# h-walk/PSA

Hardware: AMD Instinct MI355X
Metric: SED throughput (k-points*timesteps*atoms/s) (higher is better)
Workload: dtype f32 (2xf16 split MFMA, fp32 accumulate)

## Files before the change

### include/psa_hip.h

```cpp
#ifndef PSA_HIP_H
#define PSA_HIP_H

#include <stdint.h>

#ifdef __cplusplus
extern "C" {
#endif

#define PSA_HIP_ABI_VERSION 6

#define PSA_OK          0
#define PSA_EINVAL     -1
#define PSA_EHIP       -2
#define PSA_EFFT       -3
#define PSA_ERCCL      -4
#define PSA_ESTATE     -5
#define PSA_ENOMEM     -6

#define PSA_SLOT_VELOCITIES 0
#define PSA_SLOT_POSITIONS  1
#define PSA_NUM_SLOTS       2

#define PSA_F_DISPLACEMENTS  0x1
#define PSA_F_INTENSITY      0x2

#define PSA_K1_AUTO   0
#define PSA_K1_WAVE   1
#define PSA_K1_MFMA32 2
#define PSA_K1_SPLIT_BF16 3

typedef struct psa_ctx psa_ctx;

int         psa_abi_version(void);
const char* psa_last_error(void);
int         psa_device_count(int* count);
int         psa_host_alloc(size_t bytes, void** out);
int         psa_host_free(void* p);
int         psa_create(int device, psa_ctx** out);
int         psa_destroy(psa_ctx* ctx);
int         psa_synchronize(psa_ctx* ctx);
int         psa_set_k1(psa_ctx* ctx, int selector);
#define PSA_OPT_PLANES         0
#define PSA_OPT_PLANES_BUDGET  1
#define PSA_OPT_PLANES_EAGER   2
#define PSA_OPT_PLANES_MIN_K   3
#define PSA_OPT_FOLD_PAIRS     4
#define PSA_OPT_FFT_PRIME      5
#define PSA_OPT_K1_LOADER_WAVES 6
#define PSA_OPT_K1_WIDE         7
#define PSA_OPT_K1_LOWRANK      8
#define PSA_OPT_K1_LOWRANK_MIN_K 9
#define PSA_OPT_K1_LOWRANK_MIN_LOCAL 10
#define PSA_OPT_VDOS_WORK_BYTES 11
#define PSA_OPT_MODES_WORK_BYTES 12
#define PSA_OPT_DYNAMIC_WORK_BYTES 13
#define PSA_OPT_K1_LOWRANK_PAIR 15
int         psa_set_option(psa_ctx* ctx, int option, int64_t value);
int         psa_option_info(int index, int32_t* option, int64_t* default_value, const char** name);
int         psa_device_info(psa_ctx* ctx, char* name, int name_len,
                            int* compute_units, int64_t* hbm_bytes);

int psa_data_upload(psa_ctx* ctx, int slot, const float* host, int64_t T, int64_t N);
int psa_data_alloc(psa_ctx* ctx, int slot, int64_t T, int64_t N);
int psa_data_download(psa_ctx* ctx, int slot, float* host, int64_t t0, int64_t nt);
int psa_data_release(psa_ctx* ctx, int slot);
int psa_data_shape(psa_ctx* ctx, int slot, int64_t* T, int64_t* N);

int psa_data_fill_synthetic(psa_ctx* ctx, int slot, uint64_t seed, int64_t t_offset, int n_modes,
                            const float* amp, const int32_t* mode_comp,
                            const float* ct, const float* st,
                            const float* ca, const float* sa);

int psa_mean_positions(psa_ctx* ctx, int slot, float* mean_host );

int psa_host_mean_frames(const float* x , int64_t T, int64_t cols, float* mean_out, int threads);

int psa_set_atom_weights(psa_ctx* ctx, const float* w , int64_t N);

int psa_set_segments(psa_ctx* ctx, int64_t L, int64_t hop, const float* window );

int psa_sed_project(psa_ctx* ctx, int slot,
                    const float* mean_pos_all,
                    const float* k_vectors, int64_t K_local,
                    int64_t K_total, int64_t k_offset,
                    const int32_t* group_idx, const int64_t* group_off, int32_t G,
                    int32_t flags);

int psa_sed_project_upload(psa_ctx* ctx, int slot, const float* host, int64_t T, int64_t N,
                           const float* mean_pos_all, const float* k_vectors, int64_t K,
                           const int32_t* group_idx, const int64_t* group_off, int32_t G,
                           int32_t flags);

int psa_sed_finalize(psa_ctx* ctx, void* out_host, size_t out_bytes,
                     float* out_intensity, size_t out_intensity_bytes);

int psa_sed_calculate(psa_ctx* ctx, int slot, const float* mean_pos_all,
                      const float* k_vectors, int64_t K,
                      const int32_t* group_idx, const int64_t* group_off, int32_t G,
                      int32_t flags, void* out_host, size_t out_bytes,
                      float* out_intensity, size_t out_intensity_bytes);

int psa_vdos(psa_ctx* ctx, int slot, const float* mean_pos_all ,
             const int32_t* group_idx, const int64_t* group_off, int32_t G,
             int32_t flags , float* out_host , size_t out_bytes);

int psa_sed_modes(psa_ctx* ctx, int slot, const float* mean_pos_all, const float* k_vectors, int64_t K,
                  const int32_t* group_idx, const int64_t* group_off, int32_t B,
                  const void* eig , int64_t M, int32_t flags ,
                  float* out_host , size_t out_bytes);

int psa_sed_covariance(psa_ctx* ctx, int slot, const float* mean_pos_all, const float* k_vectors, int64_t K,
                       const int32_t* group_idx, const int64_t* group_off, int32_t B,
                       const float* freq_weights , int32_t n_w, int32_t flags ,
                       double* out_host , size_t out_bytes);

typedef struct {
    float   window_hwhm;
    int32_t half_window_bins;
    int32_t max_iter;
} psa_peak_opts;
int psa_fit_peaks(psa_ctx* ctx, const float* spec_host, int64_t F, int64_t C, double df, const int32_t* bands, int32_t lo,
                  int32_t hi, const psa_peak_opts* opts, float* fit , int32_t* info );
int psa_sed_modes_fit(psa_ctx* ctx, int slot, const float* mean_pos_all, const float* k_vectors, int64_t K,
                      const int32_t* group_idx, const int64_t* group_off, int32_t B, const void* eig, int64_t M,
                      int32_t flags, double df, const int32_t* bands, int32_t lo, int32_t hi, const psa_peak_opts* opts,
                      float* fit , int32_t* info , float* out_host, size_t out_bytes);

int psa_sed_modes_welch(psa_ctx* ctx, int slot, const float* mean_pos_all, const float* k_vectors, int64_t K,
                        const int32_t* group_idx, const int64_t* group_off, int32_t B,
                        const void* eig , int64_t M, int32_t flags ,
                        float* out_host , size_t out_bytes);
int psa_sed_modes_welch_fit(psa_ctx* ctx, int slot, const float* mean_pos_all, const float* k_vectors, int64_t K,
                            const int32_t* group_idx, const int64_t* group_off, int32_t B, const void* eig, int64_t M,
                            int32_t flags, double df, const int32_t* bands, int32_t lo, int32_t hi, const psa_peak_opts* opts,
                            float* fit , int32_t* info , float* out_host, size_t out_bytes);

int psa_dynamic_spectra(psa_ctx* ctx, const float* k_vectors, int64_t K, const int32_t* idx, int64_t n_g,
                        int32_t currents , float* out_host ,
                        size_t out_bytes);

int psa_lattice_spectra(psa_ctx* ctx, const double* box_inverse , const int32_t* indices , int64_t K,
                        const int32_t* bin_of , int64_t n_bins, const int32_t* idx, int64_t n_g,
                        int32_t currents , float* out_host ,
                        size_t out_bytes);

int psa_self_spectra(psa_ctx* ctx, const double* box_inverse , const int32_t* indices , int64_t K,
                     const int32_t* bin_of , int64_t n_bins, const int32_t* idx, int64_t n_g,
                     float* out_host , size_t out_bytes);

int psa_partial_spectra(psa_ctx* ctx, const double* box_inverse , const int32_t* indices , int64_t K,
                        const int32_t* bin_of , int64_t n_bins, const int32_t* idx, const int64_t* species_start ,
                        int32_t n_species, int32_t currents ,
                        float* out_host , size_t out_bytes);

int psa_lattice_correlations(psa_ctx* ctx, const double* box_inverse , const int32_t* indices , int64_t K,
                             const int32_t* bin_of , int64_t n_bins, const int32_t* idx, int64_t n_g,
                             int32_t currents , int64_t n_lags,
                             float* out_host , size_t out_bytes);

int psa_self_correlations(psa_ctx* ctx, const double* box_inverse , const int32_t* indices , int64_t K,
                          const int32_t* bin_of , int64_t n_bins, const int32_t* idx, int64_t n_g, int64_t n_lags,
                          float* out_host , size_t out_bytes);

int psa_displacement_moments(psa_ctx* ctx, const double* box , const double* box_inverse , const int32_t* idx,
                             const int64_t* group_start , int32_t n_groups, int64_t n_lags, int64_t origin_step,
                             int32_t unwrap, double* out_host , size_t out_bytes);

int psa_van_hove_self(psa_ctx* ctx, const double* box , const double* box_inverse , const int32_t* idx,
                      const int64_t* group_start , int32_t n_groups, const int64_t* lags , int64_t n_vh,
                      int64_t origin_step, int32_t unwrap, double dr, int32_t n_r, uint64_t* out_host ,
                      size_t out_bytes);

int psa_pair_histogram(psa_ctx* ctx, const double* box , const double* box_inverse , const int32_t* idx,
                       const int64_t* group_start , int32_t n_groups, const int64_t* lags , int64_t n_lags,
                       int64_t origin_step, double dr, int32_t n_r, uint64_t* out_host ,
                       size_t out_bytes);

int psa_angle_histogram(psa_ctx* ctx, const double* box , const double* box_inverse , const int32_t* idx,
                        const int64_t* group_start , int32_t n_groups, const double* r_cut , int64_t origin_step,
                        int32_t n_theta, uint64_t* angles , size_t angles_bytes,
                        uint64_t* coord , size_t coord_bytes, uint64_t* truncated );

int psa_bond_order(psa_ctx* ctx, const double* box , const double* box_inverse , const int32_t* idx,
                   const int64_t* group_start , int32_t n_groups, const double* r_cut , int64_t origin_step,
                   const int32_t* ls , int32_t n_ls, int32_t n_q, uint64_t* hist , size_t hist_bytes,
                   uint64_t* truncated , uint64_t* isolated , uint64_t* undefined ,
                   int64_t* x , int32_t* n );

#define PSA_KMAP_MIRROR 0x80000000u
int psa_k_pairs(const float* k_vectors, int64_t K, int32_t* kmap ,
                int32_t* unique_idx , int64_t* n_unique);
int psa_sed_set_kmap(psa_ctx* ctx, const int32_t* kmap, int64_t K_out);

int psa_lowrank_plan(const float* k_vectors, int64_t K, const float* mean_pos_all, int64_t N, const int32_t* idx,
                     int64_t n_g, int32_t* ok, double* geo, double* kappa, float* C, float* L, float* phi);

int psa_sed_single_bin(psa_ctx* ctx, int slot, const float* mean_pos_all, const float* k_vector,
                       const int32_t* idx, int64_t n_g, int32_t flags, int64_t i_w,
                       float* out_c64x3 );

int psa_slab_read(psa_ctx* ctx, int64_t row0, int64_t nrows, void* host);
int psa_slab_write(psa_ctx* ctx, int64_t row0, int64_t nrows, const void* host);

int psa_result_intensity(psa_ctx* ctx, float* out_host , size_t out_bytes);
int psa_result_chiral_phase(psa_ctx* ctx, int c1, int c2, float* out_host, size_t out_bytes);

int psa_last_timings(psa_ctx* ctx, double* ms );
int psa_k1_stats(psa_ctx* ctx, int64_t* launches, double* total_ms);
int psa_k1_lowrank_launches(psa_ctx* ctx, int64_t* launches);
int psa_k1_lowrank_pair_launches(psa_ctx* ctx, int64_t* launches);
int psa_lowrank_pair_image(int32_t n_stage, int64_t* index, int64_t* bytes);
int psa_debug_device_buffers(int64_t* count, int64_t* bytes);
#define PSA_SCRATCH_REAL 0
#define PSA_SCRATCH_INDEX 1
#define PSA_SCRATCH_STATE 2
int psa_debug_scratch_info(int index, const char** name, int32_t* cls);
int psa_debug_scratch_fill(psa_ctx* ctx, int byte, int64_t* buffers, int64_t* bytes);
int psa_oneoff_stats(psa_ctx* ctx, double* ms );

int psa_debug_phase_table(psa_ctx* ctx, const float* mean_pos_all,
                          const float* k_vectors, int64_t K,
                          const int32_t* idx, int64_t n_g, int64_t N,
                          void* out_host);
int psa_debug_project_only(psa_ctx* ctx, int slot, const float* mean_pos_all,
                           const float* k_vectors, int64_t K,
                           const int32_t* idx, int64_t n_g, int32_t flags,
                           void* out_host);
int psa_debug_project_route(psa_ctx* ctx, int slot, const float* mean_pos_all,
                            const float* k_vectors, int64_t K,
                            const int32_t* idx, int64_t n_g, int32_t flags,
                            void* out_host);
int psa_debug_project_frames(psa_ctx* ctx, int slot, const float* mean_pos_all,
                             const float* k_vectors, int64_t K,
                             const int32_t* idx, int64_t n_g, int32_t flags,
                             int64_t t_begin, int64_t t_count, void* out_host);
int psa_debug_mode_power(psa_ctx* ctx, const void* S_host, const void* eig, int32_t B, int64_t K, int64_t M, int64_t T,
                         float* out_host);
int psa_debug_covariance(psa_ctx* ctx, const void* S_host , int32_t B, int64_t K,
                         int64_t T, const float* freq_weights, int32_t n_w, double scale, double* out_host);
int psa_debug_mode_power_welch(psa_ctx* ctx, const void* S_host, const void* eig, int32_t B, int64_t K, int64_t M, int64_t L,
                               int64_t ns, int64_t seg_block, float scale, float* out_host);
int psa_debug_dynamic_project(psa_ctx* ctx, const float* k_vectors, int64_t K, const int32_t* idx, int64_t n_g,
                              int32_t currents, void* out_host);
int psa_debug_dynamic_sincos(psa_ctx* ctx, const float* turns, int64_t n, float* out_host);
int psa_debug_lattice_project(psa_ctx* ctx, const double* box_inverse, const int32_t* indices, int64_t K, const int32_t* idx,
                              int64_t n_g, int32_t currents, void* out_host);
int psa_debug_self_series(psa_ctx* ctx, const double* box_inverse, const int32_t* indices, int64_t K, const int32_t* idx,
                          int64_t n_g, void* out_host);
int psa_debug_dynamic_power(psa_ctx* ctx, const void* seg_host, const float* k_vectors , int64_t K, int32_t currents,
                            int64_t n_seg, int64_t L, int64_t k_block, int64_t seg_block, float scale, float* out_host);
int psa_debug_lattice_shell(psa_ctx* ctx, const void* seg_host, const float* khat , const int32_t* bin_of ,
                            int64_t K, int64_t n_bins, int32_t currents, int64_t n_seg, int64_t L, int64_t k_block,
                            int64_t seg_block, double norm, float* out_host);
int psa_debug_self_power(psa_ctx* ctx, const void* work_host, int64_t na, int64_t nv, int64_t n_seg, int64_t L,
                         const int32_t* groups, int64_t n_groups, int64_t cols, const double* scale, int32_t mirror,
                         int64_t n_chunks, int64_t atom_block, int64_t vec_block, int64_t seg_block, float* out_host);
int psa_debug_partial_project(psa_ctx* ctx, const double* box_inverse, const int32_t* indices, int64_t K, const int32_t* idx,
                              const int64_t* species_start, int32_t n_species, int32_t currents, void* out_host);
int psa_debug_partial_power(psa_ctx* ctx, const void* seg_host, const float* khat , const int32_t* bin_of ,
                            int64_t K, int64_t n_bins, int32_t n_species, int32_t currents, int64_t n_seg, int64_t L,
                            int64_t k_block, int64_t seg_block, double norm, float* out_host);
int psa_debug_plane_cache(psa_ctx* ctx, int64_t* n_sets, int64_t* bytes);

#define PSA_UNIQUE_ID_BYTES 128
int psa_comm_unique_id(void* out );
int psa_comm_init(psa_ctx* ctx, const void* unique_id, int rank, int nranks);
int psa_comm_destroy(psa_ctx* ctx);
int psa_comm_selftest(psa_ctx* ctx);
int psa_sed_gather(psa_ctx* ctx, int root, const int64_t* k_offsets, const int64_t* k_counts);
int psa_comm_barrier(psa_ctx* ctx);

int psa_sed_fs_project(psa_ctx* ctx, int slot, const float* mean_pos_all,
                       const float* k_vectors, int64_t K_total,
                       const int32_t* idx, int64_t n_g, int32_t flags,
                       int64_t T_total, int64_t k_offset, int64_t k_count);
int psa_sed_fs_exchange(psa_ctx* ctx, const int64_t* t_offsets, const int64_t* t_counts,
                        const int64_t* k_offsets, const int64_t* k_counts);
int psa_sed_fs_read(psa_ctx* ctx, int64_t k0, int64_t nk, void* host);
int psa_sed_fs_write(psa_ctx* ctx, int64_t t0, int64_t nt, const void* host);
int psa_sed_fs_finish(psa_ctx* ctx, int32_t first_group);

int psa_debug_correlation_transform(psa_ctx* ctx, const double* X_host, int64_t fields, int64_t P, int64_t cols, int64_t L,
                                    int64_t n_seg, int64_t n_lags, int32_t as_float32, float* out_host);

int psa_debug_unwrap(psa_ctx* ctx, const double* box , const double* box_inverse , const int32_t* idx, int64_t n_g,
                     int32_t unwrap, double* out_u , int32_t* out_images );

int psa_debug_pair_fractions(psa_ctx* ctx, const double* box_inverse , const int32_t* idx, int64_t n_g,
                             float* out );

int psa_debug_pair_plan(const int64_t* sizes , int32_t n_groups, int32_t sym, int64_t n_origins, int64_t* out );

int psa_debug_neighbour_lists(psa_ctx* ctx, const double* box , const double* box_inverse , const int32_t* idx,
                              const int64_t* group_start , int32_t n_groups, const double* r_cut , int64_t frame,
                              int32_t* count , int32_t* list );

#ifdef __cplusplus
}
#endif
#endif
```

### psa_amd/_hip.py

```python
from __future__ import annotations

import ctypes as C
import os
import threading
import weakref
from pathlib import Path
from typing import Optional, Sequence

import numpy as np

LIB_PATH = Path(__file__).resolve().parent / "csrc" / "libpsa_hip.so"

SLOT_VELOCITIES, SLOT_POSITIONS = 0, 1
F_DISPLACEMENTS, F_INTENSITY = 0x1, 0x2
K1_AUTO, K1_WAVE, K1_MFMA32, K1_SPLIT_BF16 = 0, 1, 2, 3
OPT_PLANES, OPT_PLANES_BUDGET, OPT_PLANES_EAGER, OPT_PLANES_MIN_K, OPT_FOLD_PAIRS, OPT_FFT_PRIME = 0, 1, 2, 3, 4, 5
OPT_K1_LOADER_WAVES = 6
OPT_K1_WIDE = 7
OPT_K1_LOWRANK = 8
OPT_K1_LOWRANK_MIN_K = 9
OPT_K1_LOWRANK_MIN_LOCAL = 10
OPT_VDOS_WORK_BYTES = 11
OPT_MODES_WORK_BYTES = 12
OPT_DYNAMIC_WORK_BYTES = 13
OPT_K1_LOWRANK_PAIR = 15
KMAP_MIRROR = 0x80000000
ABI_VERSION = 6
COV_CHAIN = 128
COV_FOLDS = 32
COV_TILE = 64
COV_CHUNK = COV_CHAIN * COV_FOLDS
COV_MAX_ROWS = 96
DYN_THREADS = 256
DYN_ATOMS = 512
DYN_CHAIN = 128
DYN_FRAMES = 4
DYN_SINCOS_ERR = 2.6e-7
LAT_THREADS = 256
LAT_KS = 512
LAT_ATOMS = 128
LAT_TABLE = 3584
LAT_CHAIN = 128
LAT_FRAMES = 4
LAT_MAX_INDEX = 64
LAT_MAX_ENTRIES = 3 * (2 * LAT_MAX_INDEX + 1)
PARTIAL_MAX_SPECIES = 8
SELF_THREADS = 256
SELF_ATOMS = 4
SELF_FRAMES = 64
SELF_ENTRIES = 24
SELF_KS = 64
MSD_LAGS = 256
MSD_ORIGINS = 1024
MSD_WINDOW = 1280
MSD_MAX_GROUPS = 8
MSD_MAX_BINS = 1024
MSD_MAX_VH_LAGS = 64
MSD_UNWRAP_FRAMES = 64
MSD_UNWRAP_ATOMS = 16
PAIR_TILE = 256
PAIR_MAX_BINS = 1024
PAIR_MAX_LAGS = 64
PAIR_MAX_SPECIES = 8
ANGLE_MAX_NEIGHBOURS = 64
ANGLE_MAX_BINS = 1024
ORDER_MAX_L = 12
ORDER_MAX_LS = 8
ORDER_MAX_BINS = 1024
ORDER_SHIFT = 24
UNIQUE_ID_BYTES = 128
TIMING_NAMES = ("h2d", "phase", "project", "fft", "epilogue", "gather", "transpose", "d2h")

_f32p = C.POINTER(C.c_float)
_i32p = C.POINTER(C.c_int32)
_i64p = C.POINTER(C.c_int64)
_f64p = C.POINTER(C.c_double)
_u64p = C.POINTER(C.c_uint64)
_ctx = C.c_void_p

SIGNATURES = {
    "psa_abi_version": (C.c_int, []),
    "psa_last_error": (C.c_char_p, []),
    "psa_device_count": (C.c_int, [C.POINTER(C.c_int)]),
    "psa_host_alloc": (C.c_int, [C.c_size_t, C.POINTER(C.c_void_p)]),
    "psa_host_free": (C.c_int, [C.c_void_p]),
    "psa_create": (C.c_int, [C.c_int, C.POINTER(_ctx)]),
    "psa_destroy": (C.c_int, [_ctx]),
    "psa_synchronize": (C.c_int, [_ctx]),
    "psa_set_k1": (C.c_int, [_ctx, C.c_int]),
    "psa_set_option": (C.c_int, [_ctx, C.c_int, C.c_int64]),
    "psa_device_info": (C.c_int, [_ctx, C.c_char_p, C.c_int, C.POINTER(C.c_int), _i64p]),
    "psa_data_upload": (C.c_int, [_ctx, C.c_int, _f32p, C.c_int64, C.c_int64]),
    "psa_data_alloc": (C.c_int, [_ctx, C.c_int, C.c_int64, C.c_int64]),
    "psa_data_download": (C.c_int, [_ctx, C.c_int, _f32p, C.c_int64, C.c_int64]),
    "psa_data_release": (C.c_int, [_ctx, C.c_int]),
    "psa_data_shape": (C.c_int, [_ctx, C.c_int, _i64p, _i64p]),
    "psa_data_fill_synthetic": (C.c_int, [_ctx, C.c_int, C.c_uint64, C.c_int64, C.c_int, _f32p, _i32p,
                                          _f32p, _f32p, _f32p, _f32p]),
    "psa_mean_positions": (C.c_int, [_ctx, C.c_int, _f32p]),
    "psa_host_mean_frames": (C.c_int, [_f32p, C.c_int64, C.c_int64, _f32p, C.c_int]),
    "psa_set_atom_weights": (C.c_int, [_ctx, _f32p, C.c_int64]),
    "psa_set_segments": (C.c_int, [_ctx, C.c_int64, C.c_int64, _f32p]),
    "psa_sed_project": (C.c_int, [_ctx, C.c_int, _f32p, _f32p, C.c_int64, C.c_int64, C.c_int64,
                                  _i32p, _i64p, C.c_int32, C.c_int32]),
    "psa_sed_project_upload": (C.c_int, [_ctx, C.c_int, _f32p, C.c_int64, C.c_int64, _f32p, _f32p, C.c_int64,
                                         _i32p, _i64p, C.c_int32, C.c_int32]),
    "psa_sed_finalize": (C.c_int, [_ctx, C.c_void_p, C.c_size_t, _f32p, C.c_size_t]),
    "psa_sed_calculate": (C.c_int, [_ctx, C.c_int, _f32p, _f32p, C.c_int64, _i32p, _i64p,
                                    C.c_int32, C.c_int32, C.c_void_p, C.c_size_t, _f32p, C.c_size_t]),
    "psa_vdos": (C.c_int, [_ctx, C.c_int, _f32p, _i32p, _i64p, C.c_int32, C.c_int32, _f32p, C.c_size_t]),
    "psa_sed_modes": (C.c_int, [_ctx, C.c_int, _f32p, _f32p, C.c_int64, _i32p, _i64p, C.c_int32, C.c_void_p, C.c_int64,
                                C.c_int32, _f32p, C.c_size_t]),
    "psa_fit_peaks": (C.c_int, [_ctx, _f32p, C.c_int64, C.c_int64, C.c_double, _i32p, C.c_int32, C.c_int32, C.c_void_p,
                                _f32p, _i32p]),
    "psa_sed_modes_fit": (C.c_int, [_ctx, C.c_int, _f32p, _f32p, C.c_int64, _i32p, _i64p, C.c_int32, C.c_void_p, C.c_int64,
                                    C.c_int32, C.c_double, _i32p, C.c_int32, C.c_int32, C.c_void_p, _f32p, _i32p, _f32p,
                                    C.c_size_t]),
    "psa_sed_modes_welch": (C.c_int, [_ctx, C.c_int, _f32p, _f32p, C.c_int64, _i32p, _i64p, C.c_int32, C.c_void_p, C.c_int64,
                                      C.c_int32, _f32p, C.c_size_t]),
    "psa_sed_modes_welch_fit": (C.c_int, [_ctx, C.c_int, _f32p, _f32p, C.c_int64, _i32p, _i64p, C.c_int32, C.c_void_p,
                                          C.c_int64, C.c_int32, C.c_double, _i32p, C.c_int32, C.c_int32, C.c_void_p, _f32p,
                                          _i32p, _f32p, C.c_size_t]),
    "psa_dynamic_spectra": (C.c_int, [_ctx, _f32p, C.c_int64, _i32p, C.c_int64, C.c_int32, _f32p, C.c_size_t]),
    "psa_debug_dynamic_project": (C.c_int, [_ctx, _f32p, C.c_int64, _i32p, C.c_int64, C.c_int32, C.c_void_p]),
    "psa_debug_dynamic_sincos": (C.c_int, [_ctx, _f32p, C.c_int64, _f32p]),
    "psa_lattice_spectra": (C.c_int, [_ctx, _f64p, _i32p, C.c_int64, _i32p, C.c_int64, _i32p, C.c_int64, C.c_int32,
                                      _f32p, C.c_size_t]),
    "psa_debug_lattice_project": (C.c_int, [_ctx, _f64p, _i32p, C.c_int64, _i32p, C.c_int64, C.c_int32, C.c_void_p]),
    "psa_self_spectra": (C.c_int, [_ctx, _f64p, _i32p, C.c_int64, _i32p, C.c_int64, _i32p, C.c_int64, _f32p,
                                   C.c_size_t]),
    "psa_debug_self_series": (C.c_int, [_ctx, _f64p, _i32p, C.c_int64, _i32p, C.c_int64, C.c_void_p]),
    "psa_debug_dynamic_power": (C.c_int, [_ctx, C.c_void_p, _f32p, C.c_int64, C.c_int32, C.c_int64, C.c_int64, C.c_int64, C.c_int64,
                                          C.c_float, _f32p]),
    "psa_debug_lattice_shell": (C.c_int, [_ctx, C.c_void_p, _f32p, _i32p, C.c_int64, C.c_int64, C.c_int32, C.c_int64, C.c_int64,
                                          C.c_int64, C.c_int64, C.c_double, _f32p]),
    "psa_debug_self_power": (C.c_int, [_ctx, C.c_void_p, C.c_int64, C.c_int64, C.c_int64, C.c_int64, _i32p, C.c_int64, C.c_int64,
                                       _f64p, C.c_int32, C.c_int64, C.c_int64, C.c_int64, C.c_int64, _f32p]),
    "psa_partial_spectra": (C.c_int, [_ctx, _f64p, _i32p, C.c_int64, _i32p, C.c_int64, _i32p, _i64p, C.c_int32,
                                      C.c_int32, _f32p, C.c_size_t]),
    "psa_debug_partial_project": (C.c_int, [_ctx, _f64p, _i32p, C.c_int64, _i32p, _i64p, C.c_int32, C.c_int32,
                                            C.c_void_p]),
    "psa_debug_partial_power": (C.c_int, [_ctx, C.c_void_p, _f32p, _i32p, C.c_int64, C.c_int64, C.c_int32, C.c_int32, C.c_int64,
                                          C.c_int64, C.c_int64, C.c_int64, C.c_double, _f32p]),
    "psa_lattice_correlations": (C.c_int, [_ctx, _f64p, _i32p, C.c_int64, _i32p, C.c_int64, _i32p, C.c_int64,
                                           C.c_int32, C.c_int64, _f32p, C.c_size_t]),
    "psa_self_correlations": (C.c_int, [_ctx, _f64p, _i32p, C.c_int64, _i32p, C.c_int64, _i32p, C.c_int64,
                                        C.c_int64, _f32p, C.c_size_t]),
    "psa_debug_correlation_transform": (C.c_int, [_ctx, _f64p, C.c_int64, C.c_int64, C.c_int64, C.c_int64,
                                                  C.c_int64, C.c_int64, C.c_int32, _f32p]),
    "psa_displacement_moments": (C.c_int, [_ctx, _f64p, _f64p, _i32p, _i64p, C.c_int32, C.c_int64,
                                           C.c_int64, C.c_int32, _f64p, C.c_size_t]),
    "psa_van_hove_self": (C.c_int, [_ctx, _f64p, _f64p, _i32p, _i64p, C.c_int32, _i64p, C.c_int64,
                                    C.c_int64, C.c_int32, C.c_double, C.c_int32, _u64p, C.c_size_t]),
    "psa_debug_unwrap": (C.c_int, [_ctx, _f64p, _f64p, _i32p, C.c_int64, C.c_int32,
                                   _f64p, _i32p]),
    "psa_pair_histogram": (C.c_int, [_ctx, _f64p, _f64p, _i32p, _i64p, C.c_int32, _i64p, C.c_int64,
                                     C.c_int64, C.c_double, C.c_int32, _u64p, C.c_size_t]),
    "psa_debug_pair_fractions": (C.c_int, [_ctx, _f64p, _i32p, C.c_int64, _f32p]),
    "psa_debug_pair_plan": (C.c_int, [_i64p, C.c_int32, C.c_int32, C.c_int64, _i64p]),
    "psa_angle_histogram": (C.c_int, [_ctx, _f64p, _f64p, _i32p, _i64p, C.c_int32, _f64p,
                                      C.c_int64, C.c_int32, _u64p, C.c_size_t, _u64p, C.c_size_t,
                                      _u64p]),
    "psa_debug_neighbour_lists": (C.c_int, [_ctx, _f64p, _f64p, _i32p, _i64p, C.c_int32,
                                            _f64p, C.c_int64, _i32p, _i32p]),
    "psa_bond_order": (C.c_int, [_ctx, _f64p, _f64p, _i32p, _i64p, C.c_int32, _f64p, C.c_int64,
                                 _i32p, C.c_int32, C.c_int32, _u64p, C.c_size_t, _u64p, _u64p, _u64p,
                                 _i64p, _i32p]),
    "psa_k_pairs": (C.c_int, [_f32p, C.c_int64, _i32p, _i32p, _i64p]),
    "psa_lowrank_plan": (C.c_int, [_f32p, C.c_int64, _f32p, C.c_int64, _i32p, C.c_int64, _i32p, _f64p,
                                   _f64p, _f32p, _f32p, _f32p]),
    "psa_sed_set_kmap": (C.c_int, [_ctx, _i32p, C.c_int64]),
    "psa_sed_single_bin": (C.c_int, [_ctx, C.c_int, _f32p, _f32p, _i32p, C.c_int64, C.c_int32, C.c_int64, _f32p]),
    "psa_slab_read": (C.c_int, [_ctx, C.c_int64, C.c_int64, C.c_void_p]),
    "psa_slab_write": (C.c_int, [_ctx, C.c_int64, C.c_int64, C.c_void_p]),
    "psa_result_intensity": (C.c_int, [_ctx, _f32p, C.c_size_t]),
    "psa_result_chiral_phase": (C.c_int, [_ctx, C.c_int, C.c_int, _f32p, C.c_size_t]),
    "psa_last_timings": (C.c_int, [_ctx, _f64p]),
    "psa_k1_stats": (C.c_int, [_ctx, _i64p, _f64p]),
    "psa_k1_lowrank_launches": (C.c_int, [_ctx, _i64p]),
    "psa_k1_lowrank_pair_launches": (C.c_int, [_ctx, _i64p]),
    "psa_lowrank_pair_image": (C.c_int, [C.c_int32, _i64p, _i64p]),
    "psa_oneoff_stats": (C.c_int, [_ctx, _f64p]),
    "psa_option_info": (C.c_int, [C.c_int, C.POINTER(C.c_int32), _i64p, C.POINTER(C.c_char_p)]),
    "psa_debug_device_buffers": (C.c_int, [_i64p, _i64p]),
    "psa_debug_scratch_info": (C.c_int, [C.c_int, C.POINTER(C.c_char_p), C.POINTER(C.c_int32)]),
    "psa_debug_scratch_fill": (C.c_int, [_ctx, C.c_int, _i64p, _i64p]),
    "psa_debug_phase_table": (C.c_int, [_ctx, _f32p, _f32p, C.c_int64, _i32p, C.c_int64,
                                        C.c_int64, C.c_void_p]),
    "psa_debug_project_only": (C.c_int, [_ctx, C.c_int, _f32p, _f32p, C.c_int64, _i32p,
                                         C.c_int64, C.c_int32, C.c_void_p]),
    "psa_debug_project_route": (C.c_int, [_ctx, C.c_int, _f32p, _f32p, C.c_int64, _i32p,
                                          C.c_int64, C.c_int32, C.c_void_p]),
    "psa_debug_project_frames": (C.c_int, [_ctx, C.c_int, _f32p, _f32p, C.c_int64, _i32p,
                                           C.c_int64, C.c_int32, C.c_int64, C.c_int64, C.c_void_p]),
    "psa_debug_mode_power": (C.c_int, [_ctx, C.c_void_p, C.c_void_p, C.c_int32, C.c_int64, C.c_int64, C.c_int64, _f32p]),
    "psa_debug_mode_power_welch": (C.c_int, [_ctx, C.c_void_p, C.c_void_p, C.c_int32, C.c_int64, C.c_int64, C.c_int64,
                                             C.c_int64, C.c_int64, C.c_float, _f32p]),
    "psa_sed_covariance": (C.c_int, [_ctx, C.c_int, _f32p, _f32p, C.c_int64, _i32p, _i64p, C.c_int32, _f32p, C.c_int32, C.c_int32,
                                     C.c_void_p, C.c_size_t]),
    "psa_debug_covariance": (C.c_int, [_ctx, C.c_void_p, C.c_int32, C.c_int64, C.c_int64, _f32p, C.c_int32, C.c_double,
                                       C.c_void_p]),
    "psa_debug_plane_cache": (C.c_int, [_ctx, _i64p, _i64p]),
    "psa_comm_unique_id": (C.c_int, [C.c_void_p]),
    "psa_comm_init": (C.c_int, [_ctx, C.c_void_p, C.c_int, C.c_int]),
    "psa_comm_destroy": (C.c_int, [_ctx]),
    "psa_comm_selftest": (C.c_int, [_ctx]),
    "psa_sed_gather": (C.c_int, [_ctx, C.c_int, _i64p, _i64p]),
    "psa_comm_barrier": (C.c_int, [_ctx]),
    "psa_sed_fs_project": (C.c_int, [_ctx, C.c_int, _f32p, _f32p, C.c_int64, _i32p, C.c_int64, C.c_int32,
                                     C.c_int64, C.c_int64, C.c_int64]),
    "psa_sed_fs_exchange": (C.c_int, [_ctx, _i64p, _i64p, _i64p, _i64p]),
    "psa_sed_fs_read": (C.c_int, [_ctx, C.c_int64, C.c_int64, C.c_void_p]),
    "psa_sed_fs_write": (C.c_int, [_ctx, C.c_int64, C.c_int64, C.c_void_p]),
    "psa_sed_fs_finish": (C.c_int, [_ctx, C.c_int32]),
}


class PeakOpts(C.Structure):
    _fields_ = [("window_hwhm", C.c_float), ("half_window_bins", C.c_int32), ("max_iter", C.c_int32)]


class PsaHipError(RuntimeError):
    """A libpsa_hip entry point returned a non-zero code."""


_lib = None
_lib_lock = threading.Lock()


def load_library() -> C.CDLL:
    global _lib
    with _lib_lock:
        if _lib is not None:
            return _lib
        path = Path(os.environ.get("PSA_HIP_LIBRARY", LIB_PATH))
        if not path.exists():
            raise PsaHipError(
                f"{path} not found: build it with `make -C psa_amd/csrc` (needs hipcc, gfx950). "
                "psa_amd has no CPU fallback.")
        os.environ.setdefault("HSA_ENABLE_IPC_MODE_LEGACY", "0")
        lib = C.CDLL(str(path))
        for name, (res, args) in SIGNATURES.items():
            fn = getattr(lib, name)
            fn.restype, fn.argtypes = res, args
        _lib = lib
        return lib


def _check(rc: int, what: str):
    if rc != 0:
        msg = load_library().psa_last_error().decode("utf-8", "replace")
        if rc == -1 and "out of bounds" in msg:
            raise ValueError(msg)
        raise PsaHipError(f"{what} failed (rc={rc}): {msg}")


def _f32(a: np.ndarray):
    return a.ctypes.data_as(_f32p)


def _as_f32(a, shape_tail=None) -> np.ndarray:
    arr = np.ascontiguousarray(a, dtype=np.float32)
    if shape_tail is not None and arr.shape[1:] != shape_tail:
        raise ValueError(f"expected (*,{shape_tail}) array, got {arr.shape}")
    return arr


def device_count() -> int:
    n = C.c_int(0)
    _check(load_library().psa_device_count(C.byref(n)), "psa_device_count")
    return n.value


def option_table():
    lib, rows = load_library(), []
    opt, default, name = C.c_int32(0), C.c_int64(0), C.c_char_p()
    while lib.psa_option_info(len(rows), C.byref(opt), C.byref(default), C.byref(name)) == 0:
        rows.append((opt.value, name.value.decode(), default.value))
    return rows


def device_buffers():
    n, b = C.c_int64(0), C.c_int64(0)
    _check(load_library().psa_debug_device_buffers(C.byref(n), C.byref(b)), "psa_debug_device_buffers")
    return n.value, b.value


SCRATCH_CLASSES = ("real", "index", "state")


def scratch_table():
    lib, rows = load_library(), []
    name, cls = C.c_char_p(), C.c_int32(0)
    while lib.psa_debug_scratch_info(len(rows), C.byref(name), C.byref(cls)) == 0:
        rows.append((name.value.decode(), SCRATCH_CLASSES[cls.value]))
    return rows


def k_pairs(k_vectors):
    kv = _as_f32(k_vectors, (3,)) if len(k_vectors) else np.zeros((0, 3), np.float32)
    K = kv.shape[0]
    kmap, uidx, n = np.zeros(K, np.int32), np.zeros(K, np.int32), C.c_int64(0)
    _check(load_library().psa_k_pairs(_f32(kv), K, kmap.ctypes.data_as(_i32p), uidx.ctypes.data_as(_i32p), C.byref(n)),
           "psa_k_pairs")
    return kmap.view(np.uint32), uidx[:n.value].copy()


def lowrank_plan(k_vectors, mean_pos_all, idx=None):
    kv = _as_f32(k_vectors, (3,))
    mean = _as_f32(mean_pos_all, (3,))
    K, N = kv.shape[0], mean.shape[0]
    ix = None if idx is None else np.ascontiguousarray(idx, np.int32)
    n_g = N if ix is None else ix.size
    ok, geo = C.c_int32(0), np.zeros(12, np.float64)
    kappa, cm = np.zeros(64, np.float64), np.zeros((K, 64), np.complex64)
    lw, phi = np.zeros((K, 64), np.float32), np.zeros(K, np.complex64)
    _check(load_library().psa_lowrank_plan(_f32(kv), K, _f32(mean), N, None if ix is None else ix.ctypes.data_as(_i32p), n_g,
                                           C.byref(ok), geo.ctypes.data_as(_f64p), kappa.ctypes.data_as(_f64p),
                                           cm.ctypes.data_as(_f32p), _f32(lw), phi.ctypes.data_as(_f32p)), "psa_lowrank_plan")
    if not ok.value:
        return None
    return {"u": geo[0:3].copy(), "k0": geo[3:6].copy(), "x_c": geo[6], "h_x": geo[7], "width": geo[8],
            "interval": int(geo[9]), "d_bound": geo[10], "dscale": geo[11], "kappa": kappa, "C": cm, "L": lw, "phi": phi}


def lowrank_pair_image(n_stage: int):
    index, nbytes = np.zeros((512, 32 * int(n_stage)), np.int64), C.c_int64(0)
    _check(load_library().psa_lowrank_pair_image(int(n_stage), index.ctypes.data_as(_i64p), C.byref(nbytes)), "psa_lowrank_pair_image")
    return index, nbytes.value


def host_mean_frames(x: np.ndarray, threads: int = 0) -> np.ndarray:
    if x.dtype != np.float32 or not x.flags.c_contiguous or x.ndim < 2 or x.shape[0] < 1 or x.size == 0:
        raise ValueError("host_mean_frames needs a non-empty C-contiguous float32 array")
    out = np.empty(x.shape[1:], np.float32)
    cols = int(np.prod(x.shape[1:], dtype=np.int64))
    _check(load_library().psa_host_mean_frames(_f32(x), x.shape[0], cols, _f32(out), int(threads)), "psa_host_mean_frames")
    return out


def pack_groups(groups: Optional[Sequence[np.ndarray]]):
    if groups is None:
        return None, None, 1
    off = np.zeros(len(groups) + 1, dtype=np.int64)
    off[1:] = np.cumsum([len(g) for g in groups])
    idx = (np.concatenate([np.asarray(g).ravel() for g in groups]) if off[-1] > 0
           else np.zeros(0, dtype=np.int64))
    if idx.size and (idx.min() < 0 or idx.max() >= 2 ** 31):
        raise ValueError("Atom indices in basis out of bounds.")
    return np.ascontiguousarray(idx, dtype=np.int32), off, len(groups)


class _PinnedPool:

    granule = 2 << 20
    min_bytes = 1 << 20
    keep_bytes = 4 << 30
    max_live_bytes = 16 << 30

    def __init__(self):
        self._idle = {}
        self._idle_bytes = 0
        self._live_bytes = 0
        self._lock = threading.Lock()
        self.stats = {"recycled": 0, "allocated": 0, "pageable": 0}

    def _give_back(self, address: int, size: int):
        with self._lock:
            self._live_bytes -= size
            if self._idle_bytes + size <= self.keep_bytes:
                self._idle.setdefault(size, []).append(address)
                self._idle_bytes += size
                return
        load_library().psa_host_free(C.c_void_p(address))

    def empty(self, shape, dtype) -> np.ndarray:
        dtype = np.dtype(dtype)
        nbytes = int(np.prod(shape, dtype=np.int64)) * dtype.itemsize
        if nbytes < self.min_bytes:
            return np.empty(shape, dtype)
        size = -(-nbytes // self.granule) * self.granule
        with self._lock:
            if self._live_bytes + size > self.max_live_bytes:
                self.stats["pageable"] += 1
                return np.empty(shape, dtype)
            self._live_bytes += size
            stack = self._idle.get(size)
            address = stack.pop() if stack else None
            if address is not None:
                self._idle_bytes -= size
        if address is None:
            p = C.c_void_p()
            try:
                _check(load_library().psa_host_alloc(size, C.byref(p)), "psa_host_alloc")
            except PsaHipError:
                with self._lock:
                    self._live_bytes -= size
                    self.stats["pageable"] += 1
                return np.empty(shape, dtype)
            address = p.value
            self.stats["allocated"] += 1
        else:
            self.stats["recycled"] += 1
        block = (C.c_char * size).from_address(address)
        weakref.finalize(block, self._give_back, address, size)
        return np.frombuffer(block, dtype=dtype, count=nbytes // dtype.itemsize).reshape(shape)

    def drain(self):
        with self._lock:
            idle, self._idle, self._idle_bytes = self._idle, {}, 0
        for stack in idle.values():
            for address in stack:
                load_library().psa_host_free(C.c_void_p(address))


_pinned_pool = _PinnedPool()


def pinned_empty(shape, dtype) -> np.ndarray:
    return _pinned_pool.empty(shape, dtype)


_SAMPLE_CACHE = {}


def _sample_positions(shape):
    hit = _SAMPLE_CACHE.get(shape)
    if hit is None:
        size = int(np.prod(shape, dtype=np.int64))
        lin = np.arange(0, size, max(1, size // 1021), dtype=np.int64)[:1021]
        if size > 2048:
            lin = np.concatenate([lin, np.sort(np.random.default_rng(size).integers(0, size, 1021)), [size - 1]])
        if len(_SAMPLE_CACHE) > 64:
            _SAMPLE_CACHE.clear()
        hit = _SAMPLE_CACHE[shape] = (lin, np.unravel_index(lin, shape))
    return hit


class Engine:

    def __init__(self, device: Optional[int] = None):
        self._lib = load_library()
        if device is None:
            device = int(os.environ.get("PSA_HIP_DEVICE", os.environ.get("LOCAL_RANK", "0")))
            n = device_count()
            if n == 0:
                raise PsaHipError("no HIP device visible; psa_amd has no CPU fallback")
            device %= n
        h = _ctx()
        _check(self._lib.psa_create(int(device), C.byref(h)), "psa_create")
        self._h = h
        self.device = int(device)
        self._resident = {}
        self._converted = {}
        self.lock = threading.RLock()
        self.rank, self.nranks = 0, 1
        self.result_serial = 0
        self.segment_length = 0

    def close(self):
        if getattr(self, "_h", None):
            self._lib.psa_destroy(self._h)
            self._h = None

    def __del__(self):
        try:
            self.close()
        except Exception:
            pass

    def synchronize(self):
        _check(self._lib.psa_synchronize(self._h), "psa_synchronize")

    def set_k1(self, selector: int):
        _check(self._lib.psa_set_k1(self._h, selector), "psa_set_k1")

    def device_info(self) -> dict:
        name = C.create_string_buffer(256)
        cu, mem = C.c_int(0), C.c_int64(0)
        _check(self._lib.psa_device_info(self._h, name, 256, C.byref(cu), C.byref(mem)),
               "psa_device_info")
        return {"name": name.value.decode(), "compute_units": cu.value, "hbm_bytes": mem.value}

    @staticmethod
    def _fingerprint(a: np.ndarray) -> int:
        if a.size == 0:
            return 0
        base = a
        while base is not None and not isinstance(base, np.memmap):
            base = getattr(base, "base", None)
        if base is not None and getattr(base, "filename", None):
            try:
                st = os.stat(base.filename)
                return hash((str(base.filename), st.st_size, st.st_mtime_ns, a.shape, a.strides))
            except OSError:
                pass
        lin, idx = _sample_positions(a.shape)
        if a.flags.c_contiguous:
            return hash(a.reshape(-1)[lin].tobytes())
        return hash(a[idx].tobytes())

    def _as_device_layout(self, slot: int, array: np.ndarray) -> np.ndarray:
        if array.ndim != 3 or array.shape[2] != 3:
            raise ValueError("trajectory array must be (frames, atoms, 3)")
        if array.dtype == np.float32 and array.flags.c_contiguous:
            return array
        held = self._converted.get(slot)
        fp = self._fingerprint(array)
        if held is not None and held[0]() is array and held[1] == fp:
            return held[2]
        conv = np.ascontiguousarray(array, dtype=np.float32)
        try:
            self._converted[slot] = (weakref.ref(array), fp, conv)
        except TypeError:
            self._converted.pop(slot, None)
        return conv

    def is_resident(self, slot: int, array: np.ndarray) -> bool:
        held = self._resident.get(slot)
        if held is None or held[0] is None:
            return False
        a = array if held[0]() is array else self._as_device_layout(slot, array)
        return (held[0]() is a and held[1:3] == (a.ctypes.data, a.shape) and held[3] == self._fingerprint(a))

    def _note_resident(self, slot: int, a: np.ndarray):
        try:
            ref = weakref.ref(a)
        except TypeError:
            ref = None
        self._resident[slot] = (ref, a.ctypes.data, a.shape, self._fingerprint(a))

    def ensure_resident(self, slot: int, array: np.ndarray):
        if self.is_resident(slot, array):
            return
        a = self._as_device_layout(slot, array)
        T, N = a.shape[0], a.shape[1]
        _check(self._lib.psa_data_upload(self._h, slot, _f32(a), T, N), "psa_data_upload")
        self._note_resident(slot, a)

    def invalidate(self, slot: Optional[int] = None):
        if slot is None:
            self._resident.clear()
            self._converted.clear()
        else:
            self._resident.pop(slot, None)
            self._converted.pop(slot, None)

    def alloc(self, slot: int, T: int, N: int):
        _check(self._lib.psa_data_alloc(self._h, slot, T, N), "psa_data_alloc")
        self._resident[slot] = (None, None, (T, N, 3), None)

    def fill_synthetic(self, slot: int, seed: int, amp, comp, ct, st, ca, sa, t_offset: int = 0):
        amp = np.ascontiguousarray(amp, np.float32)
        comp = np.ascontiguousarray(comp, np.int32)
        tabs = [np.ascontiguousarray(x, np.float32) for x in (ct, st, ca, sa)]
        _check(self._lib.psa_data_fill_synthetic(
            self._h, slot, C.c_uint64(seed), int(t_offset), len(amp), _f32(amp), comp.ctypes.data_as(_i32p),
            *[_f32(t) for t in tabs]), "psa_data_fill_synthetic")

    def set_option(self, option: int, value: int):
        _check(self._lib.psa_set_option(self._h, option, int(value)), "psa_set_option")

    def reset_options(self):
        for option, _, default in option_table():
            self.set_option(option, default)

    def scratch_fill(self, byte: int):
        n, b = C.c_int64(0), C.c_int64(0)
        _check(self._lib.psa_debug_scratch_fill(self._h, int(byte), C.byref(n), C.byref(b)), "psa_debug_scratch_fill")
        return n.value, b.value

    def plane_cache(self):
        n, b = C.c_int64(0), C.c_int64(0)
        _check(self._lib.psa_debug_plane_cache(self._h, C.byref(n), C.byref(b)), "psa_debug_plane_cache")
        return n.value, b.value

    def download(self, slot: int, t0: int, nt: int) -> np.ndarray:
        T, N = self.shape(slot)
        out = np.empty((nt, N, 3), np.float32)
        _check(self._lib.psa_data_download(self._h, slot, _f32(out), t0, nt), "psa_data_download")
        return out

    def release(self, slot: int):
        _check(self._lib.psa_data_release(self._h, slot), "psa_data_release")
        self._resident.pop(slot, None)

    def shape(self, slot: int):
        T, N = C.c_int64(0), C.c_int64(0)
        _check(self._lib.psa_data_shape(self._h, slot, C.byref(T), C.byref(N)), "psa_data_shape")
        return T.value, N.value

    def mean_positions(self, slot: int) -> np.ndarray:
        _, N = self.shape(slot)
        out = np.empty((N, 3), np.float32)
        _check(self._lib.psa_mean_positions(self._h, slot, _f32(out)), "psa_mean_positions")
        return out

    def set_atom_weights(self, weights: Optional[np.ndarray]):
        if weights is None:
            _check(self._lib.psa_set_atom_weights(self._h, None, 0), "psa_set_atom_weights")
            return
        w = np.ascontiguousarray(weights, np.float32)
        if w.ndim != 1 or w.size == 0:
            raise ValueError(f"atom weights must be a non-empty (N,) array, got shape {w.shape}")
        if not np.all(np.isfinite(w)):
            raise ValueError("atom weights must be finite")
        _check(self._lib.psa_set_atom_weights(self._h, _f32(w), w.shape[0]), "psa_set_atom_weights")

    def set_segments(self, segments):
        if segments is None:
            _check(self._lib.psa_set_segments(self._h, 0, 0, None), "psa_set_segments")
            self.segment_length = 0
            return
        w = np.ascontiguousarray(segments.window_array(), np.float32)
        _check(self._lib.psa_set_segments(self._h, segments.length, segments.hop, _f32(w)), "psa_set_segments")
        self.segment_length = segments.length

    def project(self, slot, mean_pos_all, k_vectors, groups=None, flags=0,
                K_total=None, k_offset=0):
        mean = _as_f32(mean_pos_all, (3,))
        kv = _as_f32(k_vectors, (3,)) if len(k_vectors) else np.zeros((0, 3), np.float32)
        idx, off, G = pack_groups(groups)
        K_local = kv.shape[0]
        self.result_serial += 1
        _check(self._lib.psa_sed_project(
            self._h, slot, _f32(mean), _f32(kv), K_local,
            K_local if K_total is None else K_total, k_offset,
            idx.ctypes.data_as(_i32p) if idx is not None else None,
            off.ctypes.data_as(_i64p) if off is not None else None, G, flags),
            "psa_sed_project")

    def project_upload(self, slot, array, mean_pos_all, k_vectors, groups=None, flags=0):
        a = self._as_device_layout(slot, array)
        mean = _as_f32(mean_pos_all, (3,))
        kv = _as_f32(k_vectors, (3,))
        idx, off, G = pack_groups(groups)
        self._resident.pop(slot, None)
        self.result_serial += 1
        _check(self._lib.psa_sed_project_upload(
            self._h, slot, _f32(a), a.shape[0], a.shape[1], _f32(mean), _f32(kv), kv.shape[0],
            idx.ctypes.data_as(_i32p) if idx is not None else None,
            off.ctypes.data_as(_i64p) if off is not None else None, G, flags), "psa_sed_project_upload")
        self._note_resident(slot, a)

    def finalize(self, T: int, K: int, intensity: bool, fetch: bool = True, with_intensity: bool = False):
        if not fetch:
            _check(self._lib.psa_sed_finalize(self._h, None, 0, None, 0), "psa_sed_finalize")
            return (None, None) if with_intensity else None
        out = pinned_empty((T, K), np.float32) if intensity else pinned_empty((T, K, 3), np.complex64)
        inten = pinned_empty((T, K), np.float32) if with_intensity and not intensity else None
        _check(self._lib.psa_sed_finalize(self._h, out.ctypes.data_as(C.c_void_p), out.nbytes,
                                          _f32(inten) if inten is not None else None,
                                          inten.nbytes if inten is not None else 0), "psa_sed_finalize")
        return (out, inten) if with_intensity else out

    def single_bin(self, slot, mean_pos_all, k_vector, idx, i_w: int, flags=0) -> np.ndarray:
        mean = _as_f32(mean_pos_all, (3,))
        kv = np.ascontiguousarray(k_vector, np.float32).reshape(3)
        ii = None if idx is None else np.ascontiguousarray(idx, np.int32)
        out = np.empty(3, np.complex64)
        _check(self._lib.psa_sed_single_bin(
            self._h, slot, _f32(mean), _f32(kv), ii.ctypes.data_as(_i32p) if ii is not None else None,
            0 if ii is None else len(ii), flags, int(i_w), out.ctypes.data_as(_f32p)), "psa_sed_single_bin")
        return out

    def calculate(self, slot, mean_pos_all, k_vectors, groups=None, flags=0, with_intensity: bool = False):
        T, _ = self.shape(slot)
        T = self.segment_length or T
        mean = _as_f32(mean_pos_all, (3,))
        kv = _as_f32(k_vectors, (3,))
        idx, off, G = pack_groups(groups)
        K = kv.shape[0]
        intensity = bool(flags & F_INTENSITY)
        out = pinned_empty((T, K), np.float32) if intensity else pinned_empty((T, K, 3), np.complex64)
        inten = pinned_empty((T, K), np.float32) if with_intensity and not intensity else None
        self.result_serial += 1
        _check(self._lib.psa_sed_calculate(
            self._h, slot, _f32(mean), _f32(kv), K,
            idx.ctypes.data_as(_i32p) if idx is not None else None,
            off.ctypes.data_as(_i64p) if off is not None else None, G, flags,
            out.ctypes.data_as(C.c_void_p), out.nbytes,
            _f32(inten) if inten is not None else None, inten.nbytes if inten is not None else 0), "psa_sed_calculate")
        return (out, inten) if with_intensity else out

    def vdos(self, slot, mean_pos_all, groups=None, flags=0) -> np.ndarray:
        T, N = self.shape(slot)
        L = self.segment_length or T
        mean = None if mean_pos_all is None else _as_f32(mean_pos_all, (3,))
        idx, off, G = pack_groups(groups)
        out = np.empty((G, 3, L // 2 + 1), np.float32)
        _check(self._lib.psa_vdos(
            self._h, slot, _f32(mean) if mean is not None else None,
            idx.ctypes.data_as(_i32p) if idx is not None else None,
            off.ctypes.data_as(_i64p) if off is not None else None, G, flags, _f32(out), out.nbytes), "psa_vdos")
        return np.ascontiguousarray(out.transpose(2, 0, 1))

    @staticmethod
    def _index_args(idx):
        if idx is None:
            return None, None, 0
        ii = np.ascontiguousarray(idx, np.int32).ravel()
        keep = ii if ii.size else np.zeros(1, np.int32)
        return keep, keep.ctypes.data_as(_i32p), int(ii.size)

    @staticmethod
    def _dynamic_args(k_vectors, idx):
        return (_as_f32(np.asarray(k_vectors, np.float32).reshape(-1, 3), (3,)),) + Engine._index_args(idx)

    def dynamic_spectra(self, k_vectors, idx=None, currents: bool = True) -> np.ndarray:
        T, _ = self.shape(SLOT_POSITIONS)
        L = self.segment_length or T
        kv, keep, ip, n_g = self._dynamic_args(k_vectors, idx)
        out = np.empty((3 if currents else 1, L, kv.shape[0]), np.float32)
        _check(self._lib.psa_dynamic_spectra(self._h, _f32(kv), kv.shape[0], ip, n_g, 1 if currents else 0, _f32(out), out.nbytes),
               "psa_dynamic_spectra")
        return out

    def debug_dynamic_project(self, k_vectors, idx=None, currents: bool = True) -> np.ndarray:
# ... 582 lines not shown
```

### psa_amd/csrc/api_core.hip

```cpp
#include "api_internal.h"

#include <unistd.h>

#include <atomic>
#include <filesystem>

namespace psa {

thread_local std::string g_error;


void set_error(const char* fmt, ...) {
    char    buf[1024];
    va_list ap;
    va_start(ap, fmt);
    vsnprintf(buf, sizeof(buf), fmt, ap);
    va_end(ap);
    g_error = buf;
}

static std::atomic<int64_t> g_devbuf_count{0}, g_devbuf_bytes{0};

int DevBuf::reserve(size_t bytes) {
    if (bytes <= cap) return PSA_OK;
// ... 228 lines not shown
static const int SCRATCH_ZERO = 0;

}

psa_ctx::psa_ctx() {
    for (const psa::Option& o : psa::OPTIONS) this->*o.field = o.def;
}

psa_ctx::~psa_ctx() {
    if (stream) (void)hipStreamSynchronize(stream);
    if (fft_primer.joinable()) fft_primer.join();
    if (comm) (void)ncclCommDestroy(comm);
    for (auto& p : timing.pending) {
        (void)hipEventDestroy(p.e0);
        (void)hipEventDestroy(p.e1);
    }
    for (auto ev : timing.pool) (void)hipEventDestroy(ev);
    psa::stager_release(this);
    if (d2h_stream) (void)hipStreamDestroy(d2h_stream);
    if (d2h_ready) (void)hipEventDestroy(d2h_ready);
    if (stream) (void)hipStreamDestroy(stream);
}

using namespace psa;

extern "C" {

int psa_abi_version(void) { return PSA_HIP_ABI_VERSION; }

const char* psa_last_error(void) { return g_error.c_str(); }

int psa_device_count(int* count) {
    PSA_REQUIRE(count != nullptr, "null count");
    PSA_HIP_CHECK(hipGetDeviceCount(count));
    return PSA_OK;
}

int psa_host_alloc(size_t bytes, void** out) {
    PSA_REQUIRE(out != nullptr && bytes > 0, "bad argument");
    PSA_HIP_CHECK(hipHostMalloc(out, bytes, hipHostMallocDefault));
    return PSA_OK;
}

int psa_host_free(void* p) {
    if (p) PSA_HIP_CHECK(hipHostFree(p));
    return PSA_OK;
}

int psa_create(int device, psa_ctx** out) {
    PSA_REQUIRE(out != nullptr, "null out");
    int n = 0;
    PSA_HIP_CHECK(hipGetDeviceCount(&n));
    PSA_REQUIRE(device >= 0 && device < n, "device %d out of range (%d visible)", device, n);
    PSA_HIP_CHECK(hipSetDevice(device));
    hipDeviceProp_t prop;
    PSA_HIP_CHECK(hipGetDeviceProperties(&prop, device));
    PSA_REQUIRE(std::strncmp(prop.gcnArchName, "gfx950", 6) == 0,
                "libpsa_hip is built for gfx950 (MI355X) only; device %d is %s", device,
                prop.gcnArchName);
    static std::once_flag fft_once;
    std::call_once(fft_once, [] {
        if (!std::getenv("ROCFFT_RTC_CACHE_PATH")) {
            std::string dir;
            if (const char* e = std::getenv("PSA_CACHE_DIR")) dir = e;
            else if (const char* x = std::getenv("XDG_CACHE_HOME")) dir = std::string(x) + "/psa_amd";
            else if (const char* h = std::getenv("HOME")) dir = std::string(h) + "/.cache/psa_amd";
            if (!dir.empty()) {
                std::error_code ec;
                std::filesystem::create_directories(dir, ec);
                if (!ec && ::access(dir.c_str(), W_OK) == 0)
                    ::setenv("ROCFFT_RTC_CACHE_PATH", (dir + "/rocfft_rtc_cache.db").c_str(), 0);
            }
        }
        (void)rocfft_setup();
    });
    psa_ctx* c = new psa_ctx();
    c->device = device;
    c->compute_units = prop.multiProcessorCount;
    if (const char* v = std::getenv("PSA_K1_LOWRANK")) c->opt_k1_lowrank = std::atoi(v) != 0;
    if (const char* v = std::getenv("PSA_K1_LOWRANK_MIN_K")) c->opt_k1_lowrank_min_k = std::max(1, std::atoi(v));
    hipError_t e = hipStreamCreateWithFlags(&c->stream, hipStreamNonBlocking);
    if (e != hipSuccess) {
        delete c;
        set_error("hipStreamCreate failed: %s", hipGetErrorString(e));
        return PSA_EHIP;
    }
    *out = c;
    return PSA_OK;
}

int psa_destroy(psa_ctx* c) {
    if (!c) return PSA_OK;
    { Guard g(c); }
    (void)hipSetDevice(c->device);
    delete c;
    return PSA_OK;
}

int psa_debug_device_buffers(int64_t* count, int64_t* bytes) {
    PSA_REQUIRE(count != nullptr && bytes != nullptr, "null argument");
    *count = g_devbuf_count.load();
    *bytes = g_devbuf_bytes.load();
    return PSA_OK;
}

int psa_debug_scratch_info(int index, const char** name, int32_t* cls) {
    PSA_REQUIRE(index >= 0 && index < (int)std::size(SCRATCH), "no device buffer at index %d", index);
    if (name) *name = SCRATCH[index].name;
    if (cls) *cls = SCRATCH[index].cls;
    return PSA_OK;
}

int psa_debug_scratch_fill(psa_ctx* c, int byte, int64_t* buffers, int64_t* bytes) {
    PSA_TRY(enter(c));
    PSA_REQUIRE(byte >= -1 && byte <= 255, "the fill byte is 0 .. 255, or -1 to disarm");
    Guard g(c);
    PSA_HIP_CHECK(hipStreamSynchronize(c->stream));
    if (c->d2h_stream) PSA_HIP_CHECK(hipStreamSynchronize(c->d2h_stream));
    if (c->stager.copy_stream) PSA_HIP_CHECK(hipStreamSynchronize(c->stager.copy_stream));
    int64_t n = 0, total = 0;
    c->scratch_byte = byte;
    for (const Scratch& s : SCRATCH) {
        DevBuf& b = c->*s.member;
        b.fill = byte < 0 || s.cls == PSA_SCRATCH_STATE ? nullptr : s.cls == PSA_SCRATCH_REAL ? &c->scratch_byte : &SCRATCH_ZERO;
        if (!b.fill || !b.ptr) continue;
        PSA_HIP_CHECK(hipMemsetAsync(b.ptr, *b.fill, b.cap, c->stream));
        n += 1;
        total += (int64_t)b.cap;
    }
    PSA_HIP_CHECK(hipStreamSynchronize(c->stream));
    if (byte >= 0) c->slab_valid = c->out_valid = c->inten_valid = false;
    if (buffers) *buffers = n;
    if (bytes) *bytes = total;
    return PSA_OK;
}

int psa_synchronize(psa_ctx* c) {
    PSA_TRY(enter(c));
    Guard g(c);
    PSA_HIP_CHECK(hipStreamSynchronize(c->stream));
    return PSA_OK;
}

int psa_set_k1(psa_ctx* c, int selector) {
    PSA_TRY(enter(c));
    PSA_REQUIRE(selector == PSA_K1_AUTO || selector == PSA_K1_WAVE || selector == PSA_K1_MFMA32 ||
                    selector == PSA_K1_SPLIT_BF16,
                "unknown K1 selector %d", selector);
    Guard g(c);
    c->k1_selector = selector;
    return PSA_OK;
}

int psa_set_option(psa_ctx* c, int option, int64_t value) {
    PSA_TRY(enter(c));
    Guard g(c);
    for (const Option& o : OPTIONS) {
        if (o.id != option) continue;
        if (o.min == OPT_FLAG) value = value != 0;
        else if (o.min == 0) PSA_REQUIRE(value >= 0, "negative plane budget");
        else PSA_REQUIRE(value >= o.min, "%s must be >= %lld", o.name, (long long)o.min);
        c->*o.field = value;
        if (option == PSA_OPT_PLANES && !value) {
            PSA_HIP_CHECK(hipStreamSynchronize(c->stream));
            c->planes.clear();
        } else if (option == PSA_OPT_K1_LOWRANK && !value) {
            PSA_HIP_CHECK(hipStreamSynchronize(c->stream));
            for (DevBuf* b : {&c->d_lr_diff, &c->d_lr_qn, &c->d_lr_L, &c->d_lr_phi, &c->d_lr_f64}) b->release();
        }
        return PSA_OK;
    }
    set_error("unknown option %d", option);
    return PSA_EINVAL;
}

int psa_option_info(int index, int32_t* option, int64_t* default_value, const char** name) {
    PSA_REQUIRE(index >= 0 && index < (int)std::size(OPTIONS), "no option at index %d", index);
    if (option) *option = OPTIONS[index].id;
    if (default_value) *default_value = OPTIONS[index].def;
    if (name) *name = OPTIONS[index].name;
    return PSA_OK;
}

int psa_device_info(psa_ctx* c, char* name, int name_len, int* compute_units, int64_t* hbm_bytes) {
    PSA_TRY(enter(c));
    hipDeviceProp_t prop;
    PSA_HIP_CHECK(hipGetDeviceProperties(&prop, c->device));
    if (name && name_len > 0) {
        std::snprintf(name, (size_t)name_len, "%s (%s)", prop.name[0] ? prop.name : "AMD GPU",
                      prop.gcnArchName);
    }
    if (compute_units) *compute_units = prop.multiProcessorCount;
    if (hbm_bytes) *hbm_bytes = (int64_t)prop.totalGlobalMem;
    return PSA_OK;
}

int psa_last_timings(psa_ctx* c, double* ms) {
    PSA_TRY(enter(c));
    PSA_REQUIRE(ms != nullptr, "null output");
    Guard guard(c);
    TimingState& ts = timing(c);
    PSA_TRY(collect(c, ts));
    for (int i = 0; i < PSA_T_COUNT; ++i) {
        ms[i] = ts.acc[i];
        ts.acc[i] = 0.0;
    }
    return PSA_OK;
}

int psa_oneoff_stats(psa_ctx* c, double* ms) {
    PSA_TRY(enter(c));
    PSA_REQUIRE(ms != nullptr, "null output");
    Guard guard(c);
    for (int i = 0; i < 4; ++i) {
        ms[i] = c->oneoff_ms[i];
        c->oneoff_ms[i] = 0.0;
    }
    return PSA_OK;
}

int psa_k1_lowrank_launches(psa_ctx* c, int64_t* launches) {
    PSA_TRY(enter(c));
    PSA_REQUIRE(launches != nullptr, "null argument");
    *launches = c->lowrank_launches;
    return PSA_OK;
}

int psa_k1_lowrank_pair_launches(psa_ctx* c, int64_t* launches) {
    PSA_TRY(enter(c));
    PSA_REQUIRE(launches != nullptr, "null argument");
    *launches = c->lowrank_pair_launches;
    return PSA_OK;
}

int psa_k1_stats(psa_ctx* c, int64_t* launches, double* total_ms) {
    PSA_TRY(enter(c));
    Guard guard(c);
    TimingState& ts = timing(c);
    PSA_TRY(collect(c, ts));
    if (launches) *launches = ts.k1_launches;
    if (total_ms) *total_ms = ts.k1_ms;
    ts.k1_launches = 0;
    ts.k1_ms = 0.0;
    return PSA_OK;
}

}
```

### psa_amd/csrc/api_internal.h

```cpp
#pragma once
#include <algorithm>
#include <chrono>
#include <cmath>
#include <condition_variable>
#include <cstdlib>
#include <cstring>
#include <functional>
#include <thread>
#include <unordered_map>

#include "k1_f16.h"

namespace psa {

extern thread_local std::string g_error;

struct HostTimer {
    double*                               into;
    std::chrono::steady_clock::time_point t0 = std::chrono::steady_clock::now();
    explicit HostTimer(double* into_) : into(into_) {}
    ~HostTimer() { *into += std::chrono::duration<double, std::milli>(std::chrono::steady_clock::now() - t0).count(); }
};

struct Guard {
    std::lock_guard<std::mutex> lk;
    explicit Guard(psa_ctx* c) : lk(c->mu) {}
};

int          enter(psa_ctx* c);
inline int synchronised(psa_ctx* c, int rc, const char* entry) {
    if (hipStreamSynchronize(c->stream) != hipSuccess && rc == PSA_OK) {
        set_error("hipStreamSynchronize failed after %s", entry);
        return PSA_EHIP;
    }
    return rc;
}
TimingState& timing(psa_ctx* c);
int          get_event(TimingState& ts, hipEvent_t* ev);
int          collect(psa_ctx* c, TimingState& ts);

struct StageTimer {
    psa_ctx*     c;
    TimingState& ts;
    int          stage;
    hipEvent_t   e0 = nullptr, e1 = nullptr;
    bool         ok = false;
    StageTimer(psa_ctx* c_, int stage_) : c(c_), ts(timing(c_)), stage(stage_) {
        if (get_event(ts, &e0) == PSA_OK && get_event(ts, &e1) == PSA_OK &&
            hipEventRecord(e0, c->stream) == hipSuccess)
            ok = true;
    }
    ~StageTimer() {
        if (ok && hipEventRecord(e1, c->stream) == hipSuccess) {
            ts.pending.push_back({stage, e0, e1});
            return;
        }
        for (hipEvent_t ev : {e0, e1})
            if (ev) ts.pool.push_back(ev);
    }
};

int upload(psa_ctx* c, DevBuf& b, const void* host, size_t bytes);
int get_plan(psa_ctx* c, int64_t T, int64_t batch, FftPlan** out);
void prime_fft(psa_ctx* c, int64_t T);
int run_fft(psa_ctx* c, float2* data, int64_t T, int64_t batch);
int check_slot(psa_ctx* c, int slot);
int validate_groups(int64_t N, const int32_t* group_idx, const int64_t* group_off, int32_t G);

struct GroupView {
    int            slot = 0;
    bool           disp = false;
    int64_t        n_g = 0;
    const int*     d_idx = nullptr;
    const int32_t* h_idx = nullptr;
    PlaneSet*      ps = nullptr;
};
inline void set_group(const psa_ctx* c, const int32_t* group_idx, const int64_t* group_off, int gi, int64_t N, GroupView* v) {
    v->n_g = group_idx ? group_off[gi + 1] - group_off[gi] : N;
    v->d_idx = group_idx ? c->d_idx.as<int>() + group_off[gi] : nullptr;
    v->h_idx = group_idx ? group_idx + group_off[gi] : nullptr;
}

int  slot_absmax(psa_ctx* c, int slot);
int  group_absmax(psa_ctx* c, int slot, const int32_t* h_idx, int64_t n_g, unsigned* bits);
int  displaced_absmax(psa_ctx* c, int slot, const float* mean_host, const int32_t* h_idx, int64_t n_g, unsigned* bits);
int  stager_init(psa_ctx* c, size_t chunk_bytes);
void stager_release(psa_ctx* c);
int  staged_upload(psa_ctx* c, float* dev, const float* host, int64_t T, int64_t N,
                   const std::function<int(int64_t, int64_t, hipEvent_t)>& on_chunk);
int  data_alloc_locked(psa_ctx* c, int slot, int64_t T, int64_t N);
int  materialise_displacements(psa_ctx* c, GroupView* v, const float* mean_host);

struct ProjectArgs {
    int            slot;
    const float*   mean_pos_all;
    const float*   k_vectors;
    int64_t        K_local, K_total, k_offset;
    const int32_t* group_idx;
    const int64_t* group_off;
    int32_t        G, flags;
};

enum class GeomRule { product, bf16_anywhere, f32_only };

size_t planes_bytes_held(psa_ctx* c);
void   drop_stale_planes(psa_ctx* c);
int    get_planes(psa_ctx* c, const GroupView& v, int64_t K_local, const float* mean_host, PlaneSet** out);
int    group_source(psa_ctx* c, GroupView* v, const float* mean_host, int64_t K);
int    make_geom(psa_ctx* c, const GroupView& v, int64_t K_local, GeomRule rule, ProjGeom* g);
int    prepare_phase(psa_ctx* c, const GroupView& v, const ProjGeom& g, int64_t k_first);
int    launch_projection(psa_ctx* c, const GroupView& v, ProjGeom g, float2* d_q, int64_t q_stride, int64_t t_begin,
                         int64_t t_count);
int    prepare_block(psa_ctx* c, const GroupView& v, GeomRule rule, const ProjectArgs* lowrank, int64_t k_first, int64_t nk,
                     ProjGeom* g);
int    project_block(psa_ctx* c, const GroupView& v, const ProjectArgs* lowrank, int64_t k_first, int64_t nk, float2* d_q);
int    check_group_indices(const GroupView& v, int64_t N);
int    upload_single_group(psa_ctx* c, GroupView* v, int64_t N, const float* k_vectors, int64_t K, const float* mean_pos_all);
void   fold_pairs(const float* k, int64_t K, std::vector<int32_t>* kmap, std::vector<int32_t>* unique_idx);
int    install_kmap(psa_ctx* c, const std::vector<int32_t>& kmap);
struct LowRankPlan {
    bool                ok = false;
    const char*         why = "";
    double              u[3] = {0, 0, 0}, k0[3] = {0, 0, 0};
    double              x_c = 0, h_x = 0, width = 0;
    int64_t             interval = 0;
    double              kappa[LOWRANK_NODES] = {};
    double              d_bound = 0;
    float               dscale = 0.f;
    std::vector<double> kline;
    std::vector<float>  L;
    std::vector<float>  phi;
};
int plan_lowrank(const float* k, int64_t K, const float* mean_all, int64_t N, const int32_t* h_idx, int64_t n_g, LowRankPlan* p,
                 float* C = nullptr);
int prepare_lowrank(psa_ctx* c, const GroupView& v, const ProjectArgs& list, int64_t k_first, int64_t nk, ProjGeom* g);
struct ModesArgs {
    int            slot;
    const float*   mean_pos_all;
    const float*   k_vectors;
    int64_t        K;
    const int32_t* group_idx;
    const int64_t* group_off;
    int32_t        B;
    const float*   eig;
    int64_t        M;
    int32_t        flags;
    float*         out;
    size_t         out_bytes;
};
int modes_run(psa_ctx* c, const ModesArgs& a, bool segments, bool device_only);
struct ModesCall {
    int64_t                T = 0, N = 0, K = 0, M = 0;
    int32_t                B = 0;
    int                    MT = 0;
    size_t                 coef_k = 0;
    int64_t                per_k = 0;
    int64_t                kb_max = 0;
    ProjectArgs            list;
    std::vector<float>     coef;
    std::vector<GroupView> src;
};
int     modes_check_groups(psa_ctx* c, int slot, const float* mean_pos_all, const float* k_vectors, int64_t K, const int32_t* group_idx,
                           const int64_t* group_off, int32_t B, int32_t flags, ModesCall* m);
int     modes_upload(psa_ctx* c, ModesCall* m);
int64_t modes_block(const psa_ctx* c, const ModesCall& m, int64_t k0, int64_t kb);
int     modes_project(psa_ctx* c, const ModesCall& m, int64_t k0, int64_t nk, float2* d_work);
struct PeakArgs {
    int64_t        F, C;
    double         df;
    const int32_t* bands;
    int32_t        lo, hi;
    psa_peak_opts  opts;
    float*         fit;
    int32_t*       info;
    int            row0 = 0, row_end = 0;
};
int check_peak_args(const psa_peak_opts* opts, PeakArgs* a);
int peaks_run(psa_ctx* c, const float* d_spec, const PeakArgs& a);
struct DynCall {
    int64_t T = 0, N = 0, K = 0, n_g = 0;
    int     NC = 1, slices = 1;
    int     n_species = 1;
    bool    cut = false;
    int64_t L = 0, H = 0, n_seg = 0;
    int64_t n_lags = 0, P = 0;
    int64_t per_k = 0, unit = 0;
    int64_t kb = 0, bk = 0, bs = 0;
    std::vector<float> kappa, khat;
};
int dynamic_inputs(psa_ctx* c, const char* entry, int64_t K, const int32_t* idx, int64_t n_g, int32_t currents, DynCall* d);
int segment_shape(const psa_ctx* c, bool segments, DynCall* d);
int dynamic_plan(psa_ctx* c, DynCall* d);
struct PowerPass {
    int          NC = 1;
    int          n_species = 0;
    int64_t      L = 0, n_seg = 0, K = 0;
    float        scale = 0.f;
    const float* d_khat = nullptr;
    float*       d_out = nullptr;
    const int*   d_bins = nullptr;
    double*      d_acc = nullptr;
    int64_t      n_bins = 0;
};
using SegFill = std::function<int(int64_t k1, int64_t nb, int64_t s0, int64_t ns, const float2** d_seg)>;
int  power_block(psa_ctx* c, const PowerPass& p, int64_t k0, int64_t nk, int64_t bk, int64_t bs, const SegFill& fill);
struct BlockSource {
    std::function<int()>                                                     upload;
    std::function<int(int64_t block, int64_t k0, int64_t nk, float2* d_q)> project;
};
struct SpectraRun {
    BlockSource src;
    bool        pairs = false;
    int64_t     n_bins = 0;
    std::function<int(const float* d_power, const double* d_acc)> finish;
    float*      out_host = nullptr;
    size_t      out_bytes = 0;
};
int spectra_run(psa_ctx* c, const DynCall& d, const SpectraRun& a);
int debug_project_run(psa_ctx* c, const DynCall& d, const BlockSource& src, void* out_host);
struct DebugPower {
    const void*    seg_host = nullptr;
    const int32_t* bin_of = nullptr;
    int64_t        K = 0, n_bins = 0;
    int            n_species = 0;
    int32_t        currents = 0;
    int64_t        n_seg = 0, L = 0, k_block = 0, seg_block = 0;
    double         norm = 1.0;
    float          scale = 0.f;
    float*         out_host = nullptr;
    int64_t        bk = 0, bs = 0;
};
int debug_power_check(DebugPower* a);
int debug_power_run(psa_ctx* c, const DebugPower& a, const float* khat);
int  upload_segments(psa_ctx* c, DevBuf& b, const void* host, int64_t r0, int64_t nr, int64_t n_seg, int64_t s0, int64_t ns, int64_t L);
void bin_counts(const int32_t* bin_of, int64_t K, int64_t n_bins, std::vector<int64_t>* count);
int  sorted_bin_counts(const int32_t* bin_of, int64_t K, int64_t n_bins, std::vector<int64_t>* count);
void lattice_bins(const std::vector<int64_t>& count, double n_seg, double U, double L, std::vector<int32_t>* bin_start,
                  std::vector<double>* scale);
int  shell_begin(psa_ctx* c, size_t bytes, double** d_acc);
int  shell_finish(psa_ctx* c, int64_t n, int64_t n_bins, float* d_out);

int  lattice_inputs(const double* box_inverse, const int32_t* indices, int64_t K, const int32_t* bin_of, int64_t n_bins);
void lattice_box_parts(const double* B, float* hi, float* lo);
void lattice_order(const int32_t* indices, int64_t K, const int32_t* bin_of, int64_t kb, std::vector<int64_t>* order);
int  lattice_tile_entries(const int32_t* indices, const int64_t* members, int64_t nt, std::vector<uint16_t>* ent, uint32_t* slot);
struct LatCall {
    DynCall  d;
    bool     shell = false;
    int64_t  n_bins = 0;
    float    box_hi[9], box_lo[9];
    std::vector<int64_t>  block_tile0;
    std::vector<int32_t>  tile_off, dest;
    std::vector<uint16_t> ent;
    std::vector<uint32_t> slot;
    std::vector<int64_t>  count;
    std::vector<int32_t>  bin_start;
    std::vector<double>   scale;
};
int lattice_plan(const psa_ctx* c, const double* box_inverse, const int32_t* indices, const int32_t* bin_of, int64_t n_bins,
                 int64_t row_mult, LatCall* p);
int lattice_check(psa_ctx* c, const char* entry, const double* box_inverse, const int32_t* indices, int64_t K, const int32_t* bin_of,
                  int64_t n_bins, const int32_t* idx, int64_t n_g, int32_t currents, int64_t n_lags, LatCall* p);
int lattice_upload(psa_ctx* c, const LatCall& p, const int32_t* idx);
int lattice_project(psa_ctx* c, const LatCall& p, bool listed, int64_t a0, int64_t n_g, int64_t block, float2* d_q);
BlockSource lattice_source(psa_ctx* c, const LatCall& p, const int32_t* idx);
struct SelfCall {
    DynCall  d;
    bool     shell = false;
    int64_t  cols = 0;
    float    box_hi[9], box_lo[9];
    std::vector<int64_t>  order;
    std::vector<int32_t>  tile;
    std::vector<uint16_t> ent;
    std::vector<uint32_t> slot;
    std::vector<int32_t>  groups;
    std::vector<int64_t>  count;
    std::vector<double>   scale;
    int64_t  n_tiles = 0, kt_max = 0, n_groups = 0;
    int64_t  at = 0, vt = 0, bs = 0;
};
int self_check(psa_ctx* c, const char* entry, const double* box_inverse, const int32_t* indices, int64_t K, const int32_t* bin_of,
// ... 44 lines not shown
```

### psa_amd/csrc/api_lowrank.hip

```cpp
#include "api_internal.h"
#include "k1_lowrank_pair.h"

namespace psa {

namespace {
constexpr double LR_OMEGA = 30.0;
constexpr double LR_D_MAX = 1.0 / 8192.0;
}

int plan_lowrank(const float* k, int64_t K, const float* mean_all, int64_t N, const int32_t* h_idx, int64_t n_g, LowRankPlan* p,
                 float* C) {
    *p = LowRankPlan{};
    auto fail = [&](const char* why) {
        p->why = why;
        return PSA_OK;
    };
    if (K < 2) return fail("fewer than two k-vectors");
    if (n_g < 1) return fail("empty group");
    for (int64_t i = 0; i < 3 * K; ++i)
        if (!std::isfinite(k[i])) return fail("k-vector not finite");
    double  p0[3] = {k[0], k[1], k[2]}, far = 0.0;
    int64_t jf = 0;
    for (int64_t j = 1; j < K; ++j) {
        double d2 = 0.0;
        for (int i = 0; i < 3; ++i) d2 += ((double)k[3 * j + i] - p0[i]) * ((double)k[3 * j + i] - p0[i]);
        if (d2 > far) {
            far = d2;
            jf = j;
        }
    }
    if (!(far > 0.0)) return fail("all k-vectors equal");
    double u[3], nu = std::sqrt(far);
    for (int i = 0; i < 3; ++i) u[i] = ((double)k[3 * jf + i] - p0[i]) / nu;
    {
        int im = 0;
        for (int i = 1; i < 3; ++i)
            if (std::fabs(u[i]) > std::fabs(u[im])) im = i;
        if (u[im] < 0)
            for (double& v : u) v = -v;
    }
    bool snapped = false;
    for (int n = 1; n <= 12 && !snapped; ++n) {
        double m[3], mn = 0.0, dev = 0.0;
        const double s = n / std::max({std::fabs(u[0]), std::fabs(u[1]), std::fabs(u[2])});
        for (int i = 0; i < 3; ++i) {
            m[i] = std::nearbyint(u[i] * s);
            mn += m[i] * m[i];
        }
        mn = std::sqrt(mn);
        for (int i = 0; i < 3; ++i) dev = std::max(dev, std::fabs(m[i] / mn - u[i]));
        if (dev < 1e-6) {
            for (int i = 0; i < 3; ++i) u[i] = m[i] / mn + 0.0;
            snapped = true;
        }
    }
    if (!snapped) return fail("direction not a lattice direction");
    {
        double kmax2 = 0.0, off2 = 0.0;
        for (int64_t j = 0; j < K; ++j) {
            double kj[3], d = 0.0, n2 = 0.0;
            for (int i = 0; i < 3; ++i) {
                kj[i] = k[3 * j + i];
                d += kj[i] * u[i];
                n2 += kj[i] * kj[i];
            }
            double o2 = 0.0;
            for (int i = 0; i < 3; ++i) o2 += (kj[i] - d * u[i]) * (kj[i] - d * u[i]);
            kmax2 = std::max(kmax2, n2);
            off2 = std::max(off2, o2);
        }
        if (!(std::sqrt(off2) <= 1e-5 * std::sqrt(kmax2))) return fail("line does not pass through Gamma");
    }
    for (int i = 0; i < 3; ++i) p->u[i] = u[i];
    double xmin = INFINITY, xmax = -INFINITY, rmax = 0.0, rabs[3] = {0, 0, 0};
    for (int64_t a = 0; a < n_g; ++a) {
        const int64_t src = h_idx ? h_idx[a] : a;
        if (src < 0 || src >= N) return fail("index outside the trajectory");
        const float* r = mean_all + 3 * src;
        if (!std::isfinite(r[0]) || !std::isfinite(r[1]) || !std::isfinite(r[2])) return fail("mean position not finite");
        const double x = u[0] * r[0] + u[1] * r[1] + u[2] * r[2];
        xmin = std::min(xmin, x);
        xmax = std::max(xmax, x);
        rmax = std::max(rmax, std::sqrt((double)r[0] * r[0] + (double)r[1] * r[1] + (double)r[2] * r[2]));
        for (int i = 0; i < 3; ++i) rabs[i] = std::max(rabs[i], (double)std::fabs(r[i]));
    }
    p->x_c = 0.5 * (xmin + xmax);
    p->h_x = std::max(0.5 * (xmax - xmin), 1e-12);
    p->width = 2.0 * LR_OMEGA / p->h_x;
    p->kline.resize((size_t)3 * K);
    std::vector<double> kap((size_t)K);
    double              off = 0.0, kabs[3] = {0, 0, 0};
    for (int64_t j = 0; j < K; ++j) {
        double kj[3], kk = 0.0;
        for (int i = 0; i < 3; ++i) {
            kj[i] = k[3 * j + i];
            kk += (kj[i] - p->k0[i]) * u[i];
            kabs[i] = std::max(kabs[i], std::fabs(kj[i]));
        }
        kap[(size_t)j] = kk;
        double e2 = 0.0;
        for (int i = 0; i < 3; ++i) {
            p->kline[3 * j + i] = p->k0[i] + kk * u[i];
            e2 += (kj[i] - p->kline[3 * j + i]) * (kj[i] - p->kline[3 * j + i]);
        }
        off = std::max(off, std::sqrt(e2));
    }
    p->d_bound = 0x1p-22 * (kabs[0] * rabs[0] + kabs[1] * rabs[1] + kabs[2] * rabs[2]) + off * rmax + 0x1p-20;
    if (!(p->d_bound <= LR_D_MAX)) return fail("k-vectors not on one line (or phases too large)");
    bool pos = true, neg = true;
    for (int64_t j = 0; j < K; ++j) {
        pos = pos && kap[(size_t)j] >= 0.0;
        neg = neg && kap[(size_t)j] <= 0.0;
    }
    if (!pos && !neg) return fail("k-list crosses Gamma");
    const bool   side = pos;
    const double n0 = std::floor(std::fabs(kap[0]) / p->width);
    for (int64_t j = 0; j < K; ++j)
        if (std::floor(std::fabs(kap[(size_t)j]) / p->width) != n0) return fail("k-path longer than one node interval");
    p->interval = side ? (int64_t)n0 : -(int64_t)n0 - 1;
    const double mid = (p->interval + 0.5) * p->width, half = 0.5 * p->width;
    double       bw[LOWRANK_NODES];
    for (int l = 0; l < LOWRANK_NODES; ++l) {
        const double th = M_PI * (2 * l + 1) / (2.0 * LOWRANK_NODES);
        p->kappa[l] = mid + half * std::cos(th);
        bw[l] = ((l & 1) ? -1.0 : 1.0) * std::sin(th);
    }
    p->L.assign((size_t)K * LOWRANK_NODES, 0.f);
    p->phi.assign((size_t)K * 2, 0.f);
    for (int64_t j = 0; j < K; ++j) {
        const double kj = kap[(size_t)j];
        double       L[LOWRANK_NODES], den = 0.0;
        int          hit = -1;
        for (int l = 0; l < LOWRANK_NODES; ++l)
            if (kj == p->kappa[l]) hit = l;
        if (hit >= 0) {
            for (int l = 0; l < LOWRANK_NODES; ++l) L[l] = l == hit;
        } else {
            for (int l = 0; l < LOWRANK_NODES; ++l) {
                L[l] = bw[l] / (kj - p->kappa[l]);
                den += L[l];
            }
            for (double& v : L) v /= den;
        }
        const double cr = std::cos(kj * p->x_c), ci = std::sin(kj * p->x_c);
        p->phi[(size_t)j * 2 + 0] = (float)cr;
        p->phi[(size_t)j * 2 + 1] = (float)ci;
        for (int l = 0; l < LOWRANK_NODES; ++l) {
            p->L[(size_t)j * LOWRANK_NODES + l] = (float)L[l];
            if (C) {
                C[((size_t)j * LOWRANK_NODES + l) * 2 + 0] = (float)(cr * L[l]);
                C[((size_t)j * LOWRANK_NODES + l) * 2 + 1] = (float)(ci * L[l]);
            }
        }
    }
    p->dscale = std::ldexp(1.0f, 14 - (int)std::ceil(std::log2(p->d_bound)));
    p->ok = true;
    return PSA_OK;
}

int prepare_lowrank(psa_ctx* c, const GroupView& v, const ProjectArgs& list, int64_t k_first, int64_t nk, ProjGeom* g) {
    g->lowrank = false;
    if (!c->opt_k1_lowrank || g->split != K1Family::f16_planes || !v.ps || list.K_total < c->opt_k1_lowrank_min_k ||
        nk < c->opt_k1_lowrank_min_local)
        return PSA_OK;
    LowRankPlan p;
    PSA_TRY(plan_lowrank(list.k_vectors + 3 * k_first, nk, list.mean_pos_all, c->slot[v.slot].N, v.h_idx, g->n_g, &p));
    if (!p.ok) return PSA_OK;
    std::vector<double> f64((size_t)7 + LOWRANK_NODES + 3 * (size_t)nk);
    std::memcpy(f64.data(), p.k0, 3 * sizeof(double));
    std::memcpy(f64.data() + 3, p.u, 3 * sizeof(double));
    f64[6] = p.x_c;
    std::memcpy(f64.data() + 7, p.kappa, sizeof(p.kappa));
    std::memcpy(f64.data() + 7 + LOWRANK_NODES, p.kline.data(), p.kline.size() * sizeof(double));
    PSA_TRY(upload(c, c->d_lr_f64, f64.data(), f64.size() * sizeof(double)));
    PSA_TRY(upload(c, c->d_lr_L, p.L.data(), p.L.size() * sizeof(float)));
    PSA_TRY(upload(c, c->d_lr_phi, p.phi.data(), p.phi.size() * sizeof(float)));
    PSA_TRY(c->d_lr_qn.reserve((size_t)LOWRANK_NODES * 3 * (size_t)c->slot[v.slot].T * sizeof(float2)));
    g->lowrank = true;
    g->dscale = p.dscale;
    g->M_pad_d = (int)((2 * nk + 511) / 512 * 512);
    g->lr_pair = c->opt_k1_lowrank_pair && g->M_pad_d == LRP_ROWS;
    return PSA_OK;
}

}

using namespace psa;

extern "C" {

int psa_lowrank_plan(const float* k_vectors, int64_t K, const float* mean_pos_all, int64_t N, const int32_t* idx, int64_t n_g,
                     int32_t* ok, double* geo, double* kappa, float* C, float* L, float* phi) {
    PSA_REQUIRE(K >= 0 && K < (1ll << 29) && N >= 1 && n_g >= 0 && n_g <= (idx ? (int64_t)1 << 30 : N) && ok && geo &&
                    (K == 0 || k_vectors) && mean_pos_all,
                "bad argument");
    LowRankPlan p;
    PSA_TRY(plan_lowrank(k_vectors, K, mean_pos_all, N, idx, n_g, &p, C));
    *ok = p.ok;
    const double g[12] = {p.u[0], p.u[1], p.u[2], p.k0[0], p.k0[1], p.k0[2], p.x_c, p.h_x, p.width, (double)p.interval, p.d_bound, p.dscale};
    std::memcpy(geo, g, sizeof(g));
    if (p.ok && kappa) std::memcpy(kappa, p.kappa, sizeof(p.kappa));
    if (p.ok && L) std::memcpy(L, p.L.data(), p.L.size() * sizeof(float));
    if (p.ok && phi) std::memcpy(phi, p.phi.data(), p.phi.size() * sizeof(float));
    return PSA_OK;
}

int psa_lowrank_pair_image(int32_t n_stage, int64_t* index, int64_t* bytes) {
    PSA_REQUIRE(n_stage >= 1 && n_stage < (1 << 20) && bytes, "bad argument");
    *bytes = (int64_t)pd16_pair_table_bytes(n_stage);
    if (index)
        for (int m = 0; m < LRP_ROWS; ++m)
            for (int a = 0; a < n_stage * K1_BA; ++a) index[(size_t)m * n_stage * K1_BA + a] = (int64_t)pd16_pair_index(m, a, n_stage);
    return PSA_OK;
}

}
```

### psa_amd/csrc/api_project.hip

```cpp
#include "api_internal.h"

namespace psa {

uint64_t hash_idx(const int32_t* p, int64_t n) {
    uint64_t h = 1469598103934665603ull ^ (uint64_t)n;
    for (int64_t i = 0; i < n; ++i) h = (h ^ (uint32_t)p[i]) * 1099511628211ull;
    return h;
}

void fold_pairs(const float* k, int64_t K, std::vector<int32_t>* kmap, std::vector<int32_t>* unique_idx) {
    struct Key {
        uint32_t x, y, z;
        bool operator==(const Key& o) const { return x == o.x && y == o.y && z == o.z; }
    };
    struct KeyHash {
        size_t operator()(const Key& a) const {
            uint64_t h = 1469598103934665603ull;
            for (uint32_t v : {a.x, a.y, a.z}) h = (h ^ v) * 1099511628211ull;
            return (size_t)h;
        }
    };
    auto bits = [](float v, bool negate) {
        if (negate) v = -v;
        if (v == 0.f) v = 0.f;
// ... 72 lines not shown
    c->planes.erase(c->planes.begin() + victim);
    return true;
}

int get_planes(psa_ctx* c, const GroupView& v, int64_t K_local, const float* mean_host, PlaneSet** out) {
    *out = nullptr;
    if (c->k1_selector != PSA_K1_AUTO || !c->opt_planes) return PSA_OK;
    const int      slot = v.slot;
    const int32_t* h_idx = v.h_idx;
    const int64_t  n_g = v.n_g;
    DataSlot&      s = c->slot[slot];
    drop_stale_planes(c);
    const bool     all = h_idx == nullptr, displaced = mean_host != nullptr;
    const uint64_t h = (all ? 0 : hash_idx(h_idx, n_g)) ^ (displaced ? 0x9E3779B97F4A7C15ull : 0);
    const size_t   n_mean = (size_t)s.N * 3;
    for (auto& ps : c->planes)
        if (ps->slot == slot && ps->all_atoms == all && ps->n_g == n_g && ps->displaced == displaced &&
            (all || (ps->idx_hash == h && std::memcmp(ps->idx.data(), h_idx, (size_t)n_g * sizeof(int32_t)) == 0)) &&
            (!displaced || (ps->mean.size() == n_mean && std::memcmp(ps->mean.data(), mean_host, n_mean * sizeof(float)) == 0))) {
            ps->last_use = ++c->plane_tick;
            *out = ps.get();
            return PSA_OK;
        }
    if (K_local < c->opt_planes_min_k) return PSA_OK;
    if (!all && !c->opt_planes_eager) {
        auto& seen = c->seen_groups;
        if (std::find(seen.begin(), seen.end(), h) == seen.end()) {
            seen.push_back(h);
            if (seen.size() > 256) seen.erase(seen.begin());
            return PSA_OK;
        }
    }
    unsigned bits = 0;
    if (displaced) {
        PSA_TRY(displaced_absmax(c, slot, mean_host, h_idx, n_g, &bits));
    } else if (all) {
        PSA_TRY(slot_absmax(c, slot));
        bits = s.absmax_bits;
    } else {
        PSA_TRY(group_absmax(c, slot, h_idx, n_g, &bits));
    }
    const float vscale = k1_f16_vscale(bits);
    if (!(vscale > 0.f)) return PSA_OK;
    const int     A_pad = k1_pair_atom_pad(n_g);
    const int64_t n_fg = (s.T + 15) / 16;
    const size_t  bytes = plane_bytes(n_fg, A_pad / K1_BA);
    size_t        free_b = 0, total_b = 0;
    PSA_HIP_CHECK(hipMemGetInfo(&free_b, &total_b));
    const size_t budget = c->opt_planes_budget > 0 ? (size_t)c->opt_planes_budget : (size_t)(0.45 * (double)total_b);
    if (bytes > budget) return PSA_OK;
    while (planes_bytes_held(c) + bytes > budget)
        if (!evict_one_plane_set(c)) return PSA_OK;
    const size_t reserve = (size_t)2 << 30;
    while (free_b < bytes + reserve) {
        if (!evict_one_plane_set(c)) return PSA_OK;
        PSA_HIP_CHECK(hipMemGetInfo(&free_b, &total_b));
    }
    auto ps = std::make_unique<PlaneSet>();
    if (c->scratch_byte >= 0) ps->buf.fill = &c->scratch_byte;
    if (ps->buf.reserve(bytes) != PSA_OK) {
        (void)hipGetLastError();
        return PSA_OK;
    }
    {
        HostTimer ht(&c->oneoff_ms[2]);
        PSA_HIP_CHECK(hipStreamSynchronize(c->stream));
        PSA_TRY(launch_split_planes(c, s.buf.as<float>(), displaced ? c->d_mean_all.as<float>() : nullptr, v.d_idx, ps->buf.ptr,
                                    s.T, s.N, (int)n_g, A_pad, vscale));
        PSA_HIP_CHECK(hipStreamSynchronize(c->stream));
    }
    ps->slot = slot;
    ps->generation = s.generation;
    ps->all_atoms = all;
    if (!all) ps->idx.assign(h_idx, h_idx + n_g);
    ps->idx_hash = h;
    ps->displaced = displaced;
    if (displaced) ps->mean.assign(mean_host, mean_host + n_mean);
    ps->T = s.T;
    ps->n_fg = n_fg;
    ps->n_g = (int)n_g;
    ps->A_pad = A_pad;
    ps->vscale = vscale;
    ps->last_use = ++c->plane_tick;
    *out = ps.get();
    c->planes.push_back(std::move(ps));
    return PSA_OK;
}

int check_weights(psa_ctx* c, int64_t N) {
    PSA_REQUIRE(c->weights_N == 0 || c->weights_N == N, "atom weights were set for %lld atoms, the trajectory has %lld",
                (long long)c->weights_N, (long long)N);
    return PSA_OK;
}

void set_geom_weights(const psa_ctx* c, ProjGeom* g) {
    g->weights = c->weights_N ? c->d_weights.as<float>() : nullptr;
    g->wscale = c->weights_N ? c->weights_scale : 1.f;
}

int make_geom(psa_ctx* c, const GroupView& v, int64_t K_local, GeomRule rule, ProjGeom* g) {
    const int     slot = v.slot;
    const int64_t n_g = v.n_g;
    set_geom_weights(c, g);
    g->T = c->slot[slot].T;
    g->q_stride = g->T;
    g->N_tot = c->slot[slot].N;
    PSA_REQUIRE(n_g < (1ll << 30) && K_local < (1ll << 29), "group or k-list too large");
    g->n_g = (int)n_g;
    g->A_pad = (int)((n_g + 31) / 32 * 32);
    g->K = (int)K_local;
    g->split = K1Family::f32;
    const bool autosel = c->k1_selector == PSA_K1_AUTO;
    if (v.ps && rule == GeomRule::product) {
        g->split = K1Family::f16_planes;
        g->vscale = v.ps->vscale;
        g->m_blk = k1_planes_block_rows((int)K_local, c->opt_k1_wide != 0);
        g->A_pad = v.ps->A_pad;
        g->M_pad = (int)((2 * K_local + g->m_blk - 1) / g->m_blk * g->m_blk);
        return PSA_OK;
    }
    if (rule == GeomRule::product && autosel && k1_pair_eligible(v.d_idx, g->N_tot, n_g, K_local, v.disp)) {
        unsigned bits = 0;
        if (v.h_idx) {
            PSA_TRY(group_absmax(c, slot, v.h_idx, n_g, &bits));
        } else {
            PSA_TRY(slot_absmax(c, slot));
            bits = c->slot[slot].absmax_bits;
        }
        g->vscale = k1_f16_vscale(bits);
        if (g->vscale > 0.f) g->split = K1Family::f16_fly;
    }
    if (g->split == K1Family::f32 && rule != GeomRule::f32_only && (autosel || c->k1_selector == PSA_K1_SPLIT_BF16) &&
        k1_split_eligible(v.d_idx, g->N_tot, n_g, v.disp))
        g->split = K1Family::bf16;
    if (g->split == K1Family::f16_fly) {
        g->m_blk = k1_pair_block_rows((int)K_local);
        g->A_pad = k1_pair_atom_pad(n_g);
    } else {
        g->m_blk = g->split == K1Family::bf16 ? k1_split_block_rows((int)K_local) : k1_mfma_block_rows((int)K_local);
    }
    g->M_pad = (int)((2 * K_local + g->m_blk - 1) / g->m_blk * g->m_blk);
    return PSA_OK;
}

int prepare_phase(psa_ctx* c, const GroupView& v, const ProjGeom& g, int64_t k_first) {
    const int*   d_idx = v.d_idx;
    const float* d_kvec = c->d_kvec.as<float>() + 3 * k_first;
    const bool   f16 = g.split == K1Family::f16_fly || g.split == K1Family::f16_planes, bf16 = g.split == K1Family::bf16;
    if (g.lowrank) {
        PSA_TRY(c->d_lr_diff.reserve(pd16_table_bytes(g.M_pad_d, g.A_pad)));
        PSA_TRY(c->d_phase.reserve(pf16_table_bytes(128, g.A_pad)));
        StageTimer    st(c, PSA_T_PHASE);
        const double* f64 = c->d_lr_f64.as<double>();
        return launch_lowrank_tables(c, d_kvec, f64 + 7 + LOWRANK_NODES, f64, f64 + 7, c->d_mean_all.as<float>(), d_idx,
                                     c->d_lr_diff.ptr, c->d_phase.ptr, g, g.M_pad_d, g.dscale, g.lr_pair);
    }
    PSA_TRY(c->d_phase.reserve(f16    ? pf16_table_bytes(g.M_pad, g.A_pad)
                               : bf16 ? pb_table_bytes(g.M_pad, g.A_pad)
                                      : p_table_floats(g.M_pad, g.A_pad) * sizeof(float)));
    StageTimer st(c, PSA_T_PHASE);
    if (f16)
        PSA_TRY(launch_phase_table_f16(c, d_kvec, c->d_mean_all.as<float>(), d_idx, c->d_phase.ptr, g));
    else if (bf16)
        PSA_TRY(launch_phase_table_split(c, d_kvec, c->d_mean_all.as<float>(), d_idx, c->d_phase.ptr, g));
    else
        PSA_TRY(launch_phase_table(c, d_kvec, c->d_mean_all.as<float>(), d_idx, c->d_phase.as<float>(), g));
    if (v.disp) {
        PSA_TRY(c->d_mean_g.reserve((size_t)g.A_pad * 3 * sizeof(float)));
        PSA_TRY(launch_gather_mean(c, c->d_mean_all.as<float>(), d_idx, c->d_mean_g.as<float>(), g));
    }
    return PSA_OK;
}

static int launch_projection_once(psa_ctx* c, const GroupView& v, ProjGeom g, float2* d_q, int64_t q_stride, int64_t t_begin,
                                  int64_t t_count);

int launch_projection(psa_ctx* c, const GroupView& v, ProjGeom g, float2* d_q, int64_t q_stride, int64_t t_begin,
                      int64_t t_count) {
    static const int reps = [] {
        const char* e = std::getenv("PSA_DEBUG_REPEAT_K1");
        return e ? std::max(1, std::atoi(e)) : 1;
    }();
    for (int r = 0; r < reps; ++r) PSA_TRY(launch_projection_once(c, v, g, d_q, q_stride, t_begin, t_count));
    return PSA_OK;
}

static int launch_projection_once(psa_ctx* c, const GroupView& v, ProjGeom g, float2* d_q, int64_t q_stride, int64_t t_begin,
                                  int64_t t_count) {
    const DataSlot& s = c->slot[v.slot];
    const PlaneSet* ps = v.ps;
    PSA_REQUIRE(t_begin >= 0 && t_count > 0 && t_begin + t_count <= s.T && q_stride >= t_begin + t_count,
                "frame range [%lld,%lld) outside the slot", (long long)t_begin, (long long)(t_begin + t_count));
    g.T = t_count;
    g.q_stride = q_stride;
    StageTimer   st(c, PSA_T_PROJECT);
    const float* d_v = s.buf.as<float>() + (size_t)t_begin * 3 * (size_t)s.N;
    d_q += t_begin;
    if (g.split == K1Family::f16_planes) {
        PSA_REQUIRE(ps != nullptr && t_begin % 16 == 0, "planes are cut in groups of 16 frames");
        const int64_t fg0 = t_begin / 16, n_fg = ps->n_fg - fg0;
        const _Float16* pl = ps->buf.as<_Float16>() + (size_t)fg0 * (size_t)(ps->A_pad / K1_BA) * PL_STAGE_ELEMS;
        if (g.lowrank) {
            ProjGeom gn = g;
            gn.K = LOWRANK_NODES;
            gn.m_blk = gn.M_pad = 2 * LOWRANK_NODES;
            gn.q_stride = t_count;
            PSA_REQUIRE(c->d_lr_qn.cap >= (size_t)LOWRANK_NODES * 3 * t_count * sizeof(float2), "node projections not reserved");
            if (g.lr_pair) {
                PSA_TRY(launch_k1_lowrank_pair(c, pl, c->d_phase.ptr, c->d_lr_diff.ptr, c->d_lr_qn.as<float2>(), d_q, g, n_fg, g.dscale));
                ++c->lowrank_pair_launches;
            } else {
                PSA_TRY(launch_k1_planes_lw(c, pl, c->d_phase.ptr, c->d_lr_qn.as<float2>(), gn, n_fg));
                ProjGeom gd = g;
                gd.M_pad = g.M_pad_d;
                PSA_TRY(launch_k1_planes_diff(c, pl, c->d_lr_diff.ptr, d_q, gd, n_fg, g.dscale));
            }
            PSA_TRY(launch_lowrank_combine_r(c, c->d_lr_qn.as<float2>(), c->d_lr_L.as<float>(), c->d_lr_phi.as<float2>(), d_q, g,
                                             t_count));
            ++c->lowrank_launches;
            return PSA_OK;
        }
        if (g.m_blk == 256) return launch_k1_planes_wide(c, pl, c->d_phase.ptr, d_q, g, n_fg);
        if (g.m_blk == 128 && c->opt_k1_loader_waves) return launch_k1_planes_lw(c, pl, c->d_phase.ptr, d_q, g, n_fg);
        return launch_k1_planes(c, pl, c->d_phase.ptr, d_q, g, n_fg);
    }
    if (g.split == K1Family::f16_fly) return launch_k1_pair(c, d_v, c->d_phase.ptr, v.d_idx, d_q, g);
    if (g.split == K1Family::bf16) return launch_k1_split(c, d_v, c->d_phase.ptr, v.d_idx, d_q, g);
    if (c->k1_selector == PSA_K1_WAVE)
        return launch_k1_wave(c, d_v, c->d_phase.as<float>(), v.d_idx, c->d_mean_g.as<float>(), d_q, g, v.disp);
    return launch_k1_mfma(c, d_v, c->d_phase.as<float>(), v.d_idx, c->d_mean_g.as<float>(), d_q, g, v.disp);
}

int prepare_block(psa_ctx* c, const GroupView& v, GeomRule rule, const ProjectArgs* lowrank, int64_t k_first, int64_t nk,
                  ProjGeom* g) {
    PSA_TRY(make_geom(c, v, nk, rule, g));
    if (lowrank) PSA_TRY(prepare_lowrank(c, v, *lowrank, k_first, nk, g));
    return prepare_phase(c, v, *g, k_first);
}

int project_block(psa_ctx* c, const GroupView& v, const ProjectArgs* lowrank, int64_t k_first, int64_t nk, float2* d_q) {
    const int64_t T = c->slot[v.slot].T;
    ProjGeom      g;
    PSA_TRY(prepare_block(c, v, GeomRule::product, lowrank, k_first, nk, &g));
    return launch_projection(c, v, g, d_q, T, 0, T);
}

int group_source(psa_ctx* c, GroupView* v, const float* mean_host, int64_t K) {
    PSA_TRY(get_planes(c, *v, K, v->disp ? mean_host : nullptr, &v->ps));
    if (v->ps) {
        v->disp = false;
        return PSA_OK;
    }
    return materialise_displacements(c, v, mean_host);
}

int check_group_indices(const GroupView& v, int64_t N) {
    for (int64_t i = 0; v.h_idx && i < v.n_g; ++i)
        PSA_REQUIRE(v.h_idx[i] >= 0 && v.h_idx[i] < N, "Atom indices in basis out of bounds.");
    return PSA_OK;
}

int upload_single_group(psa_ctx* c, GroupView* v, int64_t N, const float* k_vectors, int64_t K, const float* mean_pos_all) {
    if (v->n_g == 0) return PSA_OK;
    PSA_TRY(upload(c, c->d_kvec, k_vectors, (size_t)K * 3 * sizeof(float)));
    PSA_TRY(upload(c, c->d_mean_all, mean_pos_all, (size_t)N * 3 * sizeof(float)));
    if (v->h_idx) PSA_TRY(upload(c, c->d_idx, v->h_idx, (size_t)v->n_g * sizeof(int32_t)));
    v->d_idx = v->h_idx ? c->d_idx.as<int>() : nullptr;
    return PSA_OK;
}

int check_project_args(psa_ctx* c, const ProjectArgs& a, int64_t N) {
    PSA_REQUIRE(a.mean_pos_all != nullptr, "null mean_pos_all");
    PSA_REQUIRE(a.K_local >= 0 && a.K_total >= 1 && a.k_offset >= 0 && a.k_offset + a.K_local <= a.K_total,
                "k range [%lld,%lld) outside [0,%lld)", (long long)a.k_offset, (long long)(a.k_offset + a.K_local),
                (long long)a.K_total);
    PSA_REQUIRE(a.K_local == 0 || a.k_vectors != nullptr, "null k_vectors");
    PSA_TRY(validate_groups(N, a.group_idx, a.group_off, a.G));
    PSA_REQUIRE((a.flags & PSA_F_INTENSITY) || a.G == 1, "complex output needs exactly one atom group (got %d)", a.G);
    (void)c;
    return PSA_OK;
}

int begin_result(psa_ctx* c, int64_t T, int64_t K_total, int64_t k_offset, bool intensity, char** rows) {
    PSA_TRY(c->d_slab.reserve(row_bytes(T, intensity) * (size_t)K_total));
    c->res_T = T;
    c->res_K = K_total;
    c->res_intensity = intensity;
    c->slab_valid = true;
    c->out_valid = false;
    c->inten_valid = false;
    c->kmap.clear();
    c->out_K = K_total;
    c->plane_call_mark = c->plane_tick + 1;
    *rows = (char*)c->d_slab.ptr + row_bytes(T, intensity) * (size_t)k_offset;
    return PSA_OK;
}

int upload_project_inputs(psa_ctx* c, const ProjectArgs& a, int64_t N) {
    StageTimer st(c, PSA_T_H2D);
    PSA_TRY(upload(c, c->d_kvec, a.k_vectors, (size_t)a.K_local * 3 * sizeof(float)));
    PSA_TRY(upload(c, c->d_mean_all, a.mean_pos_all, (size_t)N * 3 * sizeof(float)));
    if (a.group_idx) PSA_TRY(upload(c, c->d_idx, a.group_idx, (size_t)a.group_off[a.G] * sizeof(int32_t)));
    return PSA_OK;
}

int check_segments(psa_ctx* c, int64_t T, int32_t flags) {
    if (c->seg_L == 0) return PSA_OK;
    PSA_REQUIRE(flags & PSA_F_INTENSITY, "segment-averaged spectra are intensities: PSA_F_INTENSITY is required while segments are set");
    PSA_REQUIRE(c->seg_L <= T, "segment length %lld exceeds the trajectory's %lld frames", (long long)c->seg_L, (long long)T);
    return PSA_OK;
}

static int64_t result_frames(const psa_ctx* c, int64_t T) { return c->seg_L ? c->seg_L : T; }

static void segment_blocks(const psa_ctx* c, int64_t T, int64_t K_local, int64_t* nk, int64_t* ns) {
    const int64_t n_seg = 1 + (T - c->seg_L) / c->seg_hop;
    const int64_t units = std::max<int64_t>(1, K_local * T / c->seg_L);
    if (units >= n_seg) {
        *ns = n_seg;
        *nk = std::max<int64_t>(1, std::min(K_local, units / n_seg));
    } else {
        *ns = units;
        *nk = 1;
    }
}

static int segment_stage(psa_ctx* c, const float2* d_q, int64_t T, int64_t K_local, float* rows, bool first) {
    const int64_t L = c->seg_L, H = c->seg_hop, n_seg = 1 + (T - L) / H;
    int64_t       nk = 0, ns = 0;
    segment_blocks(c, T, K_local, &nk, &ns);
    const float inv_norm = (float)(1.0 / ((double)n_seg * c->seg_U));
    PSA_TRY(c->d_seg.reserve((size_t)nk * 3 * (size_t)ns * (size_t)L * sizeof(float2)));
    float2* d_seg = c->d_seg.as<float2>();
    for (int64_t k0 = 0; k0 < K_local; k0 += nk) {
        const int64_t bk = std::min(nk, K_local - k0);
        for (int64_t s0 = 0; s0 < n_seg; s0 += ns) {
            const int64_t bs = std::min(ns, n_seg - s0);
            {
                StageTimer st(c, PSA_T_EPILOGUE);
                PSA_TRY(launch_segment_window(c, d_q + (size_t)k0 * 3 * (size_t)T, c->d_seg_window.as<float>(), d_seg, T, L, H, s0,
                                              bs, bk));
            }
            {
                StageTimer st(c, PSA_T_FFT);
                PSA_TRY(run_fft(c, d_seg, L, 3 * bk * bs));
            }
            StageTimer st(c, PSA_T_EPILOGUE);
            PSA_TRY(launch_segment_power(c, d_seg, rows + (size_t)k0 * (size_t)L, L, bs, bk, inv_norm, first && s0 == 0));
        }
    }
    return PSA_OK;
}

static int spectrum_stage(psa_ctx* c, float2* d_q, int64_t T, int64_t K_local, bool intensity, float* rows, bool first) {
    if (c->seg_L) return segment_stage(c, d_q, T, K_local, rows, first);
    {
        StageTimer st(c, PSA_T_FFT);
        PSA_TRY(run_fft(c, d_q, T, 3 * K_local));
    }
    if (intensity) {
        StageTimer st(c, PSA_T_EPILOGUE);
        PSA_TRY(launch_intensity_accumulate(c, d_q, rows, T, K_local, first));
    }
    return PSA_OK;
}
// ... 492 lines not shown
```

### psa_amd/csrc/k1_planes_diff.hip

```cpp
#include <utility>

#include "k1_f16.h"
#include "k1_lowrank_pair.h"

namespace psa {

namespace {
constexpr int D_M_BLK = 512, D_T_BLK = 64, D_MT = 16, D_PERIOD = 40;
constexpr int D_STAGE_UNITS = 44, D_RING_UNITS = 160, D_EARLY = D_RING_UNITS - 3 * D_STAGE_UNITS;
constexpr int D_STAGE_BYTES = D_M_BLK * K1_BA * 2;
static_assert(D_EARLY == 28 && D_RING_UNITS % 4 == 0 && D_STAGE_UNITS % 4 == 0, "ring arithmetic");
constexpr auto d_unit_off = unit_off<D_STAGE_UNITS, D_RING_UNITS, D_PERIOD>;
}

__host__ __device__ inline size_t pd16_index(int m, int a, int n_stage) {
    const int row = m % D_M_BLK, rt = row >> 4, v = 2 * (rt & 15) + (rt >> 4), r = row & 15, al = a % K1_BA;
    return (((size_t)(m / D_M_BLK) * n_stage + a / K1_BA) * 32 + v) * (16 * K1_BA) + (size_t)r * K1_BA +
           (size_t)((((al >> 3) ^ pl_swizzle(r)) << 3) + (al & 7));
}
size_t pd16_table_bytes(int M_pad, int A_pad) { return ((size_t)M_pad * A_pad + 4 * (size_t)D_M_BLK * K1_BA) * 2; }

template <bool NT_V>
__global__ void __launch_bounds__(512, 2)
k1_planes_diff_kernel(const _Float16* __restrict__ planes, const _Float16* __restrict__ Db, float2* __restrict__ Q, int64_t T,
                      int64_t q_stride, int n_fg, int n_stage, int K, int n_mblk, int n_tblk, float qscale) {
    using PR = F16x2;
    using E8 = PR::v8;
    __shared__ __attribute__((aligned(16))) unsigned char smem[D_RING_UNITS * 1024];
    const unsigned lds0 = (unsigned)(size_t)(lds_u8*)smem;

    int mb, tb;
    if (!k1_block_map(n_mblk, n_tblk, mb, tb)) return;

    const int tid = threadIdx.x, lane = tid & 63;
    const int w = __builtin_amdgcn_readfirstlane(tid >> 6);
    const int wh = w >> 2, wf = w & 3;
    const int r16 = lane & 15, q = lane >> 4;

    const unsigned char* src[11];
    {
        int fg = tb * 4 + (w & 3);
        if (fg >= n_fg) fg = n_fg - 1;
        const unsigned char* pl0 = reinterpret_cast<const unsigned char*>(planes) + (size_t)fg * n_stage * PL_STAGE_BYTES;
#pragma unroll
        for (int i = 0; i < 3; ++i) src[i] = pl0 + 1024 * (2 * i);
        const unsigned char* d0 = reinterpret_cast<const unsigned char*>(Db) + (size_t)mb * n_stage * D_STAGE_BYTES;
#pragma unroll
        for (int i = 3; i < 11; ++i) src[i] = d0 + 1024 * ((w & 3) + 4 * (i - 3));
    }
    const unsigned dma_voff = 16 * lane;
    const unsigned wbase = lds0 + 1024 * (w & 3);
    using std::integral_constant;
    auto dma = [&](auto s40_c, auto i_c) __attribute__((always_inline)) {
        constexpr int      S40 = decltype(s40_c)::value, I = decltype(i_c)::value;
        constexpr unsigned OFF = d_unit_off(S40, 4 * I);
        if constexpr (I < 3) {
            lds_dma16_at<OFF, NT_V>(src[I], dma_voff, wbase);
            src[I] += PL_STAGE_BYTES;
        } else {
            lds_dma16_at<OFF, false>(src[I], dma_voff, wbase);
            src[I] += D_STAGE_BYTES;
        }
    };
    auto dma_range = [&]<int S40, int... Is>(integral_constant<int, S40>, std::integer_sequence<int, Is...>) __attribute__((always_inline)) {
        (dma(integral_constant<int, S40>{}, integral_constant<int, Is>{}), ...);
    };
    auto dma_late = [&](auto s40_c) __attribute__((always_inline)) {
        dma_range(s40_c, std::integer_sequence<int, 7, 8, 9, 10>{});
    };
    auto dma_early = [&](auto s40_c) __attribute__((always_inline)) {
        dma_range(s40_c, std::make_integer_sequence<int, 7>{});
    };

    const unsigned lane_off = lds0 + r16 * (K1_BA * 2) + ((q ^ pl_swizzle(r16)) << 4);
    unsigned       lane_a[3], lane_b[3];
    unit_ring_windows(lane_off + 1024 * wh, lane_off + 1024 * wf, lane_a, lane_b);
    E8    a[4];
    E8    bf[3];
    f32x4 acc[D_MT][3];
    auto  read_a = [&](auto s40_c, auto mt_c) __attribute__((always_inline)) {
        constexpr int S40 = decltype(s40_c)::value, MTI = decltype(mt_c)::value;
        a[MTI & 3] = lds_frag(lane_a, d_unit_off(S40, 12 + 2 * MTI));
    };
    auto read_b = [&](auto s40_c, auto c_c) __attribute__((always_inline)) {
        constexpr int S40 = decltype(s40_c)::value, CC = decltype(c_c)::value;
        bf[CC] = lds_frag(lane_b, d_unit_off(S40, 4 * CC));
    };
#pragma unroll
    for (int mt = 0; mt < D_MT; ++mt)
#pragma unroll
        for (int c = 0; c < 3; ++c) acc[mt][c] = f32x4{0.f, 0.f, 0.f, 0.f};

    using I0 = integral_constant<int, 0>;
    using I1 = integral_constant<int, 1>;
    using I2 = integral_constant<int, 2>;
    if (wh == 0) {
        dma_early(I0{});
        dma_late(I0{});
        dma_early(I1{});
        dma_late(I1{});
        dma_early(I2{});
    }
    asm volatile("s_waitcnt vmcnt(7)\n\ts_barrier" ::: "memory");
    read_b(I0{}, I0{});
    read_b(I0{}, I1{});
    read_b(I0{}, I2{});
    read_a(I0{}, I0{});
    read_a(I0{}, I1{});

    int  left = n_stage;
    auto stage = [&](auto s40_c) __attribute__((always_inline)) {
        constexpr int S40 = decltype(s40_c)::value;
        if (left <= S40) return;
        using SN = integral_constant<int, (S40 + 1) % D_PERIOD>;
        using SNN = integral_constant<int, (S40 + 2) % D_PERIOD>;
        using S3 = integral_constant<int, (S40 + 3) % D_PERIOD>;
        if (wh == 0) {
            dma_late(SNN{});
            dma_early(S3{});
        }
        auto tile = [&](auto mt_c) __attribute__((always_inline)) {
            constexpr int MTI = decltype(mt_c)::value;
            if constexpr (MTI + 2 < D_MT)
                read_a(s40_c, integral_constant<int, MTI + 2>{});
            else
                read_a(SN{}, integral_constant<int, MTI + 2 - D_MT>{});
            auto comp = [&](auto c_c) __attribute__((always_inline)) {
                constexpr int CC = decltype(c_c)::value;
                acc[MTI][CC] = PR::mma(a[MTI & 3], bf[CC], acc[MTI][CC]);
                if constexpr (MTI == D_MT - 1) read_b(SN{}, c_c);
            };
            comp(I0{});
            comp(I1{});
            comp(I2{});
            __builtin_amdgcn_sched_barrier(0);
        };
        [&]<int... Ms>(std::integer_sequence<int, Ms...>) __attribute__((always_inline)) { (tile(integral_constant<int, Ms>{}), ...); }(
            std::make_integer_sequence<int, D_MT>{});
        asm volatile("s_waitcnt vmcnt(7)\n\ts_barrier" ::: "memory");
    };
    for (; left > 0; left -= D_PERIOD)
        [&]<int... Ss>(std::integer_sequence<int, Ss...>) __attribute__((always_inline)) { (stage(integral_constant<int, Ss>{}), ...); }(
            std::make_integer_sequence<int, D_PERIOD>{});
    asm volatile("s_waitcnt vmcnt(0)" ::: "memory");

    const int lane_e = __builtin_amdgcn_mbcnt_hi(~0u, __builtin_amdgcn_mbcnt_lo(~0u, 0u));
    const int r16_e = lane_e & 15, q_e = lane_e >> 4;
    k1_store_q(Q, acc, wh * (D_M_BLK / 2) + mb * D_M_BLK, q_e, (int64_t)tb * D_T_BLK + wf * 16 + r16_e, T, K, q_stride, qscale);
}

int launch_k1_planes_diff(psa_ctx* c, const void* d_planes, const void* d_diff, float2* d_q, const ProjGeom& g, int64_t n_fg, float dscale) {
    PSA_REQUIRE(g.M_pad % D_M_BLK == 0 && g.M_pad >= 2 * g.K && g.M_pad > 0, "D pass: 512-row M blocks only");
    PSA_REQUIRE(dscale > 0.f, "planes do not cover the launch");
    return launch_planes_family(c, k1_planes_diff_kernel<true>, k1_planes_diff_kernel<false>, D_M_BLK, 512, "D pass", K1_BA, dscale,
                                d_planes, d_diff, d_q, g, n_fg);
}

template <bool PAIR>
__global__ void __launch_bounds__(256)
diff_table_kernel(const float* __restrict__ kvec, const double* __restrict__ kline, const float* __restrict__ mean_all,
                  const int* __restrict__ idx, const float* __restrict__ w, float wnorm, _Float16* __restrict__ Db, int K,
                  int n_g, int A_pad, float dscale) {
    const int a = blockIdx.y * 256 + threadIdx.x;
    const int k = blockIdx.x;
    if (a >= A_pad) return;
    float d[2] = {0.f, 0.f};
    if (k < K && a < n_g) {
        const int   src = idx ? idx[a] : a;
        const float rx = mean_all[3 * (size_t)src + 0], ry = mean_all[3 * (size_t)src + 1], rz = mean_all[3 * (size_t)src + 2];
        const float kx = kvec[3 * k + 0], ky = kvec[3 * k + 1], kz = kvec[3 * k + 2];
        const float arg = __fmaf_rn(kz, rz, __fmaf_rn(ky, ry, __fmul_rn(kx, rx)));
        float       cs[2];
        sincosf(arg, &cs[1], &cs[0]);
        const double th = kline[3 * k + 0] * (double)rx + kline[3 * k + 1] * (double)ry + kline[3 * k + 2] * (double)rz;
        double       se, ce;
        sincos(th, &se, &ce);
        const double wa = w ? (double)(w[src] * wnorm) : 1.0;
        d[0] = (float)(((double)cs[0] - ce) * (double)dscale * wa);
        d[1] = (float)(((double)cs[1] - se) * (double)dscale * wa);
    }
    const int n_stage = A_pad / K1_BA;
    Db[PAIR ? pd16_pair_index(2 * k, a, n_stage) : pd16_index(2 * k, a, n_stage)] = (_Float16)d[0];
    Db[PAIR ? pd16_pair_index(2 * k + 1, a, n_stage) : pd16_index(2 * k + 1, a, n_stage)] = (_Float16)d[1];
}

__global__ void __launch_bounds__(256)
node_table_kernel(const double* __restrict__ geo, const double* __restrict__ kappa, const float* __restrict__ mean_all,
                  const int* __restrict__ idx, const float* __restrict__ w, float wnorm, _Float16* __restrict__ Pb, int n_g,
                  int A_pad) {
    const int a = blockIdx.y * 256 + threadIdx.x;
    const int l = blockIdx.x;
    if (a >= A_pad) return;
    double cs[2] = {0.0, 0.0};
    if (a < n_g) {
        const int    src = idx ? idx[a] : a;
        const double rx = mean_all[3 * (size_t)src + 0], ry = mean_all[3 * (size_t)src + 1], rz = mean_all[3 * (size_t)src + 2];
        const double th = (geo[0] * rx + geo[1] * ry + geo[2] * rz) + kappa[l] * ((geo[3] * rx + geo[4] * ry + geo[5] * rz) - geo[6]);
        sincos(th, &cs[1], &cs[0]);
        if (w) {
            const double wa = (double)(w[src] * wnorm);
            cs[0] *= wa;
            cs[1] *= wa;
        }
    }
    const int n_stage = A_pad / K1_BA;
#pragma unroll
    for (int ri = 0; ri < 2; ++ri) {
        const double   x = cs[ri] * (double)F16x2::P_SCALE;
        const _Float16 lead = (_Float16)(float)x;
        Pb[pf16_tile_index(0, 2 * l + ri, a, 128, n_stage)] = lead;
        Pb[pf16_tile_index(1, 2 * l + ri, a, 128, n_stage)] = (_Float16)(float)(x - (double)lead);
    }
}

int launch_lowrank_tables(psa_ctx* c, const float* d_kvec, const double* d_kline, const double* d_geo, const double* d_kappa,
                          const float* d_mean_all, const int* d_idx, void* d_diff, void* d_nodes, const ProjGeom& g, int M_pad_d,
                          float dscale, bool pair) {
    PSA_REQUIRE(M_pad_d % D_M_BLK == 0 && M_pad_d >= 2 * g.K && g.A_pad % K1_BA == 0, "bad low-rank table geometry");
    PSA_REQUIRE(!pair || M_pad_d == LRP_ROWS, "the pair launch's image is one 512-row block");
    hipLaunchKernelGGL(pair ? diff_table_kernel<true> : diff_table_kernel<false>, dim3(M_pad_d / 2, (g.A_pad + 255) / 256), dim3(256), 0,
                       c->stream, d_kvec, d_kline, d_mean_all, d_idx, g.weights, 1.f / g.wscale, (_Float16*)d_diff, g.K, g.n_g, g.A_pad,
                       dscale);
    PSA_HIP_CHECK(hipGetLastError());
    if (pair) {
        const size_t n_stage = (size_t)g.A_pad / K1_BA, a_pad = LRP_PAD_STAGES * LRP_A_UNITS * 1024, b_pad = LRP_PAD_STAGES * LRP_B_UNITS * 1024;
        static_assert(LRP_ROWS == D_M_BLK, "the pair image has the size of one D block");
        PSA_HIP_CHECK(hipMemsetAsync((char*)d_diff + n_stage * LRP_A_UNITS * 1024, 0, a_pad, c->stream));
        PSA_HIP_CHECK(hipMemsetAsync((char*)d_diff + pd16_pair_table_bytes((int)n_stage) - b_pad, 0, b_pad, c->stream));
    } else {
        PSA_HIP_CHECK(hipMemsetAsync((char*)d_diff + (size_t)M_pad_d * g.A_pad * 2, 0,
                                     pd16_table_bytes(M_pad_d, g.A_pad) - (size_t)M_pad_d * g.A_pad * 2, c->stream));
    }
    hipLaunchKernelGGL(node_table_kernel, dim3(LOWRANK_NODES, (g.A_pad + 255) / 256), dim3(256), 0, c->stream, d_geo, d_kappa, d_mean_all,
                       d_idx, g.weights, 1.f / g.wscale, (_Float16*)d_nodes, g.n_g, g.A_pad);
    PSA_HIP_CHECK(hipGetLastError());
    return PSA_OK;
}

}
```

### psa_amd/csrc/k1_planes_lw.hip

```cpp
#include "k1_f16.h"

namespace psa {

template <bool NT_V>
__global__ void __launch_bounds__(768, 3)
k1_planes_lw_kernel(const _Float16* __restrict__ planes, const _Float16* __restrict__ Pb, float2* __restrict__ Q,
                    int64_t T, int64_t q_stride, int n_fg, int n_stage, int K, int n_mblk, int n_tblk, float qscale) {
    using PR = F16x2;
    using E8 = PR::v8;
    constexpr int NP = PR::NP, MT16 = 4, M_BLK = 128, T_BLK = 64, FOLD = 8, RING = 4;
    constexpr int P_STAGE_BYTES = pf16_stage_bytes(M_BLK);
    constexpr int V_GROUP_BYTES = PL_STAGE_BYTES;
    constexpr int STAGE_BYTES = P_STAGE_BYTES + 4 * V_GROUP_BYTES;
    constexpr int BATCH = 10;
    static_assert(RING * STAGE_BYTES == 160 * 1024, "the ring is all of LDS");
    __shared__ __attribute__((aligned(16))) unsigned char smem[RING * STAGE_BYTES];
    const unsigned lds0 = (unsigned)(size_t)(lds_u8*)smem;

    int mb, tb;
    if (!k1_block_map(n_mblk, n_tblk, mb, tb)) return;

    const int tid = threadIdx.x, lane = tid & 63;
    const int w = __builtin_amdgcn_readfirstlane(tid >> 6);

    if (w >= 8) {
        const int j = w - 8;
        int       fg = tb * 4 + j;
        if (fg >= n_fg) fg = n_fg - 1;
        const unsigned char* p_next = reinterpret_cast<const unsigned char*>(Pb) + (size_t)mb * n_stage * P_STAGE_BYTES;
        const unsigned char* v_next = reinterpret_cast<const unsigned char*>(planes) + (size_t)fg * n_stage * V_GROUP_BYTES;
        const unsigned       p_voff = 4096 * j + 16 * lane, v_voff = 16 * lane;
        auto dma_stage = [&](int slot) {
            const unsigned dst = lds0 + slot * STAGE_BYTES;
            lds_dma16_group<4>(p_next, p_voff, dst + 4096 * j);
            lds_dma16_group<3, NT_V>(v_next, v_voff, dst + P_STAGE_BYTES + j * V_GROUP_BYTES);
            lds_dma16_group<3, NT_V>(v_next, v_voff + 3072, dst + P_STAGE_BYTES + j * V_GROUP_BYTES + 3072);
            p_next += P_STAGE_BYTES;
            v_next += V_GROUP_BYTES;
        };
        __builtin_amdgcn_s_setprio(2);
        dma_stage(0);
        dma_stage(1);
        dma_stage(2);
        asm volatile("s_waitcnt vmcnt(%0)\n\ts_barrier" ::"n"(2 * BATCH) : "memory");
        asm volatile("s_waitcnt vmcnt(%0)\n\ts_barrier" ::"n"(1 * BATCH) : "memory");
        int slot = 3;
        for (int s = 0; s < n_stage; ++s) {
            dma_stage(slot);
            slot = slot == RING - 1 ? 0 : slot + 1;
            asm volatile("s_waitcnt vmcnt(%0)\n\ts_barrier" ::"n"(BATCH) : "memory");
        }
        asm volatile("s_waitcnt vmcnt(0)" ::: "memory");
        return;
    }

    const int     wh = w >> 2, wf = w & 3;
    const int     r16 = lane & 15, q = lane >> 4;
    const int64_t t0 = (int64_t)tb * T_BLK + wf * 16;
    const int      gsw = pl_swizzle(r16);
    const unsigned p_lane = lds0 + (wh * (M_BLK / 2) + r16) * (K1_BA * 2) + ((q ^ gsw) << 4);
    const unsigned v_lane = lds0 + P_STAGE_BYTES + wf * V_GROUP_BYTES + r16 * (K1_BA * 2) + ((q ^ gsw) << 4);
    E8    a[NP][MT16];
    E8    bb[2][NP];
    f32x4 hi[MT16][3], lo[MT16][3];
    auto  read_a_tile = [&](int mt, int slot) {
        const unsigned base = p_lane + slot * STAGE_BYTES;
#pragma unroll
        for (int p = 0; p < NP; ++p)
            a[p][mt] = *reinterpret_cast<lds_cv8*>((const lds_u8*)(size_t)(base + (p * M_BLK + mt * 16) * 64));
    };
    auto read_b = [&](int buf, int slot, int c) {
#pragma unroll
        for (int p = 0; p < NP; ++p)
            bb[buf][p] = *reinterpret_cast<lds_cv8*>((const lds_u8*)(size_t)(v_lane + slot * STAGE_BYTES + (c * NP + p) * 1024));
    };
#pragma unroll
    for (int mt = 0; mt < MT16; ++mt)
#pragma unroll
        for (int c = 0; c < 3; ++c) {
            hi[mt][c] = f32x4{0.f, 0.f, 0.f, 0.f};
            lo[mt][c] = f32x4{0.f, 0.f, 0.f, 0.f};
        }

    asm volatile("s_barrier" ::: "memory");
    read_b(0, 0, 0);
#pragma unroll
    for (int mt = 0; mt < MT16; ++mt) read_a_tile(mt, 0);
    asm volatile("s_waitcnt lgkmcnt(0)\n\ts_barrier" ::: "memory");

    auto stage = [&](auto par_c, auto restart_c, int, int slot) {
        constexpr int  par = decltype(par_c)::value;
        constexpr bool restart = decltype(restart_c)::value;
        const int      slot1 = slot == RING - 1 ? 0 : slot + 1;
#pragma unroll
        for (int c = 0; c < 3; ++c) {
            const int cur = (par + c) & 1;
            if (c < 2)
                read_b(cur ^ 1, slot, c + 1);
            else
                read_b(cur ^ 1, slot1, 0);
#pragma unroll
            for (int mt = 0; mt < MT16; ++mt) {
                f32x4 ch = PR::mma(a[1][mt], bb[cur][0], restart ? f32x4{0.f, 0.f, 0.f, 0.f} : hi[mt][c]);
                ch = PR::mma(a[0][mt], bb[cur][1], ch);
                hi[mt][c] = PR::mma(a[0][mt], bb[cur][0], ch);
                if (c == 2) read_a_tile(mt, slot1);
            }
        }
        asm volatile("s_barrier" ::: "memory");
    };
    k1_chain_loop<RING, FOLD>(n_stage, lo, hi, stage);

    k1_store_q(Q, lo, wh * (M_BLK / 2) + mb * M_BLK, q, t0 + r16, T, K, q_stride, qscale);
}

int launch_k1_planes_lw(psa_ctx* c, const void* d_planes, const void* d_phase, float2* d_q, const ProjGeom& g, int64_t n_fg) {
    PSA_REQUIRE(g.m_blk == 128 && g.M_pad % 128 == 0, "loader-wave planes kernel: 128-row M blocks only");
    return launch_planes_family(c, k1_planes_lw_kernel<true>, k1_planes_lw_kernel<false>, 128, 768, "planes kernel", 2 * K1_BA,
                                F16x2::P_SCALE, d_planes, d_phase, d_q, g, n_fg);
}

}
```

### psa_amd/csrc/psa_ctx.h

```cpp
#pragma once
#include <hip/hip_runtime.h>
#include <rocfft/rocfft.h>
#include <rccl/rccl.h>

#include <cstdarg>
#include <cstdint>
#include <cstdio>
#include <map>
#include <memory>
#include <mutex>
#include <string>
#include <thread>
#include <utility>
#include <vector>

#include "psa_hip.h"

namespace psa {

void set_error(const char* fmt, ...);

#define PSA_HIP_CHECK(expr)                                                              \
    do {                                                                                 \
        hipError_t e_ = (expr);                                                          \
        if (e_ != hipSuccess) {                                                          \
            psa::set_error("%s:%d: %s -> %s", __FILE__, __LINE__, #expr,                 \
                           hipGetErrorString(e_));                                       \
            return PSA_EHIP;                                                             \
        }                                                                                \
    } while (0)

#define PSA_FFT_CHECK(expr)                                                              \
    do {                                                                                 \
        rocfft_status s_ = (expr);                                                       \
        if (s_ != rocfft_status_success) {                                               \
            psa::set_error("%s:%d: %s -> rocfft_status %d", __FILE__, __LINE__, #expr,   \
                           (int)s_);                                                     \
            return PSA_EFFT;                                                             \
        }                                                                                \
    } while (0)

#define PSA_NCCL_CHECK(expr)                                                             \
    do {                                                                                 \
        ncclResult_t r_ = (expr);                                                        \
        if (r_ != ncclSuccess) {                                                         \
            psa::set_error("%s:%d: %s -> %s", __FILE__, __LINE__, #expr,                 \
                           ncclGetErrorString(r_));                                      \
            return PSA_ERCCL;                                                            \
        }                                                                                \
    } while (0)

#define PSA_REQUIRE(cond, ...)                                                           \
    do {                                                                                 \
        if (!(cond)) {                                                                   \
            psa::set_error(__VA_ARGS__);                                                 \
            return PSA_EINVAL;                                                           \
        }                                                                                \
    } while (0)

#define PSA_TRY(expr)                                                                    \
    do {                                                                                 \
        int rc_ = (expr);                                                                \
        if (rc_ != PSA_OK) return rc_;                                                   \
    } while (0)

struct DevBuf {
    void*  ptr = nullptr;
    size_t cap = 0;
    const int* fill = nullptr;
    DevBuf() = default;
    DevBuf(DevBuf&& o) noexcept : ptr(std::exchange(o.ptr, nullptr)), cap(std::exchange(o.cap, 0)) {}
    DevBuf& operator=(DevBuf&& o) noexcept {
        if (this != &o) {
            release();
            ptr = std::exchange(o.ptr, nullptr);
            cap = std::exchange(o.cap, 0);
        }
        return *this;
    }
    ~DevBuf() { release(); }
    int reserve(size_t bytes);
    void release();
    template <class T> T* as() const { return static_cast<T*>(ptr); }
};

struct FftPlan {
    rocfft_plan           plan = nullptr;
    rocfft_execution_info info = nullptr;
    size_t                work_bytes = 0;
    FftPlan() = default;
    FftPlan(FftPlan&& o) noexcept
        : plan(std::exchange(o.plan, nullptr)), info(std::exchange(o.info, nullptr)), work_bytes(std::exchange(o.work_bytes, 0)) {}
    FftPlan& operator=(FftPlan&& o) noexcept {
        std::swap(plan, o.plan);
        std::swap(info, o.info);
        std::swap(work_bytes, o.work_bytes);
        return *this;
    }
    ~FftPlan();
};

struct DataSlot {
    DevBuf  buf;
    int64_t T = 0, N = 0;
    bool    valid = false;
    uint64_t generation = 0;
    bool     absmax_known = false;
    unsigned absmax_bits = 0;
    bool                  blocks_known = false;
    std::vector<unsigned> block_absmax;
};

struct Timed {
    int        stage;
    hipEvent_t e0, e1;
};
struct TimingState {
    std::vector<hipEvent_t> pool;
    std::vector<Timed>      pending;
    double                  acc[8] = {};
    int64_t                 k1_launches = 0;
    double                  k1_ms = 0.0;
};

constexpr int K1_BA   = 32;
constexpr int LOWRANK_NODES = 64;
constexpr int K1_VROW = 96;
constexpr int K1_PROW = 36;

__host__ __device__ inline size_t p_tile_index(int m, int a, int m_blk, int n_stage) {
    return ((size_t)(m / m_blk) * n_stage + (a / K1_BA)) * ((size_t)m_blk * K1_PROW) +
           (size_t)(m % m_blk) * K1_PROW + (a % K1_BA);
}
inline size_t p_table_floats(int M_pad, int A_pad) { return (size_t)M_pad * (A_pad / K1_BA) * K1_PROW; }

enum class K1Family : int {
    f32 = 0,
    f16_fly = 2,
    bf16 = 3,
    f16_planes = 4,
};

struct ProjGeom {
    int64_t T = 0;
    int64_t q_stride = 0;
    int64_t N_tot = 0;
    int     n_g = 0;
    int     A_pad = 0;
    int     K = 0;
    int     M_pad = 0;
    int     m_blk = 0;
    K1Family split = K1Family::f32;
    float   vscale = 0.f;
    bool    lowrank = false;
    int     M_pad_d = 0;
    float   dscale = 0.f;
    bool    lr_pair = false;
    const float* weights = nullptr;
    float        wscale = 1.f;
};

struct PlaneSet {
    DevBuf               buf;
    int                  slot = 0;
    uint64_t             generation = 0;
    bool                 all_atoms = true;
    std::vector<int32_t> idx;
    uint64_t             idx_hash = 0;
    bool                 displaced = false;
    std::vector<float>   mean;
    int64_t              T = 0, n_fg = 0;
    int                  n_g = 0, A_pad = 0;
    float                vscale = 0.f;
    uint64_t             last_use = 0;
};

constexpr int KMAP_MIRROR = (int)0x80000000u;

struct Stager {
    void*       pin[2] = {nullptr, nullptr};
    size_t      cap = 0;
    hipEvent_t  freed[2] = {nullptr, nullptr};
    hipStream_t copy_stream = nullptr;
};

}

enum { PSA_T_H2D = 0, PSA_T_PHASE, PSA_T_PROJECT, PSA_T_FFT, PSA_T_EPILOGUE, PSA_T_GATHER,
       PSA_T_TRANSPOSE, PSA_T_D2H, PSA_T_COUNT };

struct psa_ctx {
    psa_ctx();
    ~psa_ctx();
    psa_ctx(const psa_ctx&) = delete;
    psa_ctx& operator=(const psa_ctx&) = delete;

    int         device = 0;
    hipStream_t stream = nullptr;
    std::mutex  mu;
    int         k1_selector = PSA_K1_AUTO;
    int         compute_units = 0;

    psa::DataSlot slot[PSA_NUM_SLOTS + 1];
    std::vector<float> disp_mean;
    uint64_t           disp_source = 0;
    std::vector<unsigned> disp_block_absmax;
    std::vector<float>    disp_abs_mean;
    uint64_t              disp_abs_source = ~0ull;

    psa::DevBuf d_kvec, d_mean_all, d_idx, d_mean_g, d_phase, d_qwork, d_fft_work, d_tables, d_absmax;
    psa::DevBuf d_upload_max;
    psa::DevBuf d_zeros;
    psa::DevBuf d_qrows, d_stage, d_bin;

    std::vector<std::unique_ptr<psa::PlaneSet>> planes;
    std::vector<uint64_t> seen_groups;
    uint64_t plane_tick = 0, plane_call_mark = 0;
    int64_t  opt_planes, opt_planes_budget, opt_planes_eager, opt_planes_min_k;
    psa::Stager stager;
    hipStream_t d2h_stream = nullptr;
    hipEvent_t  d2h_ready = nullptr;

    int64_t fs_T_total = 0, fs_T_local = 0, fs_K_total = 0, fs_rows_k0 = 0, fs_rows_nk = 0;
    bool    fs_intensity = false;
    psa::DevBuf d_slab;
    psa::DevBuf d_out;
    psa::DevBuf d_aux;
    int64_t res_T = 0, res_K = 0;
    bool    res_intensity = false;
    int64_t              out_K = 0;
    std::vector<int32_t> kmap;
    psa::DevBuf          d_kmap, d_cols;
    int64_t              opt_fold_pairs;
    psa::DevBuf          d_inten;
    bool                 inten_valid = false;
    bool    slab_valid = false, out_valid = false;

    std::map<std::pair<int64_t, int64_t>, psa::FftPlan> plans;
    std::thread  fft_primer;
    psa::FftPlan primed;
    int64_t      primed_T = 0;
    int64_t      opt_fft_prime;
    int64_t      opt_k1_wide;
    int64_t      opt_k1_loader_waves;
    int64_t      opt_k1_lowrank;
    int64_t      opt_k1_lowrank_min_k;
    int64_t      opt_k1_lowrank_min_local;
    int64_t      lowrank_launches = 0;
    int64_t      opt_k1_lowrank_pair;
    int64_t      lowrank_pair_launches = 0;
    psa::DevBuf  d_lr_diff, d_lr_qn, d_lr_L, d_lr_phi, d_lr_f64;

    psa::DevBuf  d_weights;
    int64_t      weights_N = 0;
    float        weights_scale = 1.f;

    psa::DevBuf  d_seg_window, d_seg;
    int64_t      seg_L = 0, seg_hop = 0;
    double       seg_U = 0.0;
    bool         seg_boxcar = false;

    psa::DevBuf  d_vdos_work, d_vdos_pairs, d_vdos_off, d_vdos_mean, d_vdos_part, d_vdos_acc, d_vdos_out;
    int64_t      opt_vdos_work_bytes;

    psa::DevBuf  d_modes_work, d_modes_coef, d_modes_out;
    int64_t      opt_modes_work_bytes;

    psa::DevBuf  d_cov_slab, d_cov_g, d_cov_out;

    psa::DevBuf  d_peaks_spec, d_peaks_bands, d_peaks_part, d_peaks_fit, d_peaks_info;

    psa::DevBuf  d_rc_work, d_rc_kappa, d_rc_khat, d_rc_idx, d_rc_tiles, d_rc_ent, d_rc_slot, d_rc_dest, d_rc_bins, d_rc_scale,
                 d_rc_acc, d_rc_out, d_rc_groups, d_rc_part;
    int64_t      opt_dynamic_work_bytes;

    psa::DevBuf  d_corr_tab, d_corr_factor, d_corr_scale, d_corr_in, d_corr_out;

    psa::DevBuf  d_rs_idx, d_rs_items, d_rs_part, d_rs_acc;

    psa::DevBuf  d_msd_u, d_msd_img, d_msd_sums, d_msd_offs, d_msd_sizes, d_msd_lags, d_msd_out;

    psa::DevBuf  d_pair_c;

    psa::DevBuf  d_angle_work, d_angle_edges;

    psa::TimingState timing;
    double oneoff_ms[4] = {0, 0, 0, 0};
    psa::DevBuf      d_sync;

    int scratch_byte = -1;

    ncclComm_t comm = nullptr;
    int        rank = 0, nranks = 1;
};

namespace psa {

int launch_phase_table(psa_ctx* c, const float* d_kvec, const float* d_mean_all, const int* d_idx,
                       float* d_phase, const ProjGeom& g);
int launch_gather_mean(psa_ctx* c, const float* d_mean_all, const int* d_idx, float* d_mean_g,
                       const ProjGeom& g);
int launch_fill_synthetic(psa_ctx* c, float* d_v, int64_t T, int64_t N, uint64_t seed, int64_t t_offset, int n_modes,
                          const float* d_amp, const int* d_comp, const float* d_ct,
                          const float* d_st, const float* d_ca, const float* d_sa);
int launch_mean_over_frames(psa_ctx* c, const float* d_x, int64_t T, int64_t N, float* d_mean);
int launch_subtract_mean(psa_ctx* c, const float* d_x, const float* d_mean, float* d_out, int64_t T, int64_t N);
int launch_absmax_bits(psa_ctx* c, const float* d_x, int64_t n, unsigned* d_out, bool reset = true);
int launch_absmax_blocks(psa_ctx* c, const float* d_x, const float* d_mean, int64_t T, int64_t N, unsigned* d_out);

int  k1_mfma_block_rows(int K);
int  launch_k1_mfma(psa_ctx* c, const float* d_v, const float* d_phase, const int* d_idx,
                    const float* d_mean_g, float2* d_q, const ProjGeom& g, bool displacements);
int  launch_k1_wave(psa_ctx* c, const float* d_v, const float* d_phase, const int* d_idx,
                    const float* d_mean_g, float2* d_q, const ProjGeom& g, bool displacements);

bool   k1_split_eligible(const int* d_idx, int64_t N_tot, int64_t n_g, bool displacements);
int    k1_split_block_rows(int K);
size_t pb_table_bytes(int M_pad, int A_pad);
int    launch_phase_table_split(psa_ctx* c, const float* d_kvec, const float* d_mean_all, const int* d_idx,
                                void* d_phase, const ProjGeom& g);
int    launch_k1_split(psa_ctx* c, const float* d_v, const void* d_phase, const int* d_idx, float2* d_q,
                       const ProjGeom& g);

bool   k1_pair_eligible(const int* d_idx, int64_t N_tot, int64_t n_g, int64_t K, bool displacements);
int    k1_pair_atom_pad(int64_t n_g);
int    k1_pair_block_rows(int K);
float  k1_f16_vscale(unsigned absmax_bits);
size_t pf16_table_bytes(int M_pad, int A_pad);
int    launch_phase_table_f16(psa_ctx* c, const float* d_kvec, const float* d_mean_all, const int* d_idx,
                              void* d_phase, const ProjGeom& g);
int    launch_k1_pair(psa_ctx* c, const float* d_v, const void* d_phase, const int* d_idx, float2* d_q,
                      const ProjGeom& g);

int    k1_planes_block_rows(int K, bool wide);
int    launch_split_planes(psa_ctx* c, const float* d_x, const float* d_mean, const int* d_idx, void* d_planes, int64_t T,
                           int64_t N_tot, int n_g, int A_pad, float vscale);
int    launch_k1_planes(psa_ctx* c, const void* d_planes, const void* d_phase, float2* d_q, const ProjGeom& g,
                        int64_t n_fg);
int    launch_k1_planes_lw(psa_ctx* c, const void* d_planes, const void* d_phase, float2* d_q, const ProjGeom& g,
                           int64_t n_fg);

int    launch_k1_planes_wide(psa_ctx* c, const void* d_planes, const void* d_phase, float2* d_q, const ProjGeom& g,
                             int64_t n_fg);

size_t pd16_table_bytes(int M_pad, int A_pad);
int    launch_lowrank_tables(psa_ctx* c, const float* d_kvec, const double* d_kline, const double* d_geo, const double* d_kappa,
                             const float* d_mean_all, const int* d_idx, void* d_diff, void* d_nodes, const ProjGeom& g, int M_pad_d,
                             float dscale, bool pair);
int    launch_k1_planes_diff(psa_ctx* c, const void* d_planes, const void* d_diff, float2* d_q, const ProjGeom& g, int64_t n_fg,
                             float dscale);

int    launch_k1_lowrank_pair(psa_ctx* c, const void* d_planes, const void* d_nodes, const void* d_diff, float2* d_qn, float2* d_q,
                              const ProjGeom& g, int64_t n_fg, float dscale);

int    launch_lowrank_combine_r(psa_ctx* c, const float2* d_qn, const float* d_L, const float2* d_phi, float2* d_q, const ProjGeom& g,
                                int64_t qn_stride);

int launch_dft_bin(psa_ctx* c, const float2* d_q, int64_t T, int64_t bin, float2* d_out3);
int launch_scale_transpose_c64(psa_ctx* c, const float2* d_slab, float2* d_out, float* d_inten, int64_t T, int64_t n,
                               int64_t K_pitch, int64_t col_first, int64_t src_first, const int32_t* d_cols,
                               const int32_t* d_srcs);
int launch_intensity_accumulate(psa_ctx* c, const float2* d_q, float* d_slab_rows, int64_t T,
                                int64_t K_local, bool first_group);
int launch_transpose_f32(psa_ctx* c, const float* d_slab, float* d_out, int64_t T, int64_t K, const int32_t* d_srcs);
int launch_segment_window(psa_ctx* c, const float2* d_q, const float* d_w, float2* d_seg, int64_t T, int64_t L, int64_t H,
                          int64_t s0, int64_t ns, int64_t nk);
int launch_segment_window_rows(psa_ctx* c, const float2* d_q, const float* d_w, float2* d_seg, int64_t T, int64_t L, int64_t H,
                               int64_t s0, int64_t ns, int64_t n_series);
int launch_segment_power(psa_ctx* c, const float2* d_seg, float* d_rows, int64_t L, int64_t ns, int64_t nk, float inv_norm,
                         bool first);
constexpr int VDOS_TILE_PAIRS = 32;
int launch_vdos_gather(psa_ctx* c, const float* d_data, const float* d_mean, const float* d_weights, const float* d_win,
                       const int* d_pair_atoms, float2* d_work, int64_t T, int64_t N, int64_t L, int64_t H, int64_t s0,
                       int64_t ns, int64_t n_pairs);
int launch_vdos_power(psa_ctx* c, const float2* d_work, const int64_t* d_pair_off, double* d_part, double* d_acc, int64_t L,
                      int64_t ns, int64_t n_pairs, int64_t p0, int64_t g_first, int64_t n_groups, int64_t n_chunks);
int launch_vdos_finish(psa_ctx* c, const double* d_acc, float* d_out, int64_t L, int64_t rows, double scale);
int modes_tile(int64_t M);
int launch_mode_power(psa_ctx* c, const float2* d_S, const float2* d_coef, float* d_out, int64_t L, int64_t ns, int64_t nk,
                      int64_t B, int64_t M, int MT, int64_t K_pitch, int64_t k_col0, float scale, bool first);
int64_t covariance_chunks(int64_t T);
int64_t covariance_slab_floats(int64_t T, int64_t n, int n_w);
int launch_covariance(psa_ctx* c, const float2* d_S, const float* d_g, float* d_slab, double2* d_out, int64_t T, int64_t nk, int64_t B,
                      int n_w, int64_t K_pitch, int64_t k_col0, double scale);
int peaks_slices(int64_t C, int64_t rows);
int launch_peak_find(psa_ctx* c, const float* d_spec, int64_t C, const int32_t* d_bands, int lo, int hi, int row0, int row_end,
                     int n_slices, float* d_pmax, int* d_pidx, int* d_pflag);
int launch_peak_fit(psa_ctx* c, const float* d_spec, int64_t C, const int32_t* d_bands, int lo, int hi, const float* d_pmax,
                    const int* d_pidx, const int* d_pflag, int n_slices, double df, float window_hwhm, int half_window_bins,
                    int max_iter, float* d_fit, int32_t* d_info);
constexpr int DYN_THREADS = 256;
constexpr int DYN_ATOMS = 512;
constexpr int DYN_CHAIN = 128;
constexpr int DYN_FRAMES = 4;
int dynamic_slices(int64_t K);
int launch_dynamic_project(psa_ctx* c, const float* d_pos, const float* d_vel, const float* d_weights, const int* d_idx,
                           const float* d_kappa, float2* d_q, int64_t T, int64_t N, int64_t n_g, int64_t nk, bool currents,
                           int slices);
int launch_dynamic_power(psa_ctx* c, const float2* d_seg, const float* d_khat, float* d_out, int64_t L, int64_t ns, int64_t nk,
                         bool currents, int64_t K_pitch, int64_t k_col0, float scale, bool first);
int launch_dynamic_sincos(psa_ctx* c, const float* d_turns, float2* d_out, int64_t n);
constexpr int LAT_THREADS = 256;
constexpr int LAT_KS = 512;
constexpr int LAT_ATOMS = 128;
constexpr int LAT_TABLE = 3584;
constexpr int LAT_CHAIN = 128;
constexpr int LAT_FRAMES = 4;
constexpr int LAT_MAX_INDEX = 64;
constexpr int LAT_MAX_ENTRIES = 3 * (2 * LAT_MAX_INDEX + 1);
int launch_lattice_project(psa_ctx* c, const float* d_pos, const float* d_vel, const float* d_weights, const int* d_idx,
                           const float* box_hi, const float* box_lo, const int* d_tile_off, const unsigned short* d_ent,
                           const unsigned* d_slot, const int* d_dest, float2* d_q, int64_t T, int64_t N, int64_t n_g, int64_t tile0,
                           int64_t n_tiles, bool currents);
int launch_lattice_shell(psa_ctx* c, const float2* d_seg, const float* d_khat, const int* d_bin_start, double* d_acc, int64_t L,
                         int64_t ns, int64_t g0, int64_t nb, int64_t n_bins, bool currents);
int launch_lattice_finish(psa_ctx* c, const double* d_acc, const double* d_scale, float* d_out, int64_t n, int64_t n_bins);
constexpr int PARTIAL_MAX_SPECIES = 8;
constexpr int PARTIAL_MAX_PAIRS = PARTIAL_MAX_SPECIES * (PARTIAL_MAX_SPECIES + 1) / 2;
int launch_partial_power(psa_ctx* c, const float2* d_seg, const float* d_khat, float* d_out, int64_t L, int64_t ns, int64_t nk,
                         int n_species, bool currents, int64_t K_pitch, int64_t k_col0, float scale, bool first);
int launch_partial_shell(psa_ctx* c, const float2* d_seg, const float* d_khat, const int* d_bin_start, double* d_acc, int64_t L,
                         int64_t ns, int64_t g0, int64_t nb, int64_t n_bins, int n_species, bool currents);
constexpr int SELF_THREADS = 256;
constexpr int SELF_ATOMS = 4;
constexpr int SELF_FRAMES = 64;
constexpr int SELF_ENTRIES = 24;
constexpr int SELF_KS = 64;
int launch_self_series(psa_ctx* c, const float* d_pos, const float* d_weights, const int* d_idx, int64_t a0, const float* box_hi,
                       const float* box_lo, const int* d_tile, const unsigned short* d_ent, const unsigned* d_slot, const float* d_win,
                       float2* d_work, int64_t T, int64_t N, int64_t na, int64_t tile0, int64_t n_tiles, int64_t v0, int64_t nv,
                       int64_t L, int64_t H, int64_t s0, int64_t ns, int64_t pitch);
int launch_self_power(psa_ctx* c, const float2* d_work, const int* d_groups, double* d_part, double* d_acc, int64_t L, int64_t ns,
                      int64_t na, int64_t v0, int64_t nv, int64_t g_first, int64_t ng, int64_t cols, int64_t n_chunks, bool mirror);
constexpr int CORR_LAGS = 8;
constexpr int CORR_COLS_MIN = 64;
int launch_correlation_pad(psa_ctx* c, const float2* d_q, float2* d_seg, int64_t T, int64_t L, int64_t P, int64_t H, int64_t s0,
                           int64_t ns, int64_t n_rows);
int launch_correlation_transform(psa_ctx* c, const double* d_X, const double* d_tab, const double* d_factor, const double* d_scale,
                                 float* d_out, int64_t fields, int64_t P, int64_t cols, int64_t n_lags);
int launch_correlation_transform(psa_ctx* c, const float* d_X, const double* d_tab, const double* d_factor, const double* d_scale,
                                 float* d_out, int64_t fields, int64_t P, int64_t cols, int64_t n_lags);
constexpr int MSD_LAGS = 256;
constexpr int MSD_ORIGINS = 1024;
constexpr int MSD_WINDOW = 1280;
constexpr int MSD_MAX_GROUPS = 8;
constexpr int MSD_MAX_BINS = 1024;
constexpr int MSD_MAX_VH_LAGS = 64;
constexpr int MSD_UNWRAP_FRAMES = 64;
constexpr int MSD_UNWRAP_ATOMS = 16;
int msd_origins(int64_t step);
int launch_msd_unwrap(psa_ctx* c, const float* d_pos, const int* d_idx, int64_t a0, int64_t na, const double* box,
                      const double* box_inverse, bool unwrap, int* d_sums, int* d_offs, double* d_u, int* d_img, int64_t T, int64_t N);
int launch_msd_moments(psa_ctx* c, const double* d_u, const void* d_chunks, int64_t n_chunks, double* d_part, int64_t T, int64_t n_lags,
                       int64_t step, int64_t n_os);
int launch_msd_moments_reduce(psa_ctx* c, const double* d_part, const int32_t* group_first, double* d_acc, int64_t n_lags, int64_t n_os,
                              int32_t G);
int launch_msd_moments_finish(psa_ctx* c, const double* d_acc, const int64_t* d_group_size, double* d_out, int64_t T, int64_t n_lags,
                              int32_t G, int64_t step);
int launch_msd_hist(psa_ctx* c, const double* d_u, const void* d_chunks, int64_t n_chunks, const int64_t* d_lags, int64_t n_vh,
                    unsigned* d_part, int64_t T, int64_t step, int64_t n_os, float inv_dr, int32_t n_r);
constexpr int HIST_REDUCE_MAX_ROWS = 64;
struct HistRows {
    int lo[HIST_REDUCE_MAX_ROWS], hi[HIST_REDUCE_MAX_ROWS], factor[HIST_REDUCE_MAX_ROWS];
};
int launch_hist_reduce(psa_ctx* c, const unsigned* d_part, const HistRows& rows, int32_t n, int64_t n_outer, int64_t cols,
                       unsigned long long* d_acc);
constexpr int PAIR_TILE = 256;
constexpr int PAIR_MAX_BINS = 1024;
constexpr int PAIR_MAX_LAGS = 64;
constexpr int PAIR_MAX_SPECIES = 8;
struct PairItem {
    int a_lo, a_n, b_lo, b_hi, slab, n_os, diag, pair;
};
int launch_pair_frac(psa_ctx* c, const float* d_pos, const int* d_idx, int64_t n_a, const double* box_inverse, float* d_out, int64_t f0,
                     int64_t df, int64_t n_frames, int64_t T, int64_t N);
int launch_pair_hist(psa_ctx* c, const float* d_cA, const float* d_cB, const void* d_items, int64_t n_items, unsigned* d_part,
                     const double* box, int64_t n_a, int64_t n_ob, float inv_dr, int32_t n_r);
constexpr int ANGLE_MAX_NEIGHBOURS = 64;
constexpr int ANGLE_MAX_BINS = 1024;
constexpr int ANGLE_HIST_WORDS = 12288;
constexpr int ANGLE_CENTRES = 256;
constexpr int ANGLE_SPECIES_SHIFT = 28;
struct AngleSpecies {
    int   S, start[PAIR_MAX_SPECIES + 1], tile_first[PAIR_MAX_SPECIES + 1];
    float inv_rc[PAIR_MAX_SPECIES * PAIR_MAX_SPECIES];
};
struct AngleItem {
    int a_lo, a_n, species, slab, n_os;
};
inline int64_t angle_row_words(int S, int n_theta) {
    return (int64_t)(S * (S + 1) / 2) * (n_theta + 1) + (int64_t)S * (ANGLE_MAX_NEIGHBOURS + 1) + 1;
}
int launch_angle_neighbours(psa_ctx* c, const float* d_c, int* d_count, void* d_list, const AngleSpecies& sp, const double* box,
                            int64_t n_a, int64_t n_ob);
int launch_angle_hist(psa_ctx* c, const int* d_count, const void* d_list, const void* d_items, int64_t n_items, const float* d_edges,
                      unsigned* d_part, int32_t S, int64_t n_a, int64_t n_ob, int32_t n_theta);
constexpr int ORDER_MAX_L = 12;
constexpr int ORDER_MAX_LS = 8;
constexpr int ORDER_MAX_BINS = 1024;
constexpr int ORDER_SHIFT = 24;
struct OrderLs {
    int n_l, l_max;
    unsigned mask;
};
inline int64_t order_row_words(int n_l, int n_q) { return (int64_t)n_l * n_q + 3; }
// ... 7 lines not shown
```

Measured before the change: 54910 billion.

## Fold low-rank node error into diff table and split node projection into single f16 plane

Adds a folded low-rank path, on by default. It folds the low-rank node-combination term into the f16 difference table, using a new scale that covers the combined bound. The node projection then needs only one f16 phase plane (two MFMAs instead of three), both in a new fused pair kernel and in a variant of the loader-wave planes kernel. This removes MFMA work and table traffic on the node projections. In exchange it adds extra table-build work and accepts lower precision on the node term, absorbed into the diff residual.

```diff
diff --git a/include/psa_hip.h b/include/psa_hip.h
--- a/include/psa_hip.h
+++ b/include/psa_hip.h
@@ -40,6 +40,7 @@
 int         psa_destroy(psa_ctx* ctx);
 int         psa_synchronize(psa_ctx* ctx);
 int         psa_set_k1(psa_ctx* ctx, int selector);
+int         psa_set_k1_lowrank_fold(psa_ctx* ctx, int on);
 #define PSA_OPT_PLANES         0
 #define PSA_OPT_PLANES_BUDGET  1
 #define PSA_OPT_PLANES_EAGER   2
@@ -210,6 +211,7 @@
 int psa_k1_lowrank_launches(psa_ctx* ctx, int64_t* launches);
 int psa_k1_lowrank_pair_launches(psa_ctx* ctx, int64_t* launches);
 int psa_lowrank_pair_image(int32_t n_stage, int64_t* index, int64_t* bytes);
+int psa_lowrank_fold_image(int32_t n_stage, int64_t* index, int64_t* bytes);
 int psa_debug_device_buffers(int64_t* count, int64_t* bytes);
 #define PSA_SCRATCH_REAL 0
 #define PSA_SCRATCH_INDEX 1
diff --git a/psa_amd/_hip.py b/psa_amd/_hip.py
--- a/psa_amd/_hip.py
+++ b/psa_amd/_hip.py
@@ -88,6 +88,7 @@
     "psa_destroy": (C.c_int, [_ctx]),
     "psa_synchronize": (C.c_int, [_ctx]),
     "psa_set_k1": (C.c_int, [_ctx, C.c_int]),
+    "psa_set_k1_lowrank_fold": (C.c_int, [_ctx, C.c_int]),
     "psa_set_option": (C.c_int, [_ctx, C.c_int, C.c_int64]),
     "psa_device_info": (C.c_int, [_ctx, C.c_char_p, C.c_int, C.POINTER(C.c_int), _i64p]),
     "psa_data_upload": (C.c_int, [_ctx, C.c_int, _f32p, C.c_int64, C.c_int64]),
@@ -180,6 +181,7 @@
     "psa_k1_lowrank_launches": (C.c_int, [_ctx, _i64p]),
     "psa_k1_lowrank_pair_launches": (C.c_int, [_ctx, _i64p]),
     "psa_lowrank_pair_image": (C.c_int, [C.c_int32, _i64p, _i64p]),
+    "psa_lowrank_fold_image": (C.c_int, [C.c_int32, _i64p, _i64p]),
     "psa_oneoff_stats": (C.c_int, [_ctx, _f64p]),
     "psa_option_info": (C.c_int, [C.c_int, C.POINTER(C.c_int32), _i64p, C.POINTER(C.c_char_p)]),
     "psa_debug_device_buffers": (C.c_int, [_i64p, _i64p]),
@@ -312,7 +314,7 @@
     K, N = kv.shape[0], mean.shape[0]
     ix = None if idx is None else np.ascontiguousarray(idx, np.int32)
     n_g = N if ix is None else ix.size
-    ok, geo = C.c_int32(0), np.zeros(12, np.float64)
+    ok, geo = C.c_int32(0), np.zeros(14, np.float64)
     kappa, cm = np.zeros(64, np.float64), np.zeros((K, 64), np.complex64)
     lw, phi = np.zeros((K, 64), np.float32), np.zeros(K, np.complex64)
     _check(load_library().psa_lowrank_plan(_f32(kv), K, _f32(mean), N, None if ix is None else ix.ctypes.data_as(_i32p), n_g,
@@ -321,12 +323,19 @@
     if not ok.value:
         return None
     return {"u": geo[0:3].copy(), "k0": geo[3:6].copy(), "x_c": geo[6], "h_x": geo[7], "width": geo[8],
-            "interval": int(geo[9]), "d_bound": geo[10], "dscale": geo[11], "kappa": kappa, "C": cm, "L": lw, "phi": phi}
+            "interval": int(geo[9]), "d_bound": geo[10], "dscale": geo[11], "e_bound": geo[12],
+            "dscale_fold": geo[13], "kappa": kappa, "C": cm, "L": lw, "phi": phi}
 
 
 def lowrank_pair_image(n_stage: int):
     index, nbytes = np.zeros((512, 32 * int(n_stage)), np.int64), C.c_int64(0)
     _check(load_library().psa_lowrank_pair_image(int(n_stage), index.ctypes.data_as(_i64p), C.byref(nbytes)), "psa_lowrank_pair_image")
+    return index, nbytes.value
+
+
+def lowrank_fold_image(n_stage: int):
+    index, nbytes = np.zeros((512, 32 * int(n_stage)), np.int64), C.c_int64(0)
+    _check(load_library().psa_lowrank_fold_image(int(n_stage), index.ctypes.data_as(_i64p), C.byref(nbytes)), "psa_lowrank_fold_image")
     return index, nbytes.value
 
 
@@ -475,6 +484,9 @@
     def set_k1(self, selector: int):
         _check(self._lib.psa_set_k1(self._h, selector), "psa_set_k1")
 
+    def set_lowrank_fold(self, on: bool):
+        _check(self._lib.psa_set_k1_lowrank_fold(self._h, int(bool(on))), "psa_set_k1_lowrank_fold")
+
     def device_info(self) -> dict:
         name = C.create_string_buffer(256)
         cu, mem = C.c_int(0), C.c_int64(0)
@@ -564,6 +576,7 @@
     def reset_options(self):
         for option, _, default in option_table():
             self.set_option(option, default)
+        self.set_lowrank_fold(True)
 
     def scratch_fill(self, byte: int):
         n, b = C.c_int64(0), C.c_int64(0)
diff --git a/psa_amd/csrc/api_core.hip b/psa_amd/csrc/api_core.hip
--- a/psa_amd/csrc/api_core.hip
+++ b/psa_amd/csrc/api_core.hip
@@ -404,6 +404,13 @@
     return PSA_OK;
 }
 
+int psa_set_k1_lowrank_fold(psa_ctx* c, int on) {
+    PSA_TRY(enter(c));
+    Guard g(c);
+    c->k1_lowrank_fold = on != 0;
+    return PSA_OK;
+}
+
 int psa_set_option(psa_ctx* c, int option, int64_t value) {
     PSA_TRY(enter(c));
     Guard g(c);
diff --git a/psa_amd/csrc/api_internal.h b/psa_amd/csrc/api_internal.h
--- a/psa_amd/csrc/api_internal.h
+++ b/psa_amd/csrc/api_internal.h
@@ -127,6 +127,8 @@
     double              kappa[LOWRANK_NODES] = {};
     double              d_bound = 0;
     float               dscale = 0.f;
+    double              e_bound = 0;
+    float               dscale_fold = 0.f;
     std::vector<double> kline;
     std::vector<float>  L;
     std::vector<float>  phi;
diff --git a/psa_amd/csrc/api_lowrank.hip b/psa_amd/csrc/api_lowrank.hip
--- a/psa_amd/csrc/api_lowrank.hip
+++ b/psa_amd/csrc/api_lowrank.hip
@@ -1,4 +1,5 @@
 #include "api_internal.h"
+#include "k1_lowrank_fold.h"
 #include "k1_lowrank_pair.h"
 
 namespace psa {
@@ -154,6 +155,13 @@
         }
     }
     p->dscale = std::ldexp(1.0f, 14 - (int)std::ceil(std::log2(p->d_bound)));
+    for (int64_t j = 0; j < K; ++j) {
+        double lam = 0.0;
+        for (int l = 0; l < LOWRANK_NODES; ++l) lam += std::fabs((double)p->L[(size_t)j * LOWRANK_NODES + l]);
+        const double rot = std::fabs((double)p->phi[(size_t)j * 2]) + std::fabs((double)p->phi[(size_t)j * 2 + 1]);
+        p->e_bound = std::max(p->e_bound, rot * lam * 0x1p-12);
+    }
+    p->dscale_fold = std::ldexp(1.0f, 14 - (int)std::ceil(std::log2(p->d_bound + p->e_bound)));
     p->ok = true;
     return PSA_OK;
 }
@@ -177,9 +185,11 @@
     PSA_TRY(upload(c, c->d_lr_phi, p.phi.data(), p.phi.size() * sizeof(float)));
     PSA_TRY(c->d_lr_qn.reserve((size_t)LOWRANK_NODES * 3 * (size_t)c->slot[v.slot].T * sizeof(float2)));
     g->lowrank = true;
-    g->dscale = p.dscale;
+    g->lr_fold = c->k1_lowrank_fold;
+    g->dscale = g->lr_fold ? p.dscale_fold : p.dscale;
     g->M_pad_d = (int)((2 * nk + 511) / 512 * 512);
     g->lr_pair = c->opt_k1_lowrank_pair && g->M_pad_d == LRP_ROWS;
+    static_assert(LRF_ROWS == LRP_ROWS, "the folded pair launch serves the lists the pair launch serves");
     return PSA_OK;
 }
 
@@ -197,7 +207,8 @@
     LowRankPlan p;
     PSA_TRY(plan_lowrank(k_vectors, K, mean_pos_all, N, idx, n_g, &p, C));
     *ok = p.ok;
-    const double g[12] = {p.u[0], p.u[1], p.u[2], p.k0[0], p.k0[1], p.k0[2], p.x_c, p.h_x, p.width, (double)p.interval, p.d_bound, p.dscale};
+    const double g[14] = {p.u[0],  p.u[1],    p.u[2],           p.k0[0],   p.k0[1],  p.k0[2],   p.x_c,
+                          p.h_x,   p.width,   (double)p.interval, p.d_bound, p.dscale, p.e_bound, p.dscale_fold};
     std::memcpy(geo, g, sizeof(g));
     if (p.ok && kappa) std::memcpy(kappa, p.kappa, sizeof(p.kappa));
     if (p.ok && L) std::memcpy(L, p.L.data(), p.L.size() * sizeof(float));
@@ -214,4 +225,13 @@
     return PSA_OK;
 }
 
-}
+int psa_lowrank_fold_image(int32_t n_stage, int64_t* index, int64_t* bytes) {
+    PSA_REQUIRE(n_stage >= 1 && n_stage < (1 << 20) && bytes, "bad argument");
+    *bytes = (int64_t)pd16_fold_table_bytes(n_stage);
+    if (index)
+        for (int m = 0; m < LRF_ROWS; ++m)
+            for (int a = 0; a < n_stage * K1_BA; ++a) index[(size_t)m * n_stage * K1_BA + a] = (int64_t)pd16_fold_index(m, a, n_stage);
+    return PSA_OK;
+}
+
+}
diff --git a/psa_amd/csrc/api_project.hip b/psa_amd/csrc/api_project.hip
--- a/psa_amd/csrc/api_project.hip
+++ b/psa_amd/csrc/api_project.hip
@@ -248,6 +248,10 @@
         PSA_TRY(c->d_phase.reserve(pf16_table_bytes(128, g.A_pad)));
         StageTimer    st(c, PSA_T_PHASE);
         const double* f64 = c->d_lr_f64.as<double>();
+        if (g.lr_fold)
+            return launch_lowrank_tables_fold(c, d_kvec, f64 + 7 + LOWRANK_NODES, f64, f64 + 7, c->d_mean_all.as<float>(), d_idx,
+                                              c->d_lr_L.as<float>(), c->d_lr_phi.as<float2>(), c->d_lr_diff.ptr, c->d_phase.ptr, g,
+                                              g.M_pad_d, g.dscale, g.lr_pair);
         return launch_lowrank_tables(c, d_kvec, f64 + 7 + LOWRANK_NODES, f64, f64 + 7, c->d_mean_all.as<float>(), d_idx,
                                      c->d_lr_diff.ptr, c->d_phase.ptr, g, g.M_pad_d, g.dscale, g.lr_pair);
     }
@@ -303,10 +307,11 @@
             gn.q_stride = t_count;
             PSA_REQUIRE(c->d_lr_qn.cap >= (size_t)LOWRANK_NODES * 3 * t_count * sizeof(float2), "node projections not reserved");
             if (g.lr_pair) {
-                PSA_TRY(launch_k1_lowrank_pair(c, pl, c->d_phase.ptr, c->d_lr_diff.ptr, c->d_lr_qn.as<float2>(), d_q, g, n_fg, g.dscale));
+                PSA_TRY((g.lr_fold ? launch_k1_lowrank_fold : launch_k1_lowrank_pair)(c, pl, c->d_phase.ptr, c->d_lr_diff.ptr,
+                                                                                      c->d_lr_qn.as<float2>(), d_q, g, n_fg, g.dscale));
                 ++c->lowrank_pair_launches;
             } else {
-                PSA_TRY(launch_k1_planes_lw(c, pl, c->d_phase.ptr, c->d_lr_qn.as<float2>(), gn, n_fg));
+                PSA_TRY((g.lr_fold ? launch_k1_planes_lw2 : launch_k1_planes_lw)(c, pl, c->d_phase.ptr, c->d_lr_qn.as<float2>(), gn, n_fg));
                 ProjGeom gd = g;
                 gd.M_pad = g.M_pad_d;
                 PSA_TRY(launch_k1_planes_diff(c, pl, c->d_lr_diff.ptr, d_q, gd, n_fg, g.dscale));
diff --git a/psa_amd/csrc/k1_lowrank_fold.h b/psa_amd/csrc/k1_lowrank_fold.h
--- /dev/null
+++ b/psa_amd/csrc/k1_lowrank_fold.h
@@ -0,0 +1,28 @@
+#pragma once
+#include "k1_tile.h"
+
+namespace psa {
+
+constexpr int LRF_ROWS = 512;
+constexpr int LRF_A_ROWS = 128, LRF_A_MT = 4, LRF_A_UNITS = 2 * LRF_A_MT;
+constexpr int LRF_B_MT = 12, LRF_B_UNITS = 2 * LRF_B_MT;
+constexpr int LRF_PAD_STAGES = 4;
+static_assert(LRF_A_ROWS == 16 * LRF_A_UNITS && LRF_A_ROWS + 16 * LRF_B_UNITS == LRF_ROWS, "the two roles share the block's rows");
+
+__host__ __device__ inline size_t lrf_b_first_unit(int n_stage) { return (size_t)(n_stage + LRF_PAD_STAGES) * LRF_A_UNITS; }
+__host__ __device__ inline size_t pd16_fold_index(int m, int a, int n_stage) {
+    const int rt = m >> 4, r = m & 15, al = a % K1_BA, st = a / K1_BA;
+    size_t    unit;
+    if (rt < LRF_A_UNITS) {
+        unit = (size_t)st * LRF_A_UNITS + (size_t)(2 * (rt % LRF_A_MT) + rt / LRF_A_MT);
+    } else {
+        const int rb = rt - LRF_A_UNITS, h = rb / LRF_B_MT, mt = rb % LRF_B_MT;
+        unit = lrf_b_first_unit(n_stage) + (size_t)st * LRF_B_UNITS + (size_t)(2 * mt + h);
+    }
+    return unit * (16 * K1_BA) + (size_t)r * K1_BA + (size_t)((((al >> 3) ^ pl_swizzle(r)) << 3) + (al & 7));
+}
+__host__ __device__ inline size_t pd16_fold_table_bytes(int n_stage) {
+    return (size_t)(n_stage + LRF_PAD_STAGES) * (LRF_A_UNITS + LRF_B_UNITS) * 1024;
+}
+
+}
diff --git a/psa_amd/csrc/k1_lowrank_fold.hip b/psa_amd/csrc/k1_lowrank_fold.hip
--- /dev/null
+++ b/psa_amd/csrc/k1_lowrank_fold.hip
@@ -0,0 +1,279 @@
+#include <utility>
+
+#include "k1_f16.h"
+#include "k1_lowrank_fold.h"
+
+namespace psa {
+
+namespace {
+constexpr int LF_T_BLK = 64, LF_PERIOD = 4;
+constexpr int LFA_STAGE_UNITS = 24 + 8 + LRF_A_UNITS, LFA_RING_UNITS = LF_PERIOD * LFA_STAGE_UNITS, LFA_FOLD = 8, LFA_MT = LRF_A_MT;
+constexpr int LFA_NODE_U0 = 24, LFA_D_U0 = 32, LFA_DMA = LFA_STAGE_UNITS / 4;
+constexpr int LFB_STAGE_UNITS = 12 + LRF_B_UNITS, LFB_RING_UNITS = LF_PERIOD * LFB_STAGE_UNITS, LFB_D_U0 = 12, LFB_DMA = LFB_STAGE_UNITS / 4;
+constexpr int LF_NODE_STAGE_BYTES = pf16_stage_bytes(2 * LOWRANK_NODES);
+static_assert(LFA_STAGE_UNITS == 40 && LFA_RING_UNITS == 160 && LFA_FOLD % LF_PERIOD == 0 && LFA_DMA == 10, "role A's ring is four whole stages");
+static_assert(LFB_STAGE_UNITS == 36 && LFB_RING_UNITS == 144 && LFB_DMA == 9, "role B's ring is four whole stages");
+static_assert(3 * 2 * LFA_MT + 3 * LFA_MT == 3 * LRF_B_MT, "both roles multiply the same per stage: 36 MFMAs per wavefront");
+constexpr auto a_unit_off = unit_off<LFA_STAGE_UNITS, LFA_RING_UNITS, LF_PERIOD>;
+constexpr auto b_unit_off = unit_off<LFB_STAGE_UNITS, LFB_RING_UNITS, LF_PERIOD>;
+}
+
+__global__ void __launch_bounds__(512, 2)
+k1_lowrank_fold_kernel(const _Float16* __restrict__ planes, const _Float16* __restrict__ Pn, const _Float16* __restrict__ Dp,
+                       float2* __restrict__ Qn, float2* __restrict__ Q, int64_t T, int64_t q_stride, int n_fg, int n_stage, int K,
+                       int n_tblk, float qscale_n, float qscale_d) {
+    using PR = F16x2;
+    using E8 = PR::v8;
+    using std::integral_constant;
+    __shared__ __attribute__((aligned(16))) unsigned char smem[LFA_RING_UNITS * 1024];
+    const unsigned lds0 = (unsigned)(size_t)(lds_u8*)smem;
+
+    int mb, tb;
+    if (!k1_block_map(2, n_tblk, mb, tb)) return;
+
+    const int tid = threadIdx.x, lane = tid & 63;
+    const int w = __builtin_amdgcn_readfirstlane(tid >> 6);
+    const int wh = w >> 2, wf = w & 3;
+    const int r16 = lane & 15, q = lane >> 4;
+
+    int fg = tb * 4 + wf;
+    if (fg >= n_fg) fg = n_fg - 1;
+    const unsigned char* pl0 = reinterpret_cast<const unsigned char*>(planes) + (size_t)fg * n_stage * PL_STAGE_BYTES;
+    const unsigned dma_voff = 16 * lane;
+    const unsigned wbase = lds0 + 1024 * wf;
+    const unsigned lane_off = lds0 + r16 * (K1_BA * 2) + ((q ^ pl_swizzle(r16)) << 4);
+    unsigned       lane_a[3], lane_b[3];
+    unit_ring_windows(lane_off + 1024 * wh, lane_off + 1024 * wf, lane_a, lane_b);
+    using I0 = integral_constant<int, 0>;
+    using I1 = integral_constant<int, 1>;
+    using I2 = integral_constant<int, 2>;
+    using I3 = integral_constant<int, 3>;
+
+    if (mb == 0) {
+        const unsigned char* src[LFA_DMA];
+#pragma unroll
+        for (int i = 0; i < 6; ++i) src[i] = pl0 + 1024 * i;
+#pragma unroll
+        for (int j = 0; j < 2; ++j) {
+            const int x = 4 * j + wf;
+            src[6 + j] = reinterpret_cast<const unsigned char*>(Pn) + 1024 * (4 * (x & 1) + (x >> 1));
+            src[8 + j] = reinterpret_cast<const unsigned char*>(Dp) + 1024 * x;
+        }
+        auto dma = [&](auto s4_c, auto i_c) __attribute__((always_inline)) {
+            constexpr int      S4 = decltype(s4_c)::value, I = decltype(i_c)::value;
+            constexpr unsigned OFF = a_unit_off(S4, 4 * I);
+            if constexpr (I < 6) {
+                lds_dma16_at<OFF, (I & 1) != 0>(src[I], dma_voff, wbase);
+                src[I] += PL_STAGE_BYTES;
+            } else if constexpr (I < 8) {
+                lds_dma16_at<OFF, false>(src[I], dma_voff, wbase);
+                src[I] += LF_NODE_STAGE_BYTES;
+            } else {
+                lds_dma16_at<OFF, false>(src[I], dma_voff, wbase);
+                src[I] += LRF_A_UNITS * 1024;
+            }
+        };
+        auto dma_stage = [&](auto s4_c) __attribute__((always_inline)) {
+            [&]<int... Is>(std::integer_sequence<int, Is...>) __attribute__((always_inline)) { (dma(s4_c, integral_constant<int, Is>{}), ...); }(
+                std::make_integer_sequence<int, LFA_DMA>{});
+        };
+
+        E8    a[2][LFA_MT];
+        E8    ad[2][LFA_MT];
+        E8    bb[3][2];
+        f32x4 hi[LFA_MT][3], lo[LFA_MT][3], accd[LFA_MT][3];
+        auto  read_a = [&](auto s_c, auto mt_c) __attribute__((always_inline)) {
+            constexpr int S = decltype(s_c)::value, MTI = decltype(mt_c)::value;
+            a[S & 1][MTI] = lds_frag(lane_a, a_unit_off(S, LFA_NODE_U0 + 2 * MTI));
+        };
+        auto read_ad = [&](auto s_c, auto mt_c) __attribute__((always_inline)) {
+            constexpr int S = decltype(s_c)::value, MTI = decltype(mt_c)::value;
+            ad[S & 1][MTI] = lds_frag(lane_a, a_unit_off(S, LFA_D_U0 + 2 * MTI));
+        };
+        auto read_b = [&](auto s_c, auto c_c, auto p_c) __attribute__((always_inline)) {
+            constexpr int S = decltype(s_c)::value, CC = decltype(c_c)::value, P = decltype(p_c)::value;
+            bb[CC][P] = lds_frag(lane_b, a_unit_off(S, 4 * (2 * CC + P)));
+        };
+        auto each_mt = [&](auto&& f) __attribute__((always_inline)) {
+            f(I0{});
+            f(I1{});
+            f(I2{});
+            f(I3{});
+        };
+        static_assert(LFA_MT == 4 && LFA_FOLD % 2 == 0, "four row tiles; the fragment sets alternate with the stage");
+#pragma unroll
+        for (int mt = 0; mt < LFA_MT; ++mt)
+#pragma unroll
+            for (int c = 0; c < 3; ++c) {
+                hi[mt][c] = f32x4{0.f, 0.f, 0.f, 0.f};
+                lo[mt][c] = f32x4{0.f, 0.f, 0.f, 0.f};
+                accd[mt][c] = f32x4{0.f, 0.f, 0.f, 0.f};
+            }
+
+        if (wh == 0) {
+            dma_stage(I0{});
+            dma_stage(I1{});
+            dma_stage(I2{});
+        }
+        asm volatile("s_waitcnt vmcnt(%0)\n\ts_barrier" ::"n"(LFA_DMA) : "memory");
+        each_mt([&](auto mt_c) __attribute__((always_inline)) { read_a(I0{}, mt_c); });
+        read_b(I0{}, I0{}, I1{});
+        read_b(I0{}, I0{}, I0{});
+        each_mt([&](auto mt_c) __attribute__((always_inline)) { read_ad(I0{}, mt_c); });
+        read_b(I0{}, I1{}, I1{});
+        read_b(I0{}, I1{}, I0{});
+        read_b(I0{}, I2{}, I1{});
+        read_b(I0{}, I2{}, I0{});
+
+        int  left = n_stage;
+        auto stage = [&](auto s_c) __attribute__((always_inline)) {
+            constexpr int S = decltype(s_c)::value, PAR = S & 1;
+            if (left <= S) return;
+            constexpr bool restart = S == 0;
+            using SN = integral_constant<int, (S + 1) % LFA_FOLD>;
+            using S3 = integral_constant<int, (S + 3) % LFA_FOLD>;
+            if (wh == 0) dma_stage(S3{});
+            auto comp = [&](auto c_c) __attribute__((always_inline)) {
+                constexpr int CC = decltype(c_c)::value;
+                f32x4         ch[LFA_MT];
+                each_mt([&](auto mt_c) __attribute__((always_inline)) {
+                    constexpr int MTI = decltype(mt_c)::value;
+                    ch[MTI] = PR::mma(a[PAR][MTI], bb[CC][1], restart ? f32x4{0.f, 0.f, 0.f, 0.f} : hi[MTI][CC]);
+                });
+                read_b(SN{}, c_c, I1{});
+                if constexpr (CC == 0) each_mt([&](auto mt_c) __attribute__((always_inline)) { read_a(SN{}, mt_c); });
+                if constexpr (CC == 1) each_mt([&](auto mt_c) __attribute__((always_inline)) { read_ad(SN{}, mt_c); });
+                __builtin_amdgcn_sched_barrier(0);
+                each_mt([&](auto mt_c) __attribute__((always_inline)) {
+                    constexpr int MTI = decltype(mt_c)::value;
+                    accd[MTI][CC] = PR::mma(ad[PAR][MTI], bb[CC][0], accd[MTI][CC]);
+                });
+                each_mt([&](auto mt_c) __attribute__((always_inline)) {
+                    constexpr int MTI = decltype(mt_c)::value;
+                    hi[MTI][CC] = PR::mma(a[PAR][MTI], bb[CC][0], ch[MTI]);
+                });
+                read_b(SN{}, c_c, I0{});
+                __builtin_amdgcn_sched_barrier(0);
+            };
+            comp(I0{});
+            comp(I1{});
+            comp(I2{});
+            asm volatile("s_waitcnt vmcnt(%0)\n\ts_barrier" ::"n"(LFA_DMA) : "memory");
+        };
+        for (; left > 0; left -= LFA_FOLD) {
+            [&]<int... Ss>(std::integer_sequence<int, Ss...>) __attribute__((always_inline)) { (stage(integral_constant<int, Ss>{}), ...); }(
+                std::make_integer_sequence<int, LFA_FOLD>{});
+            k1_fold(lo, hi);
+        }
+        asm volatile("s_waitcnt vmcnt(0)" ::: "memory");
+
+        const int     lane_e = __builtin_amdgcn_mbcnt_hi(~0u, __builtin_amdgcn_mbcnt_lo(~0u, 0u));
+        const int     r16_e = lane_e & 15, q_e = lane_e >> 4;
+        const int64_t t = (int64_t)tb * LF_T_BLK + wf * 16 + r16_e;
+        k1_store_q(Qn, lo, wh * LOWRANK_NODES, q_e, t, T, LOWRANK_NODES, T, qscale_n);
+        k1_store_q(Q, accd, wh * (LRF_A_ROWS / 2), q_e, t, T, K, q_stride, qscale_d);
+    } else {
+        const unsigned char* src[LFB_DMA];
+#pragma unroll
+        for (int i = 0; i < 3; ++i) src[i] = pl0 + 1024 * (2 * i);
+        const unsigned char* d0 = reinterpret_cast<const unsigned char*>(Dp) + lrf_b_first_unit(n_stage) * 1024;
+#pragma unroll
+        for (int i = 3; i < LFB_DMA; ++i) src[i] = d0 + 1024 * (wf + 4 * (i - 3));
+        auto dma = [&](auto s4_c, auto i_c) __attribute__((always_inline)) {
+            constexpr int      S4 = decltype(s4_c)::value, I = decltype(i_c)::value;
+            constexpr unsigned OFF = b_unit_off(S4, 4 * I);
+            lds_dma16_at<OFF, false>(src[I], dma_voff, wbase);
+            src[I] += I < 3 ? PL_STAGE_BYTES : LRF_B_UNITS * 1024;
+        };
+        auto dma_stage = [&](auto s4_c) __attribute__((always_inline)) {
+            [&]<int... Is>(std::integer_sequence<int, Is...>) __attribute__((always_inline)) { (dma(s4_c, integral_constant<int, Is>{}), ...); }(
+                std::make_integer_sequence<int, LFB_DMA>{});
+        };
+
+        E8    a[4];
+        E8    bf[3];
+        f32x4 acc[LRF_B_MT][3];
+        static_assert(LRF_B_MT % 4 == 0, "row tile mt of every stage sits at mt mod 4 of the ring of four");
+        auto read_a = [&](auto s4_c, auto mt_c) __attribute__((always_inline)) {
+            constexpr int S4 = decltype(s4_c)::value, MTI = decltype(mt_c)::value;
+            a[MTI & 3] = lds_frag(lane_a, b_unit_off(S4, LFB_D_U0 + 2 * MTI));
+        };
+        auto read_b = [&](auto s4_c, auto c_c) __attribute__((always_inline)) {
+            constexpr int S4 = decltype(s4_c)::value, CC = decltype(c_c)::value;
+            bf[CC] = lds_frag(lane_b, b_unit_off(S4, 4 * CC));
+        };
+#pragma unroll
+        for (int mt = 0; mt < LRF_B_MT; ++mt)
+#pragma unroll
+            for (int c = 0; c < 3; ++c) acc[mt][c] = f32x4{0.f, 0.f, 0.f, 0.f};
+
+        if (wh == 0) {
+            dma_stage(I0{});
+            dma_stage(I1{});
+            dma_stage(I2{});
+        }
+        asm volatile("s_waitcnt vmcnt(%0)\n\ts_barrier" ::"n"(LFB_DMA) : "memory");
+        read_b(I0{}, I0{});
+        read_b(I0{}, I1{});
+        read_b(I0{}, I2{});
+        read_a(I0{}, I0{});
+        read_a(I0{}, I1{});
+
+        int  left = n_stage;
+        auto stage = [&](auto s4_c) __attribute__((always_inline)) {
+            constexpr int S4 = decltype(s4_c)::value;
+            if (left <= S4) return;
+            using SN = integral_constant<int, (S4 + 1) % LF_PERIOD>;
+            using S3 = integral_constant<int, (S4 + 3) % LF_PERIOD>;
+            if (wh == 0) dma_stage(S3{});
+            auto tile = [&](auto mt_c) __attribute__((always_inline)) {
+                constexpr int MTI = decltype(mt_c)::value;
+                if constexpr (MTI + 2 < LRF_B_MT)
+                    read_a(s4_c, integral_constant<int, MTI + 2>{});
+                else
+                    read_a(SN{}, integral_constant<int, MTI + 2 - LRF_B_MT>{});
+                auto comp = [&](auto c_c) __attribute__((always_inline)) {
+                    constexpr int CC = decltype(c_c)::value;
+                    acc[MTI][CC] = PR::mma(a[MTI & 3], bf[CC], acc[MTI][CC]);
+                    if constexpr (MTI == LRF_B_MT - 1) read_b(SN{}, c_c);
+                };
+                comp(I0{});
+                comp(I1{});
+                comp(I2{});
+                __builtin_amdgcn_sched_barrier(0);
+            };
+            [&]<int... Ms>(std::integer_sequence<int, Ms...>) __attribute__((always_inline)) { (tile(integral_constant<int, Ms>{}), ...); }(
+                std::make_integer_sequence<int, LRF_B_MT>{});
+            asm volatile("s_waitcnt vmcnt(%0)\n\ts_barrier" ::"n"(LFB_DMA) : "memory");
+        };
+        for (; left > 0; left -= LF_PERIOD)
+            [&]<int... Ss>(std::integer_sequence<int, Ss...>) __attribute__((always_inline)) { (stage(integral_constant<int, Ss>{}), ...); }(
+                std::make_integer_sequence<int, LF_PERIOD>{});
+        asm volatile("s_waitcnt vmcnt(0)" ::: "memory");
+
+        const int lane_e = __builtin_amdgcn_mbcnt_hi(~0u, __builtin_amdgcn_mbcnt_lo(~0u, 0u));
+        const int r16_e = lane_e & 15, q_e = lane_e >> 4;
+        k1_store_q(Q, acc, wh * (16 * LRF_B_MT) + LRF_A_ROWS, q_e, (int64_t)tb * LF_T_BLK + wf * 16 + r16_e, T, K, q_stride, qscale_d);
+    }
+}
+
+int launch_k1_lowrank_fold(psa_ctx* c, const void* d_planes, const void* d_nodes, const void* d_diff, float2* d_qn, float2* d_q,
+                           const ProjGeom& g, int64_t n_fg, float dscale) {
+    PSA_REQUIRE(g.M_pad_d == LRF_ROWS && 2 * g.K <= LRF_ROWS && g.K > 0, "folded pair launch: one 512-row D block only");
+    PSA_REQUIRE(g.A_pad % (2 * K1_BA) == 0 && g.A_pad > 0, "folded pair launch needs the atom axis padded to %d", 2 * K1_BA);
+    PSA_REQUIRE(g.vscale > 0.f && dscale > 0.f && n_fg * 16 >= g.T, "planes do not cover the launch");
+    ProjGeom g2 = g;
+    g2.M_pad = 2 * LRF_ROWS;
+    K1Grid gr;
+    PSA_TRY(k1_grid(g2, LRF_ROWS, LF_T_BLK, gr));
+    PSA_REQUIRE(gr.n_mblk == 2 && gr.n_tblk < (1 << 29) && n_fg < (1ll << 31), "projection grid too large");
+    const float qscale_n = 1.f / (g.vscale * F16x2::P_SCALE) * g.wscale;
+    const float qscale_d = 1.f / (g.vscale * dscale) * g.wscale;
+    hipLaunchKernelGGL(k1_lowrank_fold_kernel, dim3(gr.blocks), dim3(512), 0, c->stream, (const _Float16*)d_planes,
+                       (const _Float16*)d_nodes, (const _Float16*)d_diff, d_qn, d_q, g.T, g.q_stride, (int)n_fg, g.A_pad / K1_BA, g.K,
+                       gr.n_tblk, qscale_n, qscale_d);
+    PSA_HIP_CHECK(hipGetLastError());
+    return PSA_OK;
+}
+
+}
diff --git a/psa_amd/csrc/k1_planes_diff.hip b/psa_amd/csrc/k1_planes_diff.hip
--- a/psa_amd/csrc/k1_planes_diff.hip
+++ b/psa_amd/csrc/k1_planes_diff.hip
@@ -1,6 +1,7 @@
 #include <utility>
 
 #include "k1_f16.h"
+#include "k1_lowrank_fold.h"
 #include "k1_lowrank_pair.h"
 
 namespace psa {
@@ -156,6 +157,20 @@
                                 d_planes, d_diff, d_q, g, n_fg);
 }
 
+__device__ __forceinline__ void diff_parts(const float* __restrict__ kvec, const double* __restrict__ kline,
+                                           const float* __restrict__ mean_all, const int* __restrict__ idx,
+                                           const float* __restrict__ w, float wnorm, int k, int a, float (&cs)[2], double& ce,
+                                           double& se, double& wa) {
+    const int   src = idx ? idx[a] : a;
+    const float rx = mean_all[3 * (size_t)src + 0], ry = mean_all[3 * (size_t)src + 1], rz = mean_all[3 * (size_t)src + 2];
+    const float kx = kvec[3 * k + 0], ky = kvec[3 * k + 1], kz = kvec[3 * k + 2];
+    const float arg = __fmaf_rn(kz, rz, __fmaf_rn(ky, ry, __fmul_rn(kx, rx)));
+    sincosf(arg, &cs[1], &cs[0]);
+    const double th = kline[3 * k + 0] * (double)rx + kline[3 * k + 1] * (double)ry + kline[3 * k + 2] * (double)rz;
+    sincos(th, &se, &ce);
+    wa = w ? (double)(w[src] * wnorm) : 1.0;
+}
+
 template <bool PAIR>
 __global__ void __launch_bounds__(256)
 diff_table_kernel(const float* __restrict__ kvec, const double* __restrict__ kline, const float* __restrict__ mean_all,
@@ -213,6 +228,69 @@
     }
 }
 
+constexpr int FOLD_JB = 16;
+template <bool FOLD>
+__global__ void __launch_bounds__(256)
+diff_fold_table_kernel(const float* __restrict__ kvec, const double* __restrict__ kline, const float* __restrict__ mean_all,
+                       const int* __restrict__ idx, const float* __restrict__ w, float wnorm, const _Float16* __restrict__ Pn,
+                       const float* __restrict__ L, const float2* __restrict__ phi, _Float16* __restrict__ Db, int K, int n_g,
+                       int A_pad, float dscale) {
+    const int a = blockIdx.y * 256 + threadIdx.x;
+    const int k0 = blockIdx.x * FOLD_JB;
+    if (a >= A_pad) return;
+    const int n_stage = A_pad / K1_BA;
+    _Float16  wl[2 * LOWRANK_NODES];
+#pragma unroll
+    for (int m = 0; m < 2 * LOWRANK_NODES; ++m) wl[m] = Pn[pf16_tile_index(1, m, a, 2 * LOWRANK_NODES, n_stage)];
+    for (int k = k0; k < k0 + FOLD_JB; ++k) {
+        float d[2] = {0.f, 0.f};
+        if (k < K && a < n_g) {
+            const float* Lk = L + (size_t)k * LOWRANK_NODES;
+            float        sr = 0.f, si = 0.f;
+#pragma unroll
+            for (int l = 0; l < LOWRANK_NODES; ++l) {
+                sr = __fmaf_rn(Lk[l], (float)wl[2 * l], sr);
+                si = __fmaf_rn(Lk[l], (float)wl[2 * l + 1], si);
+            }
+            const float2 ph = phi[k];
+            const float  er = __fmaf_rn(-ph.y, si, __fmul_rn(ph.x, sr)), ei = __fmaf_rn(ph.y, sr, __fmul_rn(ph.x, si));
+            float        cs[2];
+            double       se, ce, wa;
+            diff_parts(kvec, kline, mean_all, idx, w, wnorm, k, a, cs, ce, se, wa);
+            constexpr double inv_p = 1.0 / (double)F16x2::P_SCALE;
+            d[0] = (float)((((double)cs[0] - ce) * wa + (double)er * inv_p) * (double)dscale);
+            d[1] = (float)((((double)cs[1] - se) * wa + (double)ei * inv_p) * (double)dscale);
+        }
+        Db[FOLD ? pd16_fold_index(2 * k, a, n_stage) : pd16_index(2 * k, a, n_stage)] = (_Float16)d[0];
+        Db[FOLD ? pd16_fold_index(2 * k + 1, a, n_stage) : pd16_index(2 * k + 1, a, n_stage)] = (_Float16)d[1];
+    }
+}
+
+int launch_lowrank_tables_fold(psa_ctx* c, const float* d_kvec, const double* d_kline, const double* d_geo, const double* d_kappa,
+                               const float* d_mean_all, const int* d_idx, const float* d_L, const float2* d_phi, void* d_diff,
+                               void* d_nodes, const ProjGeom& g, int M_pad_d, float dscale, bool pair) {
+    PSA_REQUIRE(M_pad_d % D_M_BLK == 0 && M_pad_d >= 2 * g.K && g.A_pad % K1_BA == 0, "bad low-rank table geometry");
+    PSA_REQUIRE(!pair || M_pad_d == LRF_ROWS, "the folded pair launch's image is one 512-row block");
+    static_assert((D_M_BLK / 2) % FOLD_JB == 0, "whole blocks of rows");
+    hipLaunchKernelGGL(node_table_kernel, dim3(LOWRANK_NODES, (g.A_pad + 255) / 256), dim3(256), 0, c->stream, d_geo, d_kappa, d_mean_all,
+                       d_idx, g.weights, 1.f / g.wscale, (_Float16*)d_nodes, g.n_g, g.A_pad);
+    PSA_HIP_CHECK(hipGetLastError());
+    hipLaunchKernelGGL(pair ? diff_fold_table_kernel<true> : diff_fold_table_kernel<false>,
+                       dim3(M_pad_d / 2 / FOLD_JB, (g.A_pad + 255) / 256), dim3(256), 0, c->stream, d_kvec, d_kline, d_mean_all, d_idx,
+                       g.weights, 1.f / g.wscale, (const _Float16*)d_nodes, d_L, d_phi, (_Float16*)d_diff, g.K, g.n_g, g.A_pad, dscale);
+    PSA_HIP_CHECK(hipGetLastError());
+    if (pair) {
+        const size_t n_stage = (size_t)g.A_pad / K1_BA, a_pad = LRF_PAD_STAGES * LRF_A_UNITS * 1024, b_pad = LRF_PAD_STAGES * LRF_B_UNITS * 1024;
+        static_assert(LRF_ROWS == D_M_BLK, "the fold image has the size of one D block");
+        PSA_HIP_CHECK(hipMemsetAsync((char*)d_diff + n_stage * LRF_A_UNITS * 1024, 0, a_pad, c->stream));
+        PSA_HIP_CHECK(hipMemsetAsync((char*)d_diff + pd16_fold_table_bytes((int)n_stage) - b_pad, 0, b_pad, c->stream));
+    } else {
+        PSA_HIP_CHECK(hipMemsetAsync((char*)d_diff + (size_t)M_pad_d * g.A_pad * 2, 0,
+                                     pd16_table_bytes(M_pad_d, g.A_pad) - (size_t)M_pad_d * g.A_pad * 2, c->stream));
+    }
+    return PSA_OK;
+}
+
 int launch_lowrank_tables(psa_ctx* c, const float* d_kvec, const double* d_kline, const double* d_geo, const double* d_kappa,
                           const float* d_mean_all, const int* d_idx, void* d_diff, void* d_nodes, const ProjGeom& g, int M_pad_d,
                           float dscale, bool pair) {
diff --git a/psa_amd/csrc/k1_planes_lw.hip b/psa_amd/csrc/k1_planes_lw.hip
--- a/psa_amd/csrc/k1_planes_lw.hip
+++ b/psa_amd/csrc/k1_planes_lw.hip
@@ -2,7 +2,7 @@
 
 namespace psa {
 
-template <bool NT_V>
+template <bool NT_V, bool TWO = false>
 __global__ void __launch_bounds__(768, 3)
 k1_planes_lw_kernel(const _Float16* __restrict__ planes, const _Float16* __restrict__ Pb, float2* __restrict__ Q,
                     int64_t T, int64_t q_stride, int n_fg, int n_stage, int K, int n_mblk, int n_tblk, float qscale) {
@@ -12,7 +12,7 @@
     constexpr int P_STAGE_BYTES = pf16_stage_bytes(M_BLK);
     constexpr int V_GROUP_BYTES = PL_STAGE_BYTES;
     constexpr int STAGE_BYTES = P_STAGE_BYTES + 4 * V_GROUP_BYTES;
-    constexpr int BATCH = 10;
+    constexpr int BATCH = TWO ? 8 : 10;
     static_assert(RING * STAGE_BYTES == 160 * 1024, "the ring is all of LDS");
     __shared__ __attribute__((aligned(16))) unsigned char smem[RING * STAGE_BYTES];
     const unsigned lds0 = (unsigned)(size_t)(lds_u8*)smem;
@@ -32,7 +32,10 @@
         const unsigned       p_voff = 4096 * j + 16 * lane, v_voff = 16 * lane;
         auto dma_stage = [&](int slot) {
             const unsigned dst = lds0 + slot * STAGE_BYTES;
-            lds_dma16_group<4>(p_next, p_voff, dst + 4096 * j);
+            if constexpr (TWO)
+                lds_dma16_group<2>(p_next, 2048 * j + 16 * lane, dst + 2048 * j);
+            else
+                lds_dma16_group<4>(p_next, p_voff, dst + 4096 * j);
             lds_dma16_group<3, NT_V>(v_next, v_voff, dst + P_STAGE_BYTES + j * V_GROUP_BYTES);
             lds_dma16_group<3, NT_V>(v_next, v_voff + 3072, dst + P_STAGE_BYTES + j * V_GROUP_BYTES + 3072);
             p_next += P_STAGE_BYTES;
@@ -66,7 +69,7 @@
     auto  read_a_tile = [&](int mt, int slot) {
         const unsigned base = p_lane + slot * STAGE_BYTES;
 #pragma unroll
-        for (int p = 0; p < NP; ++p)
+        for (int p = 0; p < (TWO ? 1 : NP); ++p)
             a[p][mt] = *reinterpret_cast<lds_cv8*>((const lds_u8*)(size_t)(base + (p * M_BLK + mt * 16) * 64));
     };
     auto read_b = [&](int buf, int slot, int c) {
@@ -101,9 +104,14 @@
                 read_b(cur ^ 1, slot1, 0);
 #pragma unroll
             for (int mt = 0; mt < MT16; ++mt) {
-                f32x4 ch = PR::mma(a[1][mt], bb[cur][0], restart ? f32x4{0.f, 0.f, 0.f, 0.f} : hi[mt][c]);
-                ch = PR::mma(a[0][mt], bb[cur][1], ch);
-                hi[mt][c] = PR::mma(a[0][mt], bb[cur][0], ch);
+                if constexpr (TWO) {
+                    const f32x4 ch = PR::mma(a[0][mt], bb[cur][1], restart ? f32x4{0.f, 0.f, 0.f, 0.f} : hi[mt][c]);
+                    hi[mt][c] = PR::mma(a[0][mt], bb[cur][0], ch);
+                } else {
+                    f32x4 ch = PR::mma(a[1][mt], bb[cur][0], restart ? f32x4{0.f, 0.f, 0.f, 0.f} : hi[mt][c]);
+                    ch = PR::mma(a[0][mt], bb[cur][1], ch);
+                    hi[mt][c] = PR::mma(a[0][mt], bb[cur][0], ch);
+                }
                 if (c == 2) read_a_tile(mt, slot1);
             }
         }
@@ -120,4 +128,10 @@
                                 F16x2::P_SCALE, d_planes, d_phase, d_q, g, n_fg);
 }
 
+int launch_k1_planes_lw2(psa_ctx* c, const void* d_planes, const void* d_phase, float2* d_q, const ProjGeom& g, int64_t n_fg) {
+    PSA_REQUIRE(g.m_blk == 128 && g.M_pad % 128 == 0, "loader-wave planes kernel: 128-row M blocks only");
+    return launch_planes_family(c, k1_planes_lw_kernel<true, true>, k1_planes_lw_kernel<false, true>, 128, 768, "planes kernel", 2 * K1_BA,
+                                F16x2::P_SCALE, d_planes, d_phase, d_q, g, n_fg);
 }
+
+}
diff --git a/psa_amd/csrc/psa_ctx.h b/psa_amd/csrc/psa_ctx.h
--- a/psa_amd/csrc/psa_ctx.h
+++ b/psa_amd/csrc/psa_ctx.h
@@ -156,6 +156,7 @@
     int     M_pad_d = 0;
     float   dscale = 0.f;
     bool    lr_pair = false;
+    bool    lr_fold = false;
     const float* weights = nullptr;
     float        wscale = 1.f;
 };
@@ -249,6 +250,7 @@
     int64_t      lowrank_launches = 0;
     int64_t      opt_k1_lowrank_pair;
     int64_t      lowrank_pair_launches = 0;
+    bool         k1_lowrank_fold = true;
     psa::DevBuf  d_lr_diff, d_lr_qn, d_lr_L, d_lr_phi, d_lr_f64;
 
     psa::DevBuf  d_weights;
@@ -339,6 +341,8 @@
                         int64_t n_fg);
 int    launch_k1_planes_lw(psa_ctx* c, const void* d_planes, const void* d_phase, float2* d_q, const ProjGeom& g,
                            int64_t n_fg);
+int    launch_k1_planes_lw2(psa_ctx* c, const void* d_planes, const void* d_phase, float2* d_q, const ProjGeom& g,
+                            int64_t n_fg);
 
 int    launch_k1_planes_wide(psa_ctx* c, const void* d_planes, const void* d_phase, float2* d_q, const ProjGeom& g,
                              int64_t n_fg);
@@ -349,8 +353,14 @@
                              float dscale, bool pair);
 int    launch_k1_planes_diff(psa_ctx* c, const void* d_planes, const void* d_diff, float2* d_q, const ProjGeom& g, int64_t n_fg,
                              float dscale);
+int    launch_lowrank_tables_fold(psa_ctx* c, const float* d_kvec, const double* d_kline, const double* d_geo, const double* d_kappa,
+                                  const float* d_mean_all, const int* d_idx, const float* d_L, const float2* d_phi, void* d_diff,
+                                  void* d_nodes, const ProjGeom& g, int M_pad_d, float dscale, bool pair);
 
 int    launch_k1_lowrank_pair(psa_ctx* c, const void* d_planes, const void* d_nodes, const void* d_diff, float2* d_qn, float2* d_q,
+                              const ProjGeom& g, int64_t n_fg, float dscale);
+
+int    launch_k1_lowrank_fold(psa_ctx* c, const void* d_planes, const void* d_nodes, const void* d_diff, float2* d_qn, float2* d_q,
                               const ProjGeom& g, int64_t n_fg, float dscale);
 
 int    launch_lowrank_combine_r(psa_ctx* c, const float2* d_qn, const float* d_L, const float2* d_phi, float2* d_q, const ProjGeom& g,
```

Result: faster. 61080 billion, median of 6 (+11.2%).
